# boqian-li/GarmentDreamer

Measured on AMD Instinct MI355X. Metric: SDS iters/sec (rasterize+UNet+bwd), 100k Gaussians ×8 views @512², 1/2/4/8 GPU, higher is better.
Workload: dtype bf16

## Files before the change

garmentdreamer_amd/csrc/nn_conv3x3.hip:

```cpp
#include <hip/hip_runtime.h>
#include <stdlib.h>
#include <stdint.h>
#include <stdio.h>

#include <mutex>
#include <vector>

#include "../../include/gd_nn.h"
#include "nn_device.h"
#include "nn_host.h"

#ifndef GD_CONV_ABLATE
#define GD_CONV_ABLATE 0
#endif

namespace {

using namespace gdnn;

#ifndef GD_PATCH_EPI
#define GD_PATCH_EPI 0
#endif
typedef __attribute__((ext_vector_type(4))) float f32x4;

// ... 15 lines not shown
    constexpr int NA = BM * 8 / THREADS;
    constexpr int NB = BN * 8 / THREADS;
    constexpr int FA = BN / WN / 32;
    constexpr int FB = BM / WM / 32;
    constexpr int kStage = (BM + BN) * BK * 2;
    extern __shared__ __attribute__((aligned(16))) char smem[];
    const int tid = threadIdx.x, lane = tid & 63;
    const int wave = __builtin_amdgcn_readfirstlane(tid >> 6);
    int bid = bid_raw;
    if ((nwg & 7) == 0) bid = (bid & 7) * (nwg >> 3) + (bid >> 3);
    const int tn = bid % tiles_n, tm = bid / tiles_n;
    const int m0 = tm * BM, n0 = tn * BN;
    const int HW = g.Hg * g.Wg;
    const int64_t M = (int64_t)Nimg * HW;
    const int H = g.Hin, W = g.Win;

    const uint32_t row_bytes = (uint32_t)Cin * 2u;
    const uint32_t back = (uint32_t)g.back * row_bytes;
    const __amdgpu_buffer_rsrc_t rs_in = buffer_rsrc((const char*)in - back, (uint32_t)Nimg * (uint32_t)(H * W) * row_bytes + back);
    const __amdgpu_buffer_rsrc_t rs_w = buffer_rsrc(wt, (uint32_t)Cout * (uint32_t)g.wtaps * row_bytes);

    uint32_t a_off[NA];
    int a_y[NA], a_x[NA];
    uint32_t b_off[NB];
#pragma unroll
    for (int i = 0; i < NA; i++) {
        const int q = tid + THREADS * i;
        const int line = q >> 4, c = (q & 15) ^ (line & 15);
        const int r = 2 * line + (c >> 3);
        const int64_t m = (int64_t)m0 + r;
        if (m < M) {
            const int nimg = (int)(m / HW);
            const int rem = (int)(m - (int64_t)nimg * HW);
            const int ga = rem / g.Wg;
            a_y[i] = ga * g.sy;
            a_x[i] = (rem - ga * g.Wg) * g.sx;
            a_off[i] = (uint32_t)((nimg * H + a_y[i]) * W + a_x[i]) * row_bytes + (uint32_t)(c & 7) * 16u;
        } else {
            a_y[i] = -100000; a_x[i] = 0; a_off[i] = kOOB;
        }
    }
#pragma unroll
    for (int i = 0; i < NB; i++) {
        const int q = tid + THREADS * i;
        const int line = q >> 4, c = (q & 15) ^ (line & 15);
        const int r = 2 * line + (c >> 3);
        const int co = n0 + r;
        b_off[i] = co < Cout ? (uint32_t)co * (uint32_t)g.wtaps * row_bytes + (uint32_t)(c & 7) * 16u : kOOB;
    }
    const int kc = Cin / BK;
    const int step0 = partial ? split_idx * steps_per_split : 0;
    const int step1 = partial ? min(g.ntaps * kc, step0 + steps_per_split) : g.ntaps * kc;
    const int nsteps = step1 - step0;
    const int tap0 = step0 / kc;

    int ld_tap = tap0, ld_c = step0 - tap0 * kc;
    uint32_t a_voff[NA];
    auto set_tap = [&](int tap) {
        const int dy = (int)((g.ty4 >> (4 * tap)) & 15u) - 8, dx = (int)((g.tx4 >> (4 * tap)) & 15u) - 8;
#pragma unroll
        for (int i = 0; i < NA; i++) {
            const int yy = a_y[i] + dy, xx = a_x[i] + dx;
            const bool ok = (unsigned)yy < (unsigned)H && (unsigned)xx < (unsigned)W;
            a_voff[i] = ok ? a_off[i] : kOOB;
        }
    };
    set_tap(tap0);
    auto issue = [&](int buf) {
        char* sA = smem + buf * kStage;
        char* sB = sA + BM * BK * 2;
        const int dy = (int)((g.ty4 >> (4 * ld_tap)) & 15u) - 8, dx = (int)((g.tx4 >> (4 * ld_tap)) & 15u) - 8;
        const uint32_t soff_a = (uint32_t)(dy * W + dx + g.back) * row_bytes + (uint32_t)ld_c * (BK * 2);
        const uint32_t soff_b = (uint32_t)((g.w4 >> (4 * ld_tap)) & 15u) * row_bytes + (uint32_t)ld_c * (BK * 2);
#if GD_CONV_ABLATE != 1 && GD_CONV_ABLATE != 2 && GD_CONV_ABLATE < 6
#pragma unroll
        for (int i = 0; i < NA; i++) bload_lds16(rs_in, a_voff[i], soff_a, sA + (wave * 64 + THREADS * i) * 16);
#endif
#if GD_CONV_ABLATE != 2 && GD_CONV_ABLATE < 6
#pragma unroll
        for (int i = 0; i < NB; i++) bload_lds16(rs_w, b_off[i], soff_b, sB + (wave * 64 + THREADS * i) * 16);
#endif
        if (++ld_c == kc) {
            ld_c = 0;
            if (++ld_tap < g.ntaps) set_tap(ld_tap);
        }
    };

    f32x16 acc[FA][FB];
#pragma unroll
    for (int a = 0; a < FA; a++)
#pragma unroll
        for (int b = 0; b < FB; b++)
#pragma unroll
            for (int k = 0; k < 16; k++) acc[a][b][k] = 0.f;

    const int wc = wave % WN, wp = wave / WN;
    const int frow = lane & 31, fk = lane >> 5;
    uint32_t w_rd[FA], p_rd[FB];
#pragma unroll
    for (int a = 0; a < FA; a++) w_rd[a] = (uint32_t)(BM * BK * 2 + swz(wc * (BN / WN) + a * 32 + frow, fk));
#pragma unroll
    for (int b = 0; b < FB; b++) p_rd[b] = (uint32_t)swz(wp * (BM / WM) + b * 32 + frow, fk);

#if GD_CONV_ABLATE == 4 || GD_CONV_ABLATE >= 6
    bf16x8_t wf0[FA], pf0[FB];
#pragma unroll
    for (int a = 0; a < FA; a++) wf0[a] = *(const bf16x8_t*)(smem + w_rd[a]);
#pragma unroll
    for (int b = 0; b < FB; b++) pf0[b] = *(const bf16x8_t*)(smem + p_rd[b]);
#endif
    issue(0);
#if GD_CONV_ABLATE == 8
    for (int s = 0; s < (nsteps > 1 ? 1 : nsteps); s++) {
#else
    for (int s = 0; s < nsteps; s++) {
#endif
        const int buf = s & 1;
        asm volatile("s_waitcnt vmcnt(0)" ::: "memory");
#if GD_CONV_ABLATE != 5 && GD_CONV_ABLATE != 6
        __syncthreads();
#endif
        if (s + 1 < nsteps) issue(buf ^ 1);
        const char* st = smem + buf * kStage;
#pragma unroll
        for (int kk = 0; kk < 4; kk++) {
            bf16x8_t wf[FA], pf[FB];
#if GD_CONV_ABLATE == 4 || GD_CONV_ABLATE >= 6
            if (s > 0) {
#pragma unroll
                for (int a = 0; a < FA; a++)
#pragma unroll
                    for (int b = 0; b < FB; b++)
                        acc[a][b] = __builtin_amdgcn_mfma_f32_32x32x16_bf16(wf0[a], pf0[b], acc[a][b], 0, 0, 0);
                continue;
            }
#endif
#pragma unroll
            for (int a = 0; a < FA; a++) wf[a] = *(const bf16x8_t*)(st + (w_rd[a] ^ (uint32_t)(kk << 5)));
#pragma unroll
            for (int b = 0; b < FB; b++) pf[b] = *(const bf16x8_t*)(st + (p_rd[b] ^ (uint32_t)(kk << 5)));
#pragma unroll
            for (int a = 0; a < FA; a++)
#pragma unroll
                for (int b = 0; b < FB; b++)
#if GD_CONV_ABLATE == 3
                    if (a == 0 && b == 0) acc[a][b] = __builtin_amdgcn_mfma_f32_32x32x16_bf16(wf[a], pf[b], acc[a][b], 0, 0, 0);
                    else { acc[a][b][0] += __builtin_bit_cast(float, (int)wf[a][0] ^ (int)pf[b][1]); }
#else
                    acc[a][b] = __builtin_amdgcn_mfma_f32_32x32x16_bf16(wf[a], pf[b], acc[a][b], 0, 0, 0);
#endif
        }
    }

#pragma unroll
    for (int b = 0; b < FB; b++) {
        const int64_t m = (int64_t)m0 + wp * (BM / WM) + b * 32 + (lane & 31);
        if (m >= M) continue;
        const int nimg = (int)(m / HW);
        const int rem = (int)(m - (int64_t)nimg * HW);
        const int ga = rem / g.Wg, gb = rem - ga * g.Wg;
        const size_t opix = ((size_t)nimg * g.Hout + (size_t)(ga * g.osy + g.ooy)) * g.Wout + (size_t)(gb * g.osx + g.oox);
        const uint16_t* bias_n = bias ? bias + (size_t)nimg * bias_img_stride : nullptr;
#pragma unroll
        for (int a = 0; a < FA; a++) {
#pragma unroll
            for (int q = 0; q < 4; q++) {
                const int co = n0 + wc * (BN / WN) + a * 32 + 8 * q + 4 * fk;
                if (co >= Cout) continue;
                float v[4];
#pragma unroll
                for (int e = 0; e < 4; e++) v[e] = acc[a][b][4 * q + e];
                if (partial) {
                    *(float4*)(partial + (((size_t)split_idx * nwg + bid) * (BN * BM / 4) +
                                          (((wave * FB + b) * FA + a) * 4 + q) * 64 + lane) * 4) = make_float4(v[0], v[1], v[2], v[3]);
                    continue;
                }
                if (bias_n) {
                    const uint2 bb = *(const uint2*)(bias_n + co);
                    v[0] += bf2f((uint16_t)(bb.x & 0xffff)); v[1] += bf2f((uint16_t)(bb.x >> 16));
                    v[2] += bf2f((uint16_t)(bb.y & 0xffff)); v[3] += bf2f((uint16_t)(bb.y >> 16));
                }
                if (residual) {
                    const uint2 rr = *(const uint2*)(residual + opix * Cout + co);
                    v[0] += bf2f((uint16_t)(rr.x & 0xffff)); v[1] += bf2f((uint16_t)(rr.x >> 16));
                    v[2] += bf2f((uint16_t)(rr.y & 0xffff)); v[3] += bf2f((uint16_t)(rr.y >> 16));
                }
                uint2 o;
                o.x = pack_bf16(v[0], v[1]);
                o.y = pack_bf16(v[2], v[3]);
                *(uint2*)(out + opix * Cout + co) = o;
            }
        }
    }
}

template <int BN, int BM, int WN, int WM>
__global__ __launch_bounds__(64 * WN * WM) void conv3x3_nhwc_bf16_kernel(
    const uint16_t* __restrict__ in, const uint16_t* __restrict__ wt, const uint16_t* __restrict__ bias,
    int bias_img_stride, const uint16_t* __restrict__ residual, uint16_t* __restrict__ out, int Nimg, const ConvGeom g,
    int Cin, int Cout, int tiles_n, int nwg, float* __restrict__ partial, int steps_per_split)
{
    conv3x3_nhwc_bf16_body<BN, BM, WN, WM>(in, wt, bias, bias_img_stride, residual, out, Nimg, g, Cin, Cout, tiles_n, nwg,
                                           partial, steps_per_split, (int)blockIdx.x, (int)blockIdx.y);
}

struct ConvGeomSet {
    ConvGeom g[4];
    const uint16_t* wt[4];
    int nwg[4];
    int n;
};

template <int BN, int BM, int WN, int WM>
__global__ __launch_bounds__(64 * WN * WM) void conv3x3_nhwc_bf16_multi_kernel(
    const uint16_t* __restrict__ in, const uint16_t* __restrict__ bias, int bias_img_stride,
    const uint16_t* __restrict__ residual, uint16_t* __restrict__ out, int Nimg, const ConvGeomSet gs, int Cin, int Cout,
    int tiles_n)
{
    const int cls = (int)blockIdx.z;
    const int nwg = gs.nwg[cls];
    if ((int)blockIdx.x >= nwg) return;
    conv3x3_nhwc_bf16_body<BN, BM, WN, WM>(in, gs.wt[cls], bias, bias_img_stride, residual, out, Nimg, gs.g[cls], Cin, Cout,
                                           tiles_n, nwg, nullptr, 0, (int)blockIdx.x, 0);
}

constexpr int kPatch = 18, kPatchPix = kPatch * kPatch;

__device__ __forceinline__ float silu_fast(float z) { return z * __builtin_amdgcn_rcpf(1.0f + __expf(-z)); }

__device__ __forceinline__ float row16_sum(float v)
{
    v += __builtin_bit_cast(float, __builtin_amdgcn_update_dpp(0, __builtin_bit_cast(int, v), 0xB1, 0xf, 0xf, false));
    v += __builtin_bit_cast(float, __builtin_amdgcn_update_dpp(0, __builtin_bit_cast(int, v), 0x4E, 0xf, 0xf, false));
    v += __builtin_bit_cast(float, __builtin_amdgcn_update_dpp(0, __builtin_bit_cast(int, v), 0x141, 0xf, 0xf, false));
    v += __builtin_bit_cast(float, __builtin_amdgcn_update_dpp(0, __builtin_bit_cast(int, v), 0x140, 0xf, 0xf, false));
    return v;
}

__device__ __forceinline__ void stat_accumulate(float2& st, uint2 o)
{
    const float r0 = __uint_as_float(o.x << 16), r1 = __uint_as_float(o.x & 0xffff0000u);
    const float r2 = __uint_as_float(o.y << 16), r3 = __uint_as_float(o.y & 0xffff0000u);
    st.x += (r0 + r1) + (r2 + r3);
    st.y += fmaf(r0, r0, fmaf(r1, r1, fmaf(r2, r2, r3 * r3)));
}

__device__ __forceinline__ void patch_col(int fn, int& rr, int& fx)
{
    if (fn < 4) { rr = 0; fx = fn; }
    else if (fn < 12) { rr = 1; fx = fn - 4; }
    else if (fn < 16) { rr = 0; fx = fn - 8; }
    else if (fn < 20) { rr = 1; fx = fn - 8; }
    else if (fn < 28) { rr = 0; fx = fn - 12; }
    else { rr = 1; fx = fn - 16; }
}

constexpr int kTrRow = 80;
constexpr int kTrWave = 64 * kTrRow;

constexpr int kResRound = 64 * 64;

__device__ __forceinline__ void res_tile_lane(int lane, uint32_t pix_bytes, uint32_t img_row_bytes, uint32_t (&off)[2])
{
    const uint32_t chunk = (uint32_t)((lane & 3) ^ ((lane >> 4) & 3));
#pragma unroll
    for (int h = 0; h < 2; h++) {
        int rr, fx;
        patch_col(16 * h + (lane >> 2), rr, fx);
        off[h] = (uint32_t)rr * img_row_bytes + (uint32_t)fx * pix_bytes + chunk * 16u;
    }
}

__device__ __forceinline__ void res_tile_issue(__amdgpu_buffer_rsrc_t rs, const uint32_t (&off)[2], uint32_t base,
                                               uint32_t two_rows, char* slot)
{
#pragma unroll
    for (int i = 0; i < 4; i++) bload_lds16(rs, off[i & 1], base + (uint32_t)(i >> 1) * two_rows, slot + i * 1024);
}

typedef __attribute__((ext_vector_type(2))) uint32_t res_u32x2;
typedef __attribute__((ext_vector_type(4))) uint32_t res_u32x4;

__device__ __forceinline__ void res_tile_read(uint32_t slot_off, int lane, res_u32x2 (&r)[2][4])
{
    const int fn = lane & 31, fk = lane >> 5;
    const uint32_t a0 = slot_off + (uint32_t)(fn * 64 + 8 * fk), key = (uint32_t)((fn >> 2) & 3);
    const uint32_t q0 = a0 + (key << 4), q1 = a0 + ((1u ^ key) << 4), q2 = a0 + ((2u ^ key) << 4), q3 = a0 + ((3u ^ key) << 4);
    asm volatile("ds_read_b64 %0, %8\n\tds_read_b64 %1, %9\n\tds_read_b64 %2, %10\n\tds_read_b64 %3, %11\n\t"
                 "ds_read_b64 %4, %8 offset:2048\n\tds_read_b64 %5, %9 offset:2048\n\t"
                 "ds_read_b64 %6, %10 offset:2048\n\tds_read_b64 %7, %11 offset:2048\n\ts_waitcnt lgkmcnt(0)"
                 : "=&v"(r[0][0]), "=&v"(r[0][1]), "=&v"(r[0][2]), "=&v"(r[0][3]), "=&v"(r[1][0]), "=&v"(r[1][1]),
                   "=&v"(r[1][2]), "=&v"(r[1][3])
                 : "v"(q0), "v"(q1), "v"(q2), "v"(q3)
                 : "memory");
}

struct ResTile {
    uint16_t* out;
    size_t pix0;
    int Cout;
    float* stat_img;
    int stat_rows, stat_row;
    bool stat_ok;
};

struct PatchPix {
    int W;
    __device__ __forceinline__ int operator()(int pr) const
    {
        int rr, fx;
        patch_col(pr & 31, rr, fx);
        return (2 * (pr >> 5) + rr) * W + fx;
    }
};

template <class PixOf, class AfterRead>
__device__ __forceinline__ void res_round(const f32x16& acc0, const f32x16& acc1, const uint2 (&bb)[4], uint32_t slot_off,
                                          uint32_t tr_off, int lane, const ResTile& t, int co0, PixOf pix_of,
                                          AfterRead after_read)
{
    const int fk = lane >> 5, fn = lane & 31;
    res_u32x2 rv[2][4];
    res_tile_read(slot_off, lane, rv);
    after_read();
#pragma unroll
    for (int q = 0; q < 4; q++) {
        const int co = co0 + 8 * q + 4 * fk;
        const float bv[4] = {bf2f((uint16_t)(bb[q].x & 0xffff)), bf2f((uint16_t)(bb[q].x >> 16)),
                             bf2f((uint16_t)(bb[q].y & 0xffff)), bf2f((uint16_t)(bb[q].y >> 16))};
        float2 st = make_float2(0.f, 0.f);
#pragma unroll
        for (int j = 0; j < 2; j++) {
            float v[4];
#pragma unroll
            for (int e = 0; e < 4; e++) v[e] = (j ? acc1 : acc0)[4 * q + e] + bv[e];
            const uint32_t r0 = rv[j][q][0], r1 = rv[j][q][1];
            v[0] += bf2f((uint16_t)(r0 & 0xffff)); v[1] += bf2f((uint16_t)(r0 >> 16));
            v[2] += bf2f((uint16_t)(r1 & 0xffff)); v[3] += bf2f((uint16_t)(r1 >> 16));
            uint2 o;
            o.x = pack_bf16(v[0], v[1]);
            o.y = pack_bf16(v[2], v[3]);
            const res_u32x2 ov = {o.x, o.y};
            asm volatile("ds_write_b64 %0, %1" ::"v"(tr_off + (uint32_t)((j * 32 + fn) * kTrRow + 16 * q + 8 * fk)), "v"(ov)
                         : "memory");
            if (t.stat_img) stat_accumulate(st, o);
        }
        if (t.stat_img) {
            const float sx = row16_sum(st.x), sy = row16_sum(st.y);
            if ((lane & 15) == 0 && t.stat_ok)
                *(float2*)(t.stat_img + ((size_t)(co >> 2) * t.stat_rows + t.stat_row + ((lane >> 4) & 1)) * 2) =
                    make_float2(sx, sy);
        }
    }
    res_u32x4 tv[4];
    asm volatile("ds_read_b128 %0, %4\n\tds_read_b128 %1, %4 offset:1280\n\tds_read_b128 %2, %4 offset:2560\n\t"
                 "ds_read_b128 %3, %4 offset:3840\n\ts_waitcnt lgkmcnt(0)"
                 : "=&v"(tv[0]), "=&v"(tv[1]), "=&v"(tv[2]), "=&v"(tv[3])
                 : "v"(tr_off + (uint32_t)((lane >> 2) * kTrRow + (lane & 3) * 16))
                 : "memory");
    static_assert(16 * kTrRow == 1280, "offsets of the four reads");
#pragma unroll
    for (int i = 0; i < 4; i++) {
        const int pr = (lane >> 2) + 16 * i;
        *(uint4*)(t.out + (t.pix0 + (size_t)pix_of(pr)) * t.Cout + co0 + 8 * (lane & 3)) =
            make_uint4(tv[i][0], tv[i][1], tv[i][2], tv[i][3]);
    }
}

template <int BN, int WN, int FA, int FB>
__device__ __forceinline__ void patch_epilogue(f32x16 (&acc)[FA][FB], char* tr, int nimg, int tyi, int txi, int n0, int wc,
                                               int wp, int lane, int H, int W, int Cout, const uint16_t* __restrict__ bias,
                                               int bias_img_stride, const uint16_t* __restrict__ residual,
                                               uint16_t* __restrict__ out, float* __restrict__ stat_part, int tpi,
                                               int tiles_x)
{
    const int fk = lane >> 5, fn = lane & 31;
    int rr, fx;
    patch_col(fn, rr, fx);
    bool ok[FB];
    size_t opix[FB];
#pragma unroll
    for (int b = 0; b < FB; b++) {
        const int oy = tyi * 16 + 4 * wp + 2 * b + rr, ox = txi * 16 + fx;
        ok[b] = oy < H && ox < W;
        opix[b] = ((size_t)nimg * H + oy) * W + ox;
    }
    const uint16_t* bias_n = bias ? bias + (size_t)nimg * bias_img_stride : nullptr;
    const int stat_rows = tpi * 8;
    const int stat_row = (tyi * tiles_x + txi) * 8 + wp * 2 + ((lane >> 4) & 1);
    const bool wide = GD_PATCH_EPI != 2 && tr != nullptr && (Cout & 7) == 0;
#pragma unroll
    for (int a = 0; a < FA; a++) {
#pragma unroll
        for (int q = 0; q < 4; q++) {
            const int co = n0 + wc * (BN / WN) + a * 32 + 8 * q + 4 * fk;
            const bool cok = co < Cout;
            float bv[4] = {0.f, 0.f, 0.f, 0.f};
            if (bias_n && cok) {
                const uint2 bb = *(const uint2*)(bias_n + co);
                bv[0] = bf2f((uint16_t)(bb.x & 0xffff)); bv[1] = bf2f((uint16_t)(bb.x >> 16));
                bv[2] = bf2f((uint16_t)(bb.y & 0xffff)); bv[3] = bf2f((uint16_t)(bb.y >> 16));
            }
            float2 st = make_float2(0.f, 0.f);
#pragma unroll
            for (int b = 0; b < FB; b++) {
                if (!ok[b] || !cok) continue;
                float v[4];
#pragma unroll
                for (int e = 0; e < 4; e++) v[e] = acc[a][b][4 * q + e] + bv[e];
                if (residual) {
                    const uint2 rv = *(const uint2*)(residual + opix[b] * Cout + co);
                    v[0] += bf2f((uint16_t)(rv.x & 0xffff)); v[1] += bf2f((uint16_t)(rv.x >> 16));
                    v[2] += bf2f((uint16_t)(rv.y & 0xffff)); v[3] += bf2f((uint16_t)(rv.y >> 16));
                }
                uint2 o;
                o.x = pack_bf16(v[0], v[1]);
                o.y = pack_bf16(v[2], v[3]);
                if (wide) *(uint2*)(tr + (b * 32 + fn) * kTrRow + 16 * q + 8 * fk) = o;
                else if (GD_PATCH_EPI != 1 || H < 0) *(uint2*)(out + opix[b] * Cout + co) = o;
                if (stat_part) stat_accumulate(st, o);
            }
            if (stat_part) {
                const float sx = row16_sum(st.x), sy = row16_sum(st.y);
                if ((lane & 15) == 0 && cok)
                    *(float2*)(stat_part + (((size_t)nimg * (Cout >> 2) + (co >> 2)) * stat_rows + stat_row) * 2) =
                        make_float2(sx, sy);
            }
        }
        if (wide) {
            __builtin_amdgcn_wave_barrier();
#pragma unroll
            for (int i = 0; i < FB * 2; i++) {
                const int pr = (lane >> 2) + 16 * i, ch = lane & 3;
                int rr2, fx2;
                patch_col(pr & 31, rr2, fx2);
                const int oy = tyi * 16 + 4 * wp + 2 * (pr >> 5) + rr2, ox = txi * 16 + fx2;
                const int co8 = n0 + wc * (BN / WN) + a * 32 + 8 * ch;
                if (oy < H && ox < W && co8 < Cout) {
                    const uint4 v = *(const uint4*)(tr + pr * kTrRow + ch * 16);
                    if (GD_PATCH_EPI != 1 || H < 0) *(uint4*)(out + (((size_t)nimg * H + oy) * W + ox) * Cout + co8) = v;
                }
            }
            __builtin_amdgcn_wave_barrier();
        }
    }
}

template <int BN, int WN, int WM, bool GN, bool RES>
__global__ __launch_bounds__(64 * WN * WM) void conv3x3_gn_patch_kernel(
    const uint16_t* __restrict__ in, const uint16_t* __restrict__ wt, const uint16_t* __restrict__ bias,
    int bias_img_stride, const uint16_t* __restrict__ residual, uint16_t* __restrict__ out, int Nimg, int H, int W,
    int Cin, int Cout, const float* __restrict__ mean_rstd, const uint16_t* __restrict__ gamma,
    const uint16_t* __restrict__ beta, int G, int apply_silu, int tiles_n, int tiles_x, int tiles_y, int nwg,
    float* __restrict__ stat_part)
{
    constexpr int BM = 256;
    constexpr int THREADS = 64 * WN * WM;
    constexpr int NB = BN * 8 / THREADS;
    constexpr int NA = (kPatchPix * 8 + THREADS - 1) / THREADS;
    constexpr int FA = BN / WN / 32, FB = BM / WM / 32;
    static_assert(FB == 2 && THREADS % 8 == 0, "wave pixel block = 4 patch rows x 16");
    constexpr int kAStage = (kPatchPix + 4) * BK * 2;
    constexpr int kBStage = BN * BK * 2;
    extern __shared__ __attribute__((aligned(16))) char smem[];
    char* sA = smem;
    char* sB = smem + 2 * kAStage;

    const int tid = threadIdx.x, lane = tid & 63;
    const int wave = __builtin_amdgcn_readfirstlane(tid >> 6);
    int bid = blockIdx.x;
    if ((nwg & 7) == 0) bid = (bid & 7) * (nwg >> 3) + (bid >> 3);
    const int tn = bid % tiles_n, tm = bid / tiles_n;
    const int tpi = tiles_x * tiles_y;
    const int nimg = tm / tpi, trem = tm - nimg * tpi;
    const int tyi = trem / tiles_x, txi = trem - tyi * tiles_x;
    const int y0 = tyi * 16 - 1, x0 = txi * 16 - 1;
    const int n0 = tn * BN;

    const uint32_t row_bytes = (uint32_t)Cin * 2u;
    const __amdgpu_buffer_rsrc_t rs_in = buffer_rsrc(in, (uint32_t)Nimg * (uint32_t)(H * W) * row_bytes);
    const __amdgpu_buffer_rsrc_t rs_w = buffer_rsrc(wt, (uint32_t)Cout * 9u * row_bytes);

    const int a_chunk = tid & 7;
    uint32_t a_goff[NA];
    uint32_t a_lds[NA];
    uint32_t a_keep = 0;
    uint32_t a_slot = 0;
#pragma unroll
    for (int i = 0; i < NA; i++) {
        const int pix = (tid + THREADS * i) >> 3;
        const int py = pix / kPatch, px = pix - py * kPatch;
        const int gy = y0 + py, gx = x0 + px;
        const bool slot = pix < kPatchPix;
        const bool inimg = slot && (unsigned)gy < (unsigned)H && (unsigned)gx < (unsigned)W;
        const int oct = GN ? a_chunk : (a_chunk ^ ((pix >> 1) & 7));
        a_goff[i] = inimg ? (uint32_t)((nimg * H + gy) * W + gx) * row_bytes + (uint32_t)oct * 16u : kOOB;
        a_lds[i] = (uint32_t)pix * 128u + (uint32_t)((a_chunk ^ ((pix >> 1) & 7)) << 4);
        if (inimg) a_keep |= 1u << i;
        if (slot) a_slot |= 1u << i;
    }
    uint4 a_reg[NA];
    auto loadA = [&](int c) {
#pragma unroll
        for (int i = 0; i < NA; i++) {
            auto v = __builtin_amdgcn_raw_buffer_load_b128(rs_in, (int)a_goff[i], (int)(c * (BK * 2)), 0);
            a_reg[i] = __builtin_bit_cast(uint4, v);
        }
    };
    const uint32_t tab_off = (uint32_t)(uintptr_t)(smem + 2 * kAStage + 2 * kBStage);
    auto storeA = [&](int buf, int c) {
        const uint32_t dst_off = (uint32_t)(uintptr_t)(sA + buf * kAStage);
        float sc[8], sh[8];
        if (mean_rstd) gn_table_read(tab_off, c * (BK / 8) + a_chunk, sc, sh);
#pragma unroll
        for (int i = 0; i < NA; i++) {
            if (!((a_slot >> i) & 1u)) continue;
            uint4 v = a_reg[i];
            if (mean_rstd) {
                uint32_t w4[4] = {v.x, v.y, v.z, v.w};
                const bool keep = (a_keep >> i) & 1u;
#pragma unroll
                for (int k = 0; k < 4; k++) {
                    float lo = __uint_as_float(w4[k] << 16), hi = __uint_as_float(w4[k] & 0xffff0000u);
                    lo = lo * sc[2 * k] + sh[2 * k];
                    hi = hi * sc[2 * k + 1] + sh[2 * k + 1];
                    if (apply_silu) { lo = silu_fast(lo); hi = silu_fast(hi); }
                    w4[k] = keep ? pack_bf16(lo, hi) : 0u;
                }
                v = make_uint4(w4[0], w4[1], w4[2], w4[3]);
            }
            typedef __attribute__((ext_vector_type(4))) uint32_t vec4;
            const vec4 vv = {v.x, v.y, v.z, v.w};
            asm volatile("ds_write_b128 %0, %1" ::"v"(dst_off + a_lds[i]), "v"(vv) : "memory");
        }
    };

    uint32_t b_off[NB];
#pragma unroll
    for (int i = 0; i < NB; i++) {
        const int q = tid + THREADS * i;
        const int line = q >> 4, cc = (q & 15) ^ (line & 15);
        const int r = 2 * line + (cc >> 3);
        const int co = n0 + r;
        b_off[i] = co < Cout ? (uint32_t)co * 9u * row_bytes + (uint32_t)(cc & 7) * 16u : kOOB;
    }
    auto issueB = [&](int buf, int tap, int c) {
        char* dst = sB + buf * kBStage;
        const uint32_t soff = (uint32_t)tap * row_bytes + (uint32_t)c * (BK * 2);
#pragma unroll
        for (int i = 0; i < NB; i++) bload_lds16(rs_w, b_off[i], soff, dst + (wave * 64 + THREADS * i) * 16);
    };

    f32x16 acc[FA][FB];
#pragma unroll
    for (int a = 0; a < FA; a++)
#pragma unroll
        for (int b = 0; b < FB; b++)
#pragma unroll
            for (int k = 0; k < 16; k++) acc[a][b][k] = 0.f;

    const int wc = wave % WN, wp = wave / WN;
    const int fk = lane >> 5, fn = lane & 31;
    int rr, fx;
    if (fn < 4) { rr = 0; fx = fn; }
    else if (fn < 12) { rr = 1; fx = fn - 4; }
    else if (fn < 16) { rr = 0; fx = fn - 8; }
    else if (fn < 20) { rr = 1; fx = fn - 8; }
    else if (fn < 28) { rr = 0; fx = fn - 12; }
    else { rr = 1; fx = fn - 16; }
    uint32_t w_rd[FA];
    int p_base[FB];
#pragma unroll
    for (int a = 0; a < FA; a++) w_rd[a] = (uint32_t)swz(wc * (BN / WN) + a * 32 + fn, fk);
#pragma unroll
    for (int b = 0; b < FB; b++) p_base[b] = (4 * wp + 2 * b + rr) * kPatch + fx;

    const int kc = Cin / BK;
    const int nsteps = 9 * kc;
    auto issueA = [&](int buf, int c) {
        char* dst = sA + buf * kAStage;
#pragma unroll
        for (int i = 0; i < NA; i++) {
            if (i == NA - 1 && wave * 64 + THREADS * i >= kPatchPix * 8) continue;
            bload_lds16(rs_in, a_goff[i], (uint32_t)c * (BK * 2), dst + (wave * 64 + THREADS * i) * 16);
        }
    };
    static_assert(FA == 2 || FA == 4, "rounds of the residual tile");
    const bool dma = RES && residual != nullptr && (Cout & 7) == 0 && tyi * 16 + 16 <= H && txi * 16 + 16 <= W && n0 + BN <= Cout &&
                     (uint64_t)Nimg * (uint64_t)(H * W) * (uint64_t)Cout * 2u < (1ull << 32);
    const uint32_t res_pix = (uint32_t)Cout * 2u, res_row = (uint32_t)W * res_pix;
    const __amdgpu_buffer_rsrc_t rs_res = buffer_rsrc(residual, (uint32_t)Nimg * (uint32_t)(H * W) * res_pix);
    auto res_slot = [&](int r) -> char* {
        if (r == 0 || r == 3) return sA + (kc & 1) * kAStage + wave * kResRound;
        return sB + (r - 1) * (8 * kResRound) + wave * kResRound;
    };
    auto issueR = [&](int r) {
        uint32_t off[2];
        res_tile_lane(lane, res_pix, res_row, off);
        const uint32_t base = (uint32_t)((nimg * H + tyi * 16 + 4 * wp) * W + txi * 16) * res_pix +
                              (uint32_t)(n0 + wc * (BN / WN) + r * 32) * 2u;
        res_tile_issue(rs_res, off, base, 2u * res_row, res_slot(r));
    };

    if (GN) {
        if (mean_rstd) gn_table_fill(tab_off, tid, THREADS, Cin, G, nimg, mean_rstd, gamma, beta);
        loadA(0);
        issueB(0, 0, 0);
        if (mean_rstd) gn_table_sync();
        storeA(0, 0);
    } else {
        issueA(0, 0);
        issueB(0, 0, 0);
    }
    int s = 0;
    for (int c = 0; c < kc; c++) {
        const char* pa = sA + (c & 1) * kAStage;
        for (int tap = 0; tap < 9; tap++, s++) {
            const int bufB = s & 1;
            if (GN) asm volatile("s_waitcnt vmcnt(0) lgkmcnt(0)" ::: "memory");
            else asm volatile("s_waitcnt vmcnt(0)" ::: "memory");
            __syncthreads();
            if (s + 1 < nsteps) issueB(bufB ^ 1, tap == 8 ? 0 : tap + 1, tap == 8 ? c + 1 : c);
            if (c + 1 < kc) {
                if (GN) {
                    if (tap == 0) loadA(c + 1);
                    else if (tap == 1) storeA((c + 1) & 1, c + 1);
                } else if (tap == 0) {
                    issueA((c + 1) & 1, c + 1);
                }
            } else if (tap == 0 && dma) {
                issueR(0);
            }
            const char* pb = sB + bufB * kBStage;
            const int tapoff = (tap / 3) * kPatch + (tap % 3);
            uint32_t p_rd[FB], p_sw[FB];
#pragma unroll
            for (int b = 0; b < FB; b++) {
                const int p = p_base[b] + tapoff;
                p_rd[b] = (uint32_t)p * 128u;
                p_sw[b] = (uint32_t)((p >> 1) & 7);
            }
#pragma unroll
            for (int kk = 0; kk < 4; kk++) {
                bf16x8_t wf[FA], pf[FB];
#pragma unroll
                for (int a = 0; a < FA; a++) wf[a] = *(const bf16x8_t*)(pb + (w_rd[a] ^ (uint32_t)(kk << 5)));
#pragma unroll
                for (int b = 0; b < FB; b++)
                    pf[b] = *(const bf16x8_t*)(pa + p_rd[b] + ((((uint32_t)(2 * kk + fk)) ^ p_sw[b]) << 4));
#pragma unroll
                for (int a = 0; a < FA; a++)
#pragma unroll
                    for (int b = 0; b < FB; b++)
                        acc[a][b] = __builtin_amdgcn_mfma_f32_32x32x16_bf16(wf[a], pf[b], acc[a][b], 0, 0, 0);
            }
        }
    }

    if (GD_PATCH_EPI != 2) __syncthreads();
    if (GD_PATCH_EPI == 0 && dma) {
        const uint32_t tr_off = (uint32_t)(uintptr_t)(sA + ((kc - 1) & 1) * kAStage + wave * kTrWave);
        const uint16_t* bias_d = bias ? bias + (size_t)nimg * bias_img_stride : nullptr;
        uint2 bb[FA][4];
#pragma unroll
        for (int a = 0; a < FA; a++)
#pragma unroll
            for (int q = 0; q < 4; q++)
                bb[a][q] = bias_d ? *(const uint2*)(bias_d + n0 + wc * (BN / WN) + a * 32 + 8 * q + 4 * fk) : make_uint2(0u, 0u);
        asm volatile("" ::: "memory");
        issueR(1);
        if (FA == 4) issueR(2);
        ResTile t;
        t.out = out; t.Cout = Cout;
        t.pix0 = ((size_t)nimg * H + (tyi * 16 + 4 * wp)) * W + txi * 16;
        t.stat_rows = tpi * 8;
        t.stat_img = stat_part ? stat_part + (size_t)nimg * (Cout >> 2) * t.stat_rows * 2 : nullptr;
        t.stat_row = (tyi * tiles_x + txi) * 8 + wp * 2;
        t.stat_ok = true;
#pragma unroll
        for (int r = 0; r < FA; r++) {
            if (r == FA - 3) asm volatile("s_waitcnt vmcnt(8)" ::: "memory");
            else if (r == FA - 2 && r > 0) asm volatile("s_waitcnt vmcnt(4)" ::: "memory");
            else if (r == FA - 1) asm volatile("s_waitcnt vmcnt(0)" ::: "memory");
            res_round(acc[r][0], acc[r][1], bb[r], (uint32_t)(uintptr_t)res_slot(r), tr_off, lane, t,
                      n0 + wc * (BN / WN) + r * 32, PatchPix{W}, [&] { if (FA == 4 && r == 0) issueR(3); });
        }
        return;
    }
    patch_epilogue<BN, WN, FA, FB>(acc, sA + ((kc - 1) & 1) * kAStage + wave * kTrWave, nimg, tyi, txi, n0, wc, wp, lane, H, W,
                                   Cout, bias, bias_img_stride, residual, out, stat_part, tpi, tiles_x);
}

template <int BN, int WN, int WM, bool GN>
__global__ __launch_bounds__(64 * WN * WM) void conv3x3_patch_stream_kernel(
    const uint16_t* __restrict__ in, const uint16_t* __restrict__ wt, const uint16_t* __restrict__ bias,
    int bias_img_stride, const uint16_t* __restrict__ residual, uint16_t* __restrict__ out, int Nimg, int H, int W,
    int Cin, int Cout, const float* __restrict__ mean_rstd, const uint16_t* __restrict__ gamma,
    const uint16_t* __restrict__ beta, int G, int apply_silu, int tiles_n, int tiles_x, int tiles_y, int nwg,
    float* __restrict__ stat_part)
{
    constexpr int BM = 256;
    constexpr int THREADS = 64 * WN * WM;
    constexpr int NB = BN * 8 / THREADS;
    constexpr int NA = (kPatchPix * 8 + THREADS - 1) / THREADS;
    constexpr int FA = BN / WN / 32, FB = BM / WM / 32;
    static_assert(FB == 2 && THREADS % 8 == 0, "wave pixel block = 4 patch rows x 16");
    constexpr int kAStage = (kPatchPix + 4) * BK * 2;
    constexpr int kBStage = BN * BK * 2;
    extern __shared__ __attribute__((aligned(16))) char smem[];
    char* sA = smem;
    char* sB = smem + 2 * kAStage;

    const int tid = threadIdx.x, lane = tid & 63;
    const int wave = __builtin_amdgcn_readfirstlane(tid >> 6);
    const int tpi = tiles_x * tiles_y;
    const bool remap = (nwg & 7) == 0 && (GN || (gridDim.x & 7) == 0);
    struct Tile { int nimg, tyi, txi, n0; };
    auto decode = [&](int vb) {
        int bid = vb;
        if (remap) bid = (vb & 7) * (nwg >> 3) + (vb >> 3);
        const int tn = bid % tiles_n, tm = bid / tiles_n;
        Tile t;
        t.nimg = tm / tpi;
        const int trem = tm - t.nimg * tpi;
        t.tyi = trem / tiles_x;
        t.txi = trem - t.tyi * tiles_x;
        t.n0 = tn * BN;
        return t;
    };

    const uint32_t row_bytes = (uint32_t)Cin * 2u;
    const __amdgpu_buffer_rsrc_t rs_in = buffer_rsrc(in, (uint32_t)Nimg * (uint32_t)(H * W) * row_bytes);
    const __amdgpu_buffer_rsrc_t rs_w = buffer_rsrc(wt, (uint32_t)Cout * 9u * row_bytes);

    const int a_chunk = tid & 7;
    uint32_t a_goff[NA];
    uint32_t a_lds[NA];
    uint32_t a_keep = 0;
    uint32_t a_slot = 0;
#pragma unroll
    for (int i = 0; i < NA; i++) {
        const int pix = (tid + THREADS * i) >> 3;
        a_lds[i] = (uint32_t)pix * 128u + (uint32_t)((a_chunk ^ ((pix >> 1) & 7)) << 4);
        if (pix < kPatchPix) a_slot |= 1u << i;
    }
    auto setupA = [&](const Tile& t) {
        const int y0 = t.tyi * 16 - 1, x0 = t.txi * 16 - 1;
        a_keep = 0;
#pragma unroll
        for (int i = 0; i < NA; i++) {
            const int pix = (tid + THREADS * i) >> 3;
            const int py = pix / kPatch, px = pix - py * kPatch;
            const int gy = y0 + py, gx = x0 + px;
            const bool inimg = pix < kPatchPix && (unsigned)gy < (unsigned)H && (unsigned)gx < (unsigned)W;
            const int oct = GN ? a_chunk : (a_chunk ^ ((pix >> 1) & 7));
            a_goff[i] = inimg ? (uint32_t)((t.nimg * H + gy) * W + gx) * row_bytes + (uint32_t)oct * 16u : kOOB;
            if (inimg) a_keep |= 1u << i;
        }
    };
    uint4 a_reg[NA];
    auto loadA = [&](int c) {
#pragma unroll
        for (int i = 0; i < NA; i++) {
            auto v = __builtin_amdgcn_raw_buffer_load_b128(rs_in, (int)a_goff[i], (int)(c * (BK * 2)), 0);
            a_reg[i] = __builtin_bit_cast(uint4, v);
        }
    };
    const uint32_t tab_off = (uint32_t)(uintptr_t)(smem + 2 * kAStage + 2 * kBStage);
    auto storeA = [&](int buf, int c) {
        const uint32_t dst_off = (uint32_t)(uintptr_t)(sA + buf * kAStage);
        float sc[8], sh[8];
        if (mean_rstd) gn_table_read(tab_off, c * (BK / 8) + a_chunk, sc, sh);
#pragma unroll
        for (int i = 0; i < NA; i++) {
            if (!((a_slot >> i) & 1u)) continue;
            uint4 v = a_reg[i];
            if (mean_rstd) {
                uint32_t w4[4] = {v.x, v.y, v.z, v.w};
                const bool keep = (a_keep >> i) & 1u;
#pragma unroll
                for (int k = 0; k < 4; k++) {
                    float lo = __uint_as_float(w4[k] << 16), hi = __uint_as_float(w4[k] & 0xffff0000u);
                    lo = lo * sc[2 * k] + sh[2 * k];
                    hi = hi * sc[2 * k + 1] + sh[2 * k + 1];
                    if (apply_silu) { lo = silu_fast(lo); hi = silu_fast(hi); }
                    w4[k] = keep ? pack_bf16(lo, hi) : 0u;
                }
                v = make_uint4(w4[0], w4[1], w4[2], w4[3]);
            }
            typedef __attribute__((ext_vector_type(4))) uint32_t vec4;
            const vec4 vv = {v.x, v.y, v.z, v.w};
            asm volatile("ds_write_b128 %0, %1" ::"v"(dst_off + a_lds[i]), "v"(vv) : "memory");
        }
    };

    uint32_t b_off[NB];
    auto setupB = [&](const Tile& t) {
#pragma unroll
        for (int i = 0; i < NB; i++) {
            const int q = tid + THREADS * i;
            const int line = q >> 4, cc = (q & 15) ^ (line & 15);
            const int r = 2 * line + (cc >> 3);
            const int co = t.n0 + r;
            b_off[i] = co < Cout ? (uint32_t)co * 9u * row_bytes + (uint32_t)(cc & 7) * 16u : kOOB;
        }
    };
    auto issueB = [&](int buf, int tap, int c) {
        char* dst = sB + buf * kBStage;
        const uint32_t soff = (uint32_t)tap * row_bytes + (uint32_t)c * (BK * 2);
#pragma unroll
        for (int i = 0; i < NB; i++) bload_lds16(rs_w, b_off[i], soff, dst + (wave * 64 + THREADS * i) * 16);
    };

    f32x16 acc[FA][FB];

    const int wc = wave % WN, wp = wave / WN;
    const int fk = lane >> 5, fn = lane & 31;
    int rr, fx;
    if (fn < 4) { rr = 0; fx = fn; }
    else if (fn < 12) { rr = 1; fx = fn - 4; }
    else if (fn < 16) { rr = 0; fx = fn - 8; }
    else if (fn < 20) { rr = 1; fx = fn - 8; }
    else if (fn < 28) { rr = 0; fx = fn - 12; }
    else { rr = 1; fx = fn - 16; }
    uint32_t w_rd[FA];
    int p_base[FB];
#pragma unroll
    for (int a = 0; a < FA; a++) w_rd[a] = (uint32_t)swz(wc * (BN / WN) + a * 32 + fn, fk);
#pragma unroll
    for (int b = 0; b < FB; b++) p_base[b] = (4 * wp + 2 * b + rr) * kPatch + fx;

    const int kc = Cin / BK;
    auto issueA = [&](int buf, int c) {
        char* dst = sA + buf * kAStage;
#pragma unroll
        for (int i = 0; i < NA; i++) {
            if (i == NA - 1 && wave * 64 + THREADS * i >= kPatchPix * 8) continue;
            bload_lds16(rs_in, a_goff[i], (uint32_t)c * (BK * 2), dst + (wave * 64 + THREADS * i) * 16);
        }
    };
    int vb = blockIdx.x;
    Tile cur = decode(vb);
    setupB(cur);
    setupA(cur);
#pragma unroll
    for (int a = 0; a < FA; a++)
#pragma unroll
        for (int b = 0; b < FB; b++)
#pragma unroll
            for (int k = 0; k < 16; k++) acc[a][b][k] = 0.f;
    if (GN) {
        if (mean_rstd) gn_table_fill(tab_off, tid, THREADS, Cin, G, cur.nimg, mean_rstd, gamma, beta);
        loadA(0);
        issueB(0, 0, 0);
        if (mean_rstd) gn_table_sync();
        storeA(0, 0);
    } else {
        issueA(0, 0);
        issueB(0, 0, 0);
    }
    int s = 0;
    int ga = 0;
    for (;;) {
        const int vnext = vb + (int)gridDim.x;
        const bool has_next = !GN && vnext < nwg;
        const Tile nxt = decode(has_next ? vnext : vb);
        for (int c = 0; c < kc; c++, ga++) {
            const char* pa = sA + (ga & 1) * kAStage;
            const bool last_chunk = c + 1 == kc;
            if (last_chunk && has_next) setupA(nxt);
            for (int tap = 0; tap < 9; tap++, s++) {
                const int bufB = s & 1;
                if (GN) asm volatile("s_waitcnt vmcnt(0) lgkmcnt(0)" ::: "memory");
                else asm volatile("s_waitcnt vmcnt(0)" ::: "memory");
                __syncthreads();
                if (!(last_chunk && tap == 8)) {
                    issueB(bufB ^ 1, tap == 8 ? 0 : tap + 1, tap == 8 ? c + 1 : c);
                } else if (has_next) {
                    setupB(nxt);
                    issueB(bufB ^ 1, 0, 0);
                }
                if (!last_chunk || has_next) {
                    const int nc = last_chunk ? 0 : c + 1;
                    const int st = (ga + 1) & 1;
                    if (GN) {
                        if (tap == 0) loadA(nc);
                        else if (tap == 1) storeA(st, nc);
                    } else if (tap == 0) {
                        issueA(st, nc);
                    }
                }
                const char* pb = sB + bufB * kBStage;
                const int tapoff = (tap / 3) * kPatch + (tap % 3);
                uint32_t p_rd[FB], p_sw[FB];
#pragma unroll
                for (int b = 0; b < FB; b++) {
                    const int p = p_base[b] + tapoff;
                    p_rd[b] = (uint32_t)p * 128u;
                    p_sw[b] = (uint32_t)((p >> 1) & 7);
                }
#pragma unroll
                for (int kk = 0; kk < 4; kk++) {
                    bf16x8_t wf[FA], pf[FB];
#pragma unroll
                    for (int a = 0; a < FA; a++) wf[a] = *(const bf16x8_t*)(pb + (w_rd[a] ^ (uint32_t)(kk << 5)));
#pragma unroll
                    for (int b = 0; b < FB; b++)
                        pf[b] = *(const bf16x8_t*)(pa + p_rd[b] + ((((uint32_t)(2 * kk + fk)) ^ p_sw[b]) << 4));
#pragma unroll
                    for (int a = 0; a < FA; a++)
#pragma unroll
                        for (int b = 0; b < FB; b++)
                            acc[a][b] = __builtin_amdgcn_mfma_f32_32x32x16_bf16(wf[a], pf[b], acc[a][b], 0, 0, 0);
                }
            }
        }

        if (GD_PATCH_EPI != 2) __syncthreads();
        patch_epilogue<BN, WN, FA, FB>(acc, sA + ((ga - 1) & 1) * kAStage + wave * kTrWave, cur.nimg, cur.tyi, cur.txi, cur.n0,
                                       wc, wp, lane, H, W, Cout, bias, bias_img_stride, residual, out, stat_part, tpi,
                                       tiles_x);
        if (!has_next) break;
        cur = nxt;
        vb = vnext;
#pragma unroll
        for (int a = 0; a < FA; a++)
#pragma unroll
            for (int b = 0; b < FB; b++)
#pragma unroll
                for (int k = 0; k < 16; k++) acc[a][b][k] = 0.f;
    }
}

#include "nn_conv_wino.h"
#include "nn_conv_wide.h"
#include "nn_conv_first_dgrad.h"
#ifdef GD_NN_EXPERIMENTAL_STREAM
#include "nn_conv_stream.h"
#endif
#ifdef GD_NN_EXPERIMENTAL_REGW
#include "nn_conv_regw.h"
#endif

template <int BM_T>
__global__ __launch_bounds__(256) void conv_splitk_reduce_kernel(const float* __restrict__ partial, int S, int nwg,
                                                                 int tiles_n, int64_t M, int Cout, int HWg, int Wg, int Hout,
                                                                 int Wout, int osy, int osx, int ooy, int oox,
                                                                 const uint16_t* __restrict__ bias, int bias_img_stride,
                                                                 const uint16_t* __restrict__ residual,
                                                                 uint16_t* __restrict__ out)
{
    constexpr int kQuads = 128 * BM_T / 4, kBlocks = kQuads / 256;
    const int tile = blockIdx.x / kBlocks;
    const int r = ((blockIdx.x % kBlocks) << 8) | threadIdx.x;
    const int lane = r & 63, q = (r >> 6) & 3, a = (r >> 8) & 1, b = (r >> 9) & 1, wave = r >> 10;
    const int tn = tile % tiles_n, tm = tile / tiles_n;
    const int64_t m = (int64_t)tm * BM_T + (wave >> 1) * 64 + b * 32 + (lane & 31);
    const int co = tn * 128 + (wave & 1) * 64 + a * 32 + 8 * q + 4 * (lane >> 5);
    if (m >= M || co >= Cout) return;
    float4 v = make_float4(0.f, 0.f, 0.f, 0.f);
    const float4* p = (const float4*)partial + (size_t)tile * kQuads + r;
    for (int sidx = 0; sidx < S; sidx++) {
        const float4 t = p[(size_t)sidx * nwg * kQuads];
        v.x += t.x; v.y += t.y; v.z += t.z; v.w += t.w;
    }
    const size_t nimg = (size_t)(m / HWg);
    const int rem = (int)(m - (int64_t)nimg * HWg);
    const int ga = rem / Wg, gb = rem - ga * Wg;
    const size_t o = ((nimg * Hout + (size_t)(ga * osy + ooy)) * Wout + (size_t)(gb * osx + oox)) * Cout + co;
    if (bias) {
        const uint2 bb = *(const uint2*)(bias + nimg * (size_t)bias_img_stride + co);
        v.x += bf2f((uint16_t)(bb.x & 0xffff)); v.y += bf2f((uint16_t)(bb.x >> 16));
        v.z += bf2f((uint16_t)(bb.y & 0xffff)); v.w += bf2f((uint16_t)(bb.y >> 16));
    }
    if (residual) {
        const uint2 rr = *(const uint2*)(residual + o);
        v.x += bf2f((uint16_t)(rr.x & 0xffff)); v.y += bf2f((uint16_t)(rr.x >> 16));
        v.z += bf2f((uint16_t)(rr.y & 0xffff)); v.w += bf2f((uint16_t)(rr.y >> 16));
    }
    uint2 ov;
    ov.x = pack_bf16(v.x, v.y);
    ov.y = pack_bf16(v.z, v.w);
    *(uint2*)(out + o) = ov;
}

template <int CIN>
__global__ __launch_bounds__(256) void conv3x3_first_kernel(const uint16_t* __restrict__ in,
                                                            const uint16_t* __restrict__ wt,
                                                            const uint16_t* __restrict__ bias,
                                                            uint16_t* __restrict__ out, int Nimg, int H, int W, int Cout)
{
    constexpr int PX = 4;
    extern __shared__ __attribute__((aligned(16))) float s_w[];
    const int K = 9 * CIN;
    for (int i = threadIdx.x; i < K * Cout; i += 256) {
        const int k = i / Cout, co = i - k * Cout;
        s_w[i] = bf2f(wt[(size_t)co * K + k]);
    }
    __syncthreads();
    const int octs = Cout >> 3;
    const int oct = threadIdx.x % octs, grp = threadIdx.x / octs;
    const int gpb = 256 / octs;
    const int gx = (W + PX - 1) / PX;
    const int64_t total = (int64_t)Nimg * H * gx;
    if (grp >= gpb) return;
    for (int64_t g = (int64_t)blockIdx.x * gpb + grp; g < total; g += (int64_t)gridDim.x * gpb) {
    const int n = (int)((uint32_t)g / (uint32_t)(H * gx));
    const int rem = (int)((uint32_t)g - (uint32_t)n * (uint32_t)(H * gx));
    const int y = rem / gx, x0 = (rem - y * gx) * PX;

    float acc[PX][8];
    {
        const uint4 bq = bias ? *(const uint4*)(bias + oct * 8) : make_uint4(0, 0, 0, 0);
        const uint32_t bw[4] = {bq.x, bq.y, bq.z, bq.w};
#pragma unroll
        for (int p = 0; p < PX; p++)
#pragma unroll
            for (int k = 0; k < 8; k++) acc[p][k] = bf2f((uint16_t)(bw[k >> 1] >> ((k & 1) * 16)));
    }
#pragma unroll 1
    for (int r = 0; r < 3; r++) {
        const int yy = y + r - 1;
        if ((unsigned)yy >= (unsigned)H) continue;
        const uint16_t* row = in + ((size_t)n * H + yy) * W * CIN;
        float win[PX + 2][CIN];
#pragma unroll
        for (int c = 0; c < PX + 2; c++) {
            const int xx = x0 + c - 1;
            const bool ok = (unsigned)xx < (unsigned)W;
#pragma unroll
            for (int ci = 0; ci < CIN; ci++) win[c][ci] = ok ? bf2f(row[(size_t)(ok ? xx : 0) * CIN + ci]) : 0.f;
        }
        const float* wr = s_w + (size_t)r * 3 * CIN * Cout + oct * 8;
#pragma unroll
        for (int kx = 0; kx < 3; kx++)
#pragma unroll
            for (int ci = 0; ci < CIN; ci++) {
                const float4 w0 = *(const float4*)(wr + (kx * CIN + ci) * Cout);
                const float4 w1 = *(const float4*)(wr + (kx * CIN + ci) * Cout + 4);
                const float wv[8] = {w0.x, w0.y, w0.z, w0.w, w1.x, w1.y, w1.z, w1.w};
#pragma unroll
                for (int p = 0; p < PX; p++) {
                    const float xv = win[p + kx][ci];
#pragma unroll
                    for (int k = 0; k < 8; k++) acc[p][k] += xv * wv[k];
                }
            }
    }
#pragma unroll
    for (int p = 0; p < PX; p++) {
        if (x0 + p >= W) break;
        uint4 o;
        o.x = pack_bf16(acc[p][0], acc[p][1]); o.y = pack_bf16(acc[p][2], acc[p][3]);
        o.z = pack_bf16(acc[p][4], acc[p][5]); o.w = pack_bf16(acc[p][6], acc[p][7]);
        *(uint4*)(out + (((size_t)n * H + y) * W + x0 + p) * Cout + oct * 8) = o;
    }
    }
}

template <int CIN>
__global__ __launch_bounds__(256) void conv3x3_first_mfma_kernel(const uint16_t* __restrict__ in,
                                                                 const uint16_t* __restrict__ wt,
                                                                 const uint16_t* __restrict__ bias,
                                                                 uint16_t* __restrict__ out, int Nimg, int H, int W,
                                                                 float* __restrict__ stat_part)
{
    constexpr int K = 9 * CIN, KS = (K + 16) / 16, FA = 4, Cout = 128;
    const int lane = threadIdx.x & 63, fn = lane & 31, fk = lane >> 5;
    const int wave_g = blockIdx.x * 4 + (threadIdx.x >> 6), nwaves = gridDim.x * 4;
    const int segs_x = (W + 31) >> 5;
    const int64_t segs = (int64_t)H * segs_x;

    int tap[KS][8];
    bf16x8_t wa[FA][KS];
#pragma unroll
    for (int s = 0; s < KS; s++) {
#pragma unroll
        for (int j = 0; j < 8; j++) {
            const int k = 16 * s + 8 * fk + j;
            const int ky = k / (3 * CIN), kx = (k / CIN) % 3, ci = k % CIN;
            const int need = k == K ? 32 : k > K ? 16 : ((ky == 0 ? 1 : 0) | (ky == 2 ? 2 : 0) | (kx == 0 ? 4 : 0) | (kx == 2 ? 8 : 0));
            const int off = k >= K ? 0 : ((ky - 1) * W + (kx - 1)) * CIN + ci;
            tap[s][j] = off * 64 + need;
        }
#pragma unroll
        for (int a = 0; a < FA; a++) {
            short w8[8];
#pragma unroll
            for (int j = 0; j < 8; j++) {
                const int k = 16 * s + 8 * fk + j;
                w8[j] = k < K ? (short)wt[(size_t)(32 * a + fn) * K + k] : (k == K && bias) ? (short)bias[32 * a + fn] : (short)0;
            }
            wa[a][s] = bf16x8_t{w8[0], w8[1], w8[2], w8[3], w8[4], w8[5], w8[6], w8[7]};
        }
    }

    int64_t t = wave_g;
    for (int n = 0; n < Nimg; n++) {
        float2 st[FA][4];
#pragma unroll
        for (int a = 0; a < FA; a++)
#pragma unroll
            for (int q = 0; q < 4; q++) st[a][q] = make_float2(0.f, 0.f);
        for (; t < (int64_t)(n + 1) * segs; t += nwaves) {
            const int seg = (int)(t - (int64_t)n * segs);
            const int y = seg / segs_x, x = (seg - y * segs_x) * 32 + fn;
            const bool pix_ok = x < W;
            const int have = pix_ok ? ((y > 0 ? 1 : 0) | (y < H - 1 ? 2 : 0) | (x > 0 ? 4 : 0) | (x < W - 1 ? 8 : 0)) : 0;
            const uint16_t* base = in + (((size_t)n * H + y) * W + (pix_ok ? x : 0)) * CIN;
            f32x16 acc[FA];
#pragma unroll
            for (int a = 0; a < FA; a++)
#pragma unroll
                for (int r = 0; r < 16; r++) acc[a][r] = 0.f;
#pragma unroll
            for (int s = 0; s < KS; s++) {
                short p8[8];
#pragma unroll
                for (int j = 0; j < 8; j++) {
                    const int need = tap[s][j] & 63;
                    const bool ok = pix_ok && (need & ~have) == 0;
                    p8[j] = need == 32 ? (short)0x3F80 : ok ? (short)base[tap[s][j] >> 6] : (short)0;
                }
                const bf16x8_t pb = bf16x8_t{p8[0], p8[1], p8[2], p8[3], p8[4], p8[5], p8[6], p8[7]};
#pragma unroll
                for (int a = 0; a < FA; a++) acc[a] = __builtin_amdgcn_mfma_f32_32x32x16_bf16(wa[a][s], pb, acc[a], 0, 0, 0);
            }
            uint16_t* orow = out + (((size_t)n * H + y) * W + x) * Cout + 8 * fk;
#pragma unroll
            for (int a = 0; a < FA; a++) {
#pragma unroll
                for (int q = 0; q < 4; q += 2) {
                    uint2 o0, o1;
                    o0.x = pack_bf16(acc[a][4 * q], acc[a][4 * q + 1]);
                    o0.y = pack_bf16(acc[a][4 * q + 2], acc[a][4 * q + 3]);
                    o1.x = pack_bf16(acc[a][4 * q + 4], acc[a][4 * q + 5]);
                    o1.y = pack_bf16(acc[a][4 * q + 6], acc[a][4 * q + 7]);
                    if (stat_part && pix_ok) {
                        stat_accumulate(st[a][q], o0);
                        stat_accumulate(st[a][q + 1], o1);
                    }
                    const auto sx = __builtin_amdgcn_permlane32_swap(o0.x, o1.x, false, false);
                    const auto sy = __builtin_amdgcn_permlane32_swap(o0.y, o1.y, false, false);
                    if (pix_ok) *(uint4*)(orow + 32 * a + 8 * q) = make_uint4(sx[0], sy[0], sx[1], sy[1]);
                }
            }
        }
        if (stat_part) {
            const int rows = nwaves * 2, row = wave_g * 2 + ((lane >> 4) & 1);
#pragma unroll
            for (int a = 0; a < FA; a++) {
#pragma unroll
                for (int q = 0; q < 4; q++) {
                    const float sx = row16_sum(st[a][q].x), sy = row16_sum(st[a][q].y);
                    const int quad = 8 * a + 2 * q + fk;
                    if ((lane & 15) == 0)
                        *(float2*)(stat_part + (((size_t)n * (Cout >> 2) + quad) * rows + row) * 2) = make_float2(sx, sy);
                }
            }
        }
    }
}

__global__ void conv3x3_flip_weights_kernel(const uint16_t* __restrict__ w, uint16_t* __restrict__ wf, int Cout,
                                            int Cin)
{
    const size_t total = (size_t)Cout * 9 * Cin;
    for (size_t i = (size_t)blockIdx.x * blockDim.x + threadIdx.x; i < total; i += (size_t)gridDim.x * blockDim.x) {
        const int co = (int)(i % Cout);
        const int tap = (int)((i / Cout) % 9);
        const int ci = (int)(i / ((size_t)Cout * 9));
        wf[i] = w[((size_t)co * 9 + (8 - tap)) * Cin + ci];
    }
}

int g_route_scale = 1;
int g_force_split = -1;
int g_force_variant = -1;

struct ConvEnv {
    int split_px = 0;
    int multi_class = 1;
    int patch_persistent = 1;
    int first_grid = 2048;
};
const ConvEnv& conv_env()
{
    static const ConvEnv env = [] {
        ConvEnv v;
        if (const char* e = getenv("GD_NN_SPLIT_PX")) v.split_px = atoi(e);
        if (const char* e = getenv("GD_NN_CONV_MULTI")) v.multi_class = atoi(e);
        if (const char* e = getenv("GD_NN_PATCH_PERSISTENT")) v.patch_persistent = atoi(e) != 0;
        if (const char* e = getenv("GD_NN_FIRST_GRID")) v.first_grid = atoi(e) > 0 ? atoi(e) : v.first_grid;
        return v;
    }();
    return env;
}

int num_cus(int dev)
{
    static const int cus = [dev] {
        int c = 0;
        return hipDeviceGetAttribute(&c, hipDeviceAttributeMultiprocessorCount, dev) == hipSuccess && c > 0 ? c : 256;
    }();
    return cus;
}

struct ConvProf {
    std::mutex mu;
    bool on = false;
    struct Rec { hipEvent_t a, b; };
    std::vector<Rec> pending;
    std::vector<hipEvent_t> pool;
    double total_ms = 0, total_flops = 0, total_bytes = 0;
    int64_t launches = 0;
    hipEvent_t get()
    {
        if (!pool.empty()) { hipEvent_t e = pool.back(); pool.pop_back(); return e; }
        hipEvent_t e;
        return hipEventCreate(&e) == hipSuccess ? e : nullptr;
    }
} g_cprof;

struct ProfScope {
    hipStream_t s;
    hipEvent_t a = nullptr, b = nullptr;
    ProfScope(const ProfScope&) = delete;
    ProfScope& operator=(const ProfScope&) = delete;
    explicit ProfScope(hipStream_t stream) : s(stream)
    {
        if (!g_cprof.on) return;
        std::lock_guard<std::mutex> lk(g_cprof.mu);
        a = g_cprof.get(); b = g_cprof.get();
        if (a && b) (void)hipEventRecord(a, s);
    }
    void close(double flops, double bytes)
    {
        if (!a || !b) return;
        (void)hipEventRecord(b, s);
        std::lock_guard<std::mutex> lk(g_cprof.mu);
        g_cprof.pending.push_back({a, b});
        g_cprof.total_flops += flops;
        g_cprof.total_bytes += bytes;
        a = b = nullptr;
    }
    ~ProfScope()
    {
        if (!a && !b) return;
        std::lock_guard<std::mutex> lk(g_cprof.mu);
        if (a) g_cprof.pool.push_back(a);
        if (b) g_cprof.pool.push_back(b);
    }
    void close_s1(int64_t M, int Cin, int Cout, bool residual)
    {
        close(2.0 * (double)M * Cout * 9.0 * Cin,
              2.0 * ((double)M * Cin + 9.0 * Cin * Cout + (double)M * Cout + (residual ? (double)M * Cout : 0.0)));
    }
};

struct TiledArgs {
    void* stream;
    const void* x;
    const float* mean_rstd;
    const void *gamma, *beta;
    int groups, silu;
    const void *w, *bias;
    int bias_img_stride;
    const void* residual;
    void* y;
    int N, H, W, Cin, Cout;
    float* stat_part;
};
constexpr int kCuLds = 160 * 1024;
static bool gn_table_fits(int lds, int Cin) { return lds + gn_table_bytes(Cin) <= kCuLds; }
template <auto Kern>
int launch_tiled(const TiledArgs& a, int lds, int tile_w, int bn, bool persistent)
{
    const int dev = current_device();
    if (dev < 0) return dev;
    if (a.mean_rstd) {
        if (!gn_table_fits(lds, a.Cin)) return fail(GD_NN_ERR_INVALID_ARG, "GroupNorm scale / shift table of Cin channels does not fit the LDS");
        lds += gn_table_bytes(a.Cin);
    }
    if (const int r = reserve_lds<Kern>(dev, a.mean_rstd ? kCuLds : lds)) return r;
    hipStream_t s = (hipStream_t)a.stream;
    const int tiles_x = (a.W + tile_w - 1) / tile_w, tiles_y = (a.H + 15) / 16, tiles_n = (a.Cout + bn - 1) / bn;
    const int nwg = a.N * tiles_x * tiles_y * tiles_n;
    int grid = nwg;
    if (persistent && nwg > num_cus(dev)) grid = (nwg & 7) == 0 ? (num_cus(dev) & ~7) : num_cus(dev);
    ProfScope prof(s);
    hipLaunchKernelGGL(Kern, dim3(grid), dim3(512), lds, s, (const uint16_t*)a.x, (const uint16_t*)a.w,
                       (const uint16_t*)a.bias, a.bias_img_stride, (const uint16_t*)a.residual, (uint16_t*)a.y, a.N, a.H,
                       a.W, a.Cin, a.Cout, a.mean_rstd, (const uint16_t*)a.gamma, (const uint16_t*)a.beta, a.groups, a.silu,
                       tiles_n, tiles_x, tiles_y, nwg, a.stat_part);
    prof.close_s1((int64_t)a.N * a.H * a.W, a.Cin, a.Cout, a.residual != nullptr);
    return launch_status();
}

}

extern "C" {

const char* gd_nn_conv_last_error(void) { return g_err; }

static int pick_split(int64_t tiles, int steps, int target = 420)
{
    int s = (int)((target + tiles / 2) / tiles);
    const int cap = steps * 2 / 15 < 24 ? steps * 2 / 15 : 24;
    if (s > cap) s = cap;
    return s < 2 ? 1 : s;
}

static size_t split_ws_bytes(int split, int64_t M, int Cout)
{
    return (size_t)split * (size_t)((M + 255) / 256 * 2) * (size_t)((Cout + 127) / 128) * 16384u * sizeof(float);
}

static int split_tile_px(int64_t M, int Cout)
{
    const int forced = conv_env().split_px;
    if (forced == 128 || forced == 256) return forced;
    M *= g_route_scale;
    return (M >= 1024 && Cout >= 1024) || M >= 2048 ? 256 : 128;
}

static bool small_tile_nosplit(int64_t M, int Cout, int ntaps, int Cin)
{
    if (g_force_split >= 0 || g_force_variant >= 0) return false;
    M *= g_route_scale;
    const int64_t t128 = ((M + 127) / 128) * ((Cout + 127) / 128), t64 = ((M + 63) / 64) * ((Cout + 63) / 64);
    return ntaps == 9 && Cin <= 320 && Cout <= 320 && Cout % 8 == 0 && t128 < 256 && t64 >= 256;
}

static int choose_split(int64_t M, int Cout, int ntaps, int Cin)
{
    const int steps = ntaps * (Cin / BK);
    if (g_force_split >= 0) return g_force_split > 1 && g_force_split <= steps ? g_force_split : 1;
    if (small_tile_nosplit(M, Cout, ntaps, Cin)) return 1;
    const int px = split_tile_px(M, Cout);
    M *= g_route_scale;
    if (((M + 127) / 128) * ((Cout + 127) / 128) >= 256) return 1;
    const int64_t tiles = ((M + px - 1) / px) * ((Cout + 127) / 128);
    if (tiles >= 256 || Cout % 8 || steps < 8) return 1;
    return pick_split(tiles, steps, px == 256 ? 256 : 420);
}

static void add_tap(ConvGeom& g, int dy, int dx, int widx)
{
    g.ty4 |= (uint64_t)(dy + 8) << (4 * g.ntaps);
    g.tx4 |= (uint64_t)(dx + 8) << (4 * g.ntaps);
    g.w4 |= (uint64_t)widx << (4 * g.ntaps);
    g.ntaps++;
}

static int finalize_geom(ConvGeom& g, int N, int Cin, int Cout)
{
    int minlin = 0;
    for (int t = 0; t < g.ntaps; t++) {
        const int dy = (int)((g.ty4 >> (4 * t)) & 15u) - 8, dx = (int)((g.tx4 >> (4 * t)) & 15u) - 8;
        minlin = dy * g.Win + dx < minlin ? dy * g.Win + dx : minlin;
    }
    g.back = -minlin;
    if (g.wtaps == 0) g.wtaps = 9;
    if (((double)N * g.Hin * g.Win + g.back) * Cin * 2.0 >= 2147483648.0 || (double)Cout * 9.0 * Cin * 2.0 >= 2147483648.0)
        return fail(GD_NN_ERR_INVALID_ARG, "conv3x3: activation / weight tensor must be < 2 GiB (32-bit buffer offsets)");
    return GD_NN_OK;
}

static int tile_variant(int64_t M, int Cin, int Cout)
{
    const int64_t Ms = M * g_route_scale;
    const int64_t t256 = ((Ms + 255) / 256) * ((Cout + 255) / 256);
    const int64_t t128x256 = ((Ms + 255) / 256) * ((Cout + 127) / 128);
    if (Cout % 256 == 0 && t256 >= 192) return 2;
    return t128x256 >= 512 && (Cin >= 512 || Ms >= (1 << 20)) ? 1 : 0;
}

static int s1_geom(ConvGeom& g, const void* x, const void* weight, const void* y, int N, int H, int W, int Cin, int Cout)
{
    if (!x || !weight || !y) return fail(GD_NN_ERR_INVALID_ARG, "null pointer");
    if (N <= 0 || H <= 0 || W <= 0 || Cin % BK || Cout % 4 || Cin <= 0 || Cout <= 0)
        return fail(GD_NN_ERR_INVALID_ARG, "conv3x3: need Cin % 64 == 0 and Cout % 4 == 0");
    g = ConvGeom{};
    g.Hin = g.Hg = g.Hout = H;
    g.Win = g.Wg = g.Wout = W;
    g.sy = g.sx = g.osy = g.osx = 1;
    for (int ky = 0; ky < 3; ky++)
        for (int kx = 0; kx < 3; kx++) add_tap(g, ky - 1, kx - 1, ky * 3 + kx);
    return GD_NN_OK;
}

static int launch_conv(hipStream_t s, const void* x, const void* weight, const void* bias, int bias_img_stride,
                       const void* residual, void* y, int N, ConvGeom g, int Cin, int Cout, void* ws = nullptr,
                       size_t ws_bytes = 0)
{
    const int dev = current_device();
    if (dev < 0) return dev;
    if (const int r = finalize_geom(g, N, Cin, Cout)) return r;
    const int64_t M = (int64_t)N * g.Hg * g.Wg;
    if (M <= 0) return GD_NN_OK;
    int split = ws ? choose_split(M, Cout, g.ntaps, Cin) : 1;
    if (split > 1 && ws_bytes < split_ws_bytes(split, M, Cout)) split = 1;
    float* partial = split > 1 ? (float*)ws : nullptr;
    const int total_steps = g.ntaps * (Cin / BK);
    const int tps = split > 1 ? (total_steps + split - 1) / split : total_steps;
    if (split > 1) split = (total_steps + tps - 1) / tps;
    const int spx = split > 1 ? split_tile_px(M, Cout) : 128;
    int variant = split > 1 ? (spx == 256 ? 1 : 0) : g_force_variant;
    if (variant < 0 && small_tile_nosplit(M, Cout, g.ntaps, Cin)) variant = 6;
    if (variant < 0)
        variant = Cout <= 32 && M * g_route_scale >= (1 << 18) ? 4 : tile_variant(M, Cin, Cout);
    ProfScope prof(s);
#define GD_LAUNCH(BN_, BM_, WN_, WM_)                                                                              \
    do {                                                                                                           \
        constexpr auto kern = conv3x3_nhwc_bf16_kernel<BN_, BM_, WN_, WM_>;                                        \
        constexpr int lds = 2 * (BN_ + BM_) * BK * 2;                                                              \
        if (const int r = reserve_lds<kern>(dev, lds)) return r;                                                   \
        const int tiles_m = (int)((M + BM_ - 1) / BM_), tiles_n = (Cout + BN_ - 1) / BN_;                          \
        const int nwg = tiles_m * tiles_n;                                                                         \
        hipLaunchKernelGGL(kern, dim3(nwg, split), dim3(64 * WN_ * WM_), lds, s, (const uint16_t*)x,               \
                           (const uint16_t*)weight, (const uint16_t*)bias, bias_img_stride,                        \
                           (const uint16_t*)residual, (uint16_t*)y, N, g, Cin, Cout, tiles_n, nwg, partial, tps);  \
    } while (0)
    if (variant == 2) GD_LAUNCH(256, 256, 2, 4);
    else if (variant == 4) GD_LAUNCH(32, 256, 1, 4);
    else if (variant == 1) GD_LAUNCH(128, 256, 2, 4);
    else if (variant == 5) GD_LAUNCH(64, 128, 2, 2);
    else if (variant == 6) GD_LAUNCH(64, 64, 2, 2);
    else if (variant == 7) GD_LAUNCH(128, 64, 2, 2);
    else GD_LAUNCH(128, 128, 2, 2);
#undef GD_LAUNCH
    if (split > 1) {
        const int tiles_n = (Cout + 127) / 128, nwg = (int)((M + spx - 1) / spx) * tiles_n;
        if (spx == 256)
            hipLaunchKernelGGL(conv_splitk_reduce_kernel<256>, dim3((unsigned)nwg * 32u), dim3(256), 0, s, partial, split, nwg,
                               tiles_n, M, Cout, g.Hg * g.Wg, g.Wg, g.Hout, g.Wout, g.osy, g.osx, g.ooy, g.oox,
                               (const uint16_t*)bias, bias_img_stride, (const uint16_t*)residual, (uint16_t*)y);
        else
            hipLaunchKernelGGL(conv_splitk_reduce_kernel<128>, dim3((unsigned)nwg * 16u), dim3(256), 0, s, partial, split, nwg,
                               tiles_n, M, Cout, g.Hg * g.Wg, g.Wg, g.Hout, g.Wout, g.osy, g.osx, g.ooy, g.oox,
                               (const uint16_t*)bias, bias_img_stride, (const uint16_t*)residual, (uint16_t*)y);
    }
    prof.close(2.0 * (double)M * Cout * (double)g.ntaps * Cin,
               2.0 * ((double)N * g.Hin * g.Win * Cin + (double)g.ntaps * Cin * Cout + (double)M * Cout +
                      (residual ? (double)M * Cout : 0.0)));
    return launch_status();
}

static int launch_conv_multi(hipStream_t s, const void* x, const void* const* weights, const void* bias, int bias_img_stride,
                             const void* residual, void* y, int N, ConvGeom* geoms, int ncls, int Cin, int Cout, bool may_split)
{
    if (!conv_env().multi_class || ncls < 2 || ncls > 4 || g_force_variant >= 0 || g_force_split >= 0) return 0;
    const int dev = current_device();
    if (dev < 0) return dev;
    int64_t Msum = 0;
    double flops = 0, bytes = 0;
    for (int c = 0; c < ncls; c++) {
        ConvGeom& g = geoms[c];
        if (const int r = finalize_geom(g, N, Cin, Cout)) return r;
        const int64_t M = (int64_t)N * g.Hg * g.Wg;
        if (M <= 0) return 0;
        if (may_split && choose_split(M, Cout, g.ntaps, Cin) > 1) return 0;
        Msum += M;
        flops += 2.0 * (double)M * Cout * (double)g.ntaps * Cin;
        bytes += 2.0 * ((double)g.ntaps * Cin * Cout + (double)M * Cout + (residual ? (double)M * Cout : 0.0));
    }
    bytes += 2.0 * (double)N * geoms[0].Hin * geoms[0].Win * Cin;
    const int variant = tile_variant(Msum, Cin, Cout);
    ProfScope prof(s);
#define GD_LAUNCH_M(BN_, BM_, WN_, WM_)                                                                            \
    do {                                                                                                           \
        constexpr auto kern = conv3x3_nhwc_bf16_multi_kernel<BN_, BM_, WN_, WM_>;                                  \
        constexpr int lds = 2 * (BN_ + BM_) * BK * 2;                                                              \
        if (const int r = reserve_lds<kern>(dev, lds)) return r;                                                   \
        ConvGeomSet gs = {};                                                                                       \
        gs.n = ncls;                                                                                               \
        const int tiles_n = (Cout + BN_ - 1) / BN_;                                                                \
        int nmax = 0;                                                                                              \
        for (int c = 0; c < ncls; c++) {                                                                           \
            gs.g[c] = geoms[c];                                                                                    \
            gs.wt[c] = (const uint16_t*)weights[c];                                                                \
            const int64_t M = (int64_t)N * geoms[c].Hg * geoms[c].Wg;                                              \
            gs.nwg[c] = (int)((M + BM_ - 1) / BM_) * tiles_n;                                                      \
            nmax = gs.nwg[c] > nmax ? gs.nwg[c] : nmax;                                                            \
        }                                                                                                          \
        hipLaunchKernelGGL(kern, dim3(nmax, 1, ncls), dim3(64 * WN_ * WM_), lds, s, (const uint16_t*)x,            \
                           (const uint16_t*)bias, bias_img_stride, (const uint16_t*)residual, (uint16_t*)y, N, gs, \
                           Cin, Cout, tiles_n);                                                                    \
    } while (0)
    if (variant == 2) GD_LAUNCH_M(256, 256, 2, 4);
    else if (variant == 1) GD_LAUNCH_M(128, 256, 2, 4);
    else GD_LAUNCH_M(128, 128, 2, 2);
#undef GD_LAUNCH_M
    prof.close(flops, bytes);
    const int r = launch_status();
    return r < 0 ? r : 1;
}

static int launch_patch(void* stream, const void* x, const float* mean_rstd, const void* gamma, const void* beta,
                        int groups, int apply_silu, const void* weight, const void* bias, int bias_img_stride,
                        const void* residual, void* y, int N, int H, int W, int Cin, int Cout,
                        float* stat_part = nullptr)
{
    if (!x || !weight || !y) return fail(GD_NN_ERR_INVALID_ARG, "null pointer");
    if (N <= 0 || H <= 0 || W <= 0 || Cin % BK || Cout % 4 || Cin <= 0 || Cout <= 0)
        return fail(GD_NN_ERR_INVALID_ARG, "conv3x3_gn: need Cin % 64 == 0 and Cout % 4 == 0");
    if (mean_rstd && (!gamma || !beta || groups <= 0 || Cin % groups))
        return fail(GD_NN_ERR_INVALID_ARG, "conv3x3_gn: GroupNorm needs gamma, beta and Cin % groups == 0");
    if ((double)N * H * W * Cin * 2.0 >= 2147483648.0 || (double)Cout * 9.0 * Cin * 2.0 >= 2147483648.0)
        return fail(GD_NN_ERR_INVALID_ARG, "conv3x3_gn: activation / weight tensor must be < 2 GiB (32-bit buffer offsets)");
    const TiledArgs a = {stream, x, mean_rstd, gamma, beta, groups, apply_silu, weight, bias, bias_img_stride, residual, y,
                         N, H, W, Cin, Cout, stat_part};
    int bn = (Cout % 256 == 0) ? 256 : 128;
    if (g_force_variant == 1 || g_force_variant == 0) bn = 128;
    if (g_force_variant == 2) bn = 256;
    const bool persistent = conv_env().patch_persistent != 0;
    constexpr auto lds = [](int slab) { return 2 * (kPatchPix + 4) * BK * 2 + 2 * slab * BK * 2; };
    if (mean_rstd && bn == 256 && !gn_table_fits(lds(256), Cin)) bn = 128;
    if (bn == 256) {
        if (!mean_rstd) return launch_tiled<conv3x3_patch_stream_kernel<256, 2, 4, false>>(a, lds(256), 16, 256, persistent);
        return residual ? launch_tiled<conv3x3_gn_patch_kernel<256, 2, 4, true, true>>(a, lds(256), 16, 256, false)
                        : launch_tiled<conv3x3_gn_patch_kernel<256, 2, 4, true, false>>(a, lds(256), 16, 256, false);
    }
    if (!mean_rstd) return launch_tiled<conv3x3_patch_stream_kernel<128, 2, 4, false>>(a, lds(128), 16, 128, persistent);
    return residual ? launch_tiled<conv3x3_gn_patch_kernel<128, 2, 4, true, true>>(a, lds(128), 16, 128, false)
                    : launch_tiled<conv3x3_gn_patch_kernel<128, 2, 4, true, false>>(a, lds(128), 16, 128, false);
}


static bool prefer_patch(int N, int H, int W, int Cout)
{
    if (g_force_variant >= 0 || g_force_split >= 0) return g_force_variant == 3;
    if (Cout < 64 || H < 16 || W < 16) return false;
    const int bn = Cout % 256 == 0 ? 256 : 128;
    const int64_t wgs = (int64_t)N * g_route_scale * ((H + 15) / 16) * ((W + 15) / 16) * ((Cout + bn - 1) / bn);
    return wgs >= 256;
}

size_t gd_nn_conv3x3_ws_bytes(int N, int H, int W, int Cin, int Cout)
{
    if (N <= 0 || H <= 0 || W <= 0 || Cout <= 0) return 0;
    if (prefer_patch(N, H, W, Cout)) return 0;
    const int64_t M = (int64_t)N * H * W;
    const int split = choose_split(M, Cout, 9, Cin);
    return split > 1 ? split_ws_bytes(split, M, Cout) : 0;
}

int gd_nn_conv_force_split(int s)
{
    g_force_split = s;
    return GD_NN_OK;
}

int gd_nn_conv_set_route_scale(int k)
{
    if (k < 1) return fail(GD_NN_ERR_INVALID_ARG, "conv route scale must be >= 1");
    g_route_scale = k;
    return GD_NN_OK;
}

int gd_nn_conv3x3_forward_ws(void* stream, const void* x, const void* weight, const void* bias, int bias_img_stride,
                             const void* residual, void* y, int N, int H, int W, int Cin, int Cout, void* ws,
                             size_t ws_bytes)
{
    ConvGeom g;
    if (const int r = s1_geom(g, x, weight, y, N, H, W, Cin, Cout)) return r;
    if (prefer_patch(N, H, W, Cout))
        return launch_patch(stream, x, nullptr, nullptr, nullptr, 0, 0, weight, bias, bias_img_stride, residual, y, N, H, W,
                            Cin, Cout);
    return launch_conv((hipStream_t)stream, x, weight, bias, bias_img_stride, residual, y, N, g, Cin, Cout, ws, ws_bytes);
}

int gd_nn_conv3x3_forward(void* stream, const void* x, const void* weight, const void* bias, int bias_img_stride,
                          const void* residual, void* y, int N, int H, int W, int Cin, int Cout)
{
    ConvGeom g;
    if (const int r = s1_geom(g, x, weight, y, N, H, W, Cin, Cout)) return r;
    return launch_conv((hipStream_t)stream, x, weight, bias, bias_img_stride, residual, y, N, g, Cin, Cout);
}

int gd_nn_conv3x3_gn_forward(void* stream, const void* x, const float* mean_rstd, const void* gamma, const void* beta,
                             int groups, int apply_silu, const void* weight, const void* bias, int bias_img_stride,
                             const void* residual, void* y, int N, int H, int W, int Cin, int Cout)
{
    return launch_patch(stream, x, mean_rstd, gamma, beta, groups, apply_silu, weight, bias, bias_img_stride, residual, y,
                        N, H, W, Cin, Cout);
}

size_t gd_nn_conv3x3_stat_rows(int N, int H, int W, int Cout, int gn_entry)
{
    if (N <= 0 || H <= 0 || W <= 0 || Cout <= 0 || Cout % 4) return 0;
    if (!gn_entry && !prefer_patch(N, H, W, Cout)) return 0;
    return (size_t)((H + 15) / 16) * ((W + 15) / 16) * 8;
}

int gd_nn_conv3x3_gn_forward_stats(void* stream, const void* x, const float* mean_rstd, const void* gamma,
                                   const void* beta, int groups, int apply_silu, const void* weight, const void* bias,
                                   int bias_img_stride, const void* residual, void* y, int N, int H, int W, int Cin,
                                   int Cout, float* stat_part)
{
    return launch_patch(stream, x, mean_rstd, gamma, beta, groups, apply_silu, weight, bias, bias_img_stride, residual, y,
                        N, H, W, Cin, Cout, stat_part);
}

int gd_nn_conv3x3_forward_stats(void* stream, const void* x, const void* weight, const void* bias, int bias_img_stride,
                                const void* residual, void* y, int N, int H, int W, int Cin, int Cout, float* stat_part)
{
    if (!stat_part) return fail(GD_NN_ERR_INVALID_ARG, "conv3x3_forward_stats: stat_part is NULL");
    if (!prefer_patch(N, H, W, Cout))
        return fail(GD_NN_ERR_INVALID_ARG, "conv3x3_forward_stats: this shape does not run on the patch-staged kernel "
                                           "(gd_nn_conv3x3_stat_rows() == 0)");
    return launch_patch(stream, x, nullptr, nullptr, nullptr, 0, 0, weight, bias, bias_img_stride, residual, y, N, H, W,
                        Cin, Cout, stat_part);
}


size_t gd_nn_conv3x3_wino_weights_bytes(int Cout, int Cin)
{
    if (Cout <= 0 || Cin <= 0 || Cin % kWinoCK) return 0;
    return (size_t)((Cout + 127) / 128) * 3 * (size_t)(Cin / kWinoCK) * (size_t)kWinoWStage;
}

int gd_nn_conv3x3_wino_weights(void* stream, const void* weight, void* u, int Cout, int Cin)
{
    if (!weight || !u || Cout <= 0 || Cin <= 0) return fail(GD_NN_ERR_INVALID_ARG, "wino_weights: bad argument");
    if (Cin % kWinoCK) return fail(GD_NN_ERR_INVALID_ARG, "wino_weights: Cin % 32 != 0");
    const size_t total = gd_nn_conv3x3_wino_weights_bytes(Cout, Cin) / 16;
    const int grid = (int)((total + 255) / 256 < 4096 ? (total + 255) / 256 : 4096);
    hipLaunchKernelGGL(conv3x3_wino_weights_kernel, dim3(grid), dim3(256), 0, (hipStream_t)stream, (const uint16_t*)weight,
                       (uint16_t*)u, Cout, Cin);
    return launch_status();
}

int gd_nn_conv3x3_wino_supported(int N, int H, int W, int Cin, int Cout)
{
    if (N <= 0 || H < 16 || W < 16 || Cin <= 0 || Cout < 64) return 0;
    if (Cin % kWinoCK || Cout % 8) return 0;
    if ((double)N * H * W * Cin * 2.0 >= 2147483648.0 || (double)gd_nn_conv3x3_wino_weights_bytes(Cout, Cin) >= 2147483648.0) return 0;
    return 1;
}

static int launch_wino(void* stream, const void* x, const float* mean_rstd, const void* gamma, const void* beta, int groups,
                       int apply_silu, const void* u, const void* bias, int bias_img_stride, const void* residual, void* y,
                       int N, int H, int W, int Cin, int Cout, float* stat_part)
{
    if (!x || !u || !y) return fail(GD_NN_ERR_INVALID_ARG, "null pointer");
    if (!gd_nn_conv3x3_wino_supported(N, H, W, Cin, Cout))
        return fail(GD_NN_ERR_INVALID_ARG, "conv3x3_wino: need Cin % 32 == 0, Cout % 8 == 0, Cout >= 64, H, W >= 16, tensors < 2 GiB");
    if (mean_rstd && (!gamma || !beta || groups <= 0 || Cin % groups))
        return fail(GD_NN_ERR_INVALID_ARG, "conv3x3_wino: GroupNorm needs gamma, beta and Cin % groups == 0");
    const TiledArgs a = {stream, x, mean_rstd, gamma, beta, groups, apply_silu, u, bias, bias_img_stride, residual, y,
                         N, H, W, Cin, Cout, stat_part};
    if (residual)
        return mean_rstd ? launch_tiled<conv3x3_wino_kernel<true, true>>(a, kWinoLds, 16, 128, false)
                         : launch_tiled<conv3x3_wino_kernel<false, true>>(a, kWinoLds, 16, 128, false);
    return mean_rstd ? launch_tiled<conv3x3_wino_kernel<true, false>>(a, kWinoLds, 16, 128, false)
                     : launch_tiled<conv3x3_wino_kernel<false, false>>(a, kWinoLds, 16, 128, false);
}

int gd_nn_conv3x3_wino_forward(void* stream, const void* x, const void* u, const void* bias, int bias_img_stride,
                               const void* residual, void* y, int N, int H, int W, int Cin, int Cout, float* stat_part)
{
    return launch_wino(stream, x, nullptr, nullptr, nullptr, 0, 0, u, bias, bias_img_stride, residual, y, N, H, W, Cin,
                       Cout, stat_part);
}

int gd_nn_conv3x3_wino_gn_forward(void* stream, const void* x, const float* mean_rstd, const void* gamma, const void* beta,
                                  int groups, int apply_silu, const void* u, const void* bias, int bias_img_stride,
                                  const void* residual, void* y, int N, int H, int W, int Cin, int Cout, float* stat_part)
{
    if (!mean_rstd) return fail(GD_NN_ERR_INVALID_ARG, "conv3x3_wino_gn: mean_rstd is NULL");
    return launch_wino(stream, x, mean_rstd, gamma, beta, groups, apply_silu, u, bias, bias_img_stride, residual, y, N, H, W,
                       Cin, Cout, stat_part);
}

size_t gd_nn_conv3x3_wide_weights_bytes(int Cout, int Cin)
{
    if (Cout <= 0 || Cin <= 0 || Cin % kWideCK) return 0;
    return (size_t)((Cout + 127) / 128) * 3 * (size_t)(Cin / kWideCK) * (size_t)kWideWStage;
}

int gd_nn_conv3x3_wide_weights(void* stream, const void* weight, void* u, int Cout, int Cin)
{
    if (!weight || !u || Cout <= 0 || Cin <= 0 || Cin % kWideCK) return fail(GD_NN_ERR_INVALID_ARG, "wide_weights: bad argument");
    const size_t total = gd_nn_conv3x3_wide_weights_bytes(Cout, Cin) / 16;
    const int grid = (int)((total + 255) / 256 < 4096 ? (total + 255) / 256 : 4096);
    hipLaunchKernelGGL(conv3x3_wide_weights_kernel, dim3(grid), dim3(256), 0, (hipStream_t)stream, (const uint16_t*)weight,
                       (uint16_t*)u, Cout, Cin);
    return launch_status();
}

#ifdef GD_NN_EXPERIMENTAL_STREAM
#include "nn_conv_stream_api.h"
#endif

int gd_nn_conv3x3_wide_supported(int N, int H, int W, int Cin, int Cout)
{
    if (N <= 0 || H < 16 || W < 16 || Cin <= 0 || Cout < 64) return 0;
    if (Cin % kWideCK || Cout % 8) return 0;
    if ((double)N * H * W * Cin * 2.0 >= 2147483648.0 || (double)gd_nn_conv3x3_wide_weights_bytes(Cout, Cin) >= 2147483648.0) return 0;
    return 1;
}

static int launch_wide(void* stream, const void* x, const float* mean_rstd, const void* gamma, const void* beta, int groups,
                       int apply_silu, const void* u, const void* bias, int bias_img_stride, const void* residual, void* y,
                       int N, int H, int W, int Cin, int Cout, float* stat_part)
{
    if (!x || !u || !y) return fail(GD_NN_ERR_INVALID_ARG, "null pointer");
    if (!gd_nn_conv3x3_wide_supported(N, H, W, Cin, Cout))
        return fail(GD_NN_ERR_INVALID_ARG, "conv3x3_wide: need Cin % 32 == 0, Cout % 8 == 0, Cout >= 64, H, W >= 16, tensors < 2 GiB");
    if (mean_rstd && (!gamma || !beta || groups <= 0 || Cin % groups))
        return fail(GD_NN_ERR_INVALID_ARG, "conv3x3_wide: GroupNorm needs gamma, beta and Cin % groups == 0");
    const TiledArgs a = {stream, x, mean_rstd, gamma, beta, groups, apply_silu, u, bias, bias_img_stride, residual, y,
                         N, H, W, Cin, Cout, stat_part};
    if (residual)
        return mean_rstd ? launch_tiled<conv3x3_wide_kernel<true, true>>(a, kWideLds, 32, 128, false)
                         : launch_tiled<conv3x3_wide_kernel<false, true>>(a, kWideLds, 32, 128, false);
    return mean_rstd ? launch_tiled<conv3x3_wide_kernel<true, false>>(a, kWideStages, 32, 128, false)
                     : launch_tiled<conv3x3_wide_kernel<false, false>>(a, kWideStages, 32, 128, false);
}

int gd_nn_conv3x3_wide_forward(void* stream, const void* x, const void* u, const void* bias, int bias_img_stride,
                               const void* residual, void* y, int N, int H, int W, int Cin, int Cout, float* stat_part)
{
    return launch_wide(stream, x, nullptr, nullptr, nullptr, 0, 0, u, bias, bias_img_stride, residual, y, N, H, W, Cin,
                       Cout, stat_part);
}

int gd_nn_conv3x3_wide_gn_forward(void* stream, const void* x, const float* mean_rstd, const void* gamma, const void* beta,
                                  int groups, int apply_silu, const void* u, const void* bias, int bias_img_stride,
                                  const void* residual, void* y, int N, int H, int W, int Cin, int Cout, float* stat_part)
{
    if (!mean_rstd) return fail(GD_NN_ERR_INVALID_ARG, "conv3x3_wide_gn: mean_rstd is NULL");
    return launch_wide(stream, x, mean_rstd, gamma, beta, groups, apply_silu, u, bias, bias_img_stride, residual, y, N, H, W,
                       Cin, Cout, stat_part);
}

#ifdef GD_NN_EXPERIMENTAL_REGW
#include "nn_conv_regw_api.h"
#endif

static int first_mfma_grid(int N, int H, int W)
{
    const int64_t tiles = (int64_t)N * H * ((W + 31) / 32);
    int64_t grid = (tiles + 3) / 4;
    const int64_t cap = 512;
    if (grid > cap) grid = cap;
    return (int)(grid < 1 ? 1 : grid);
}

size_t gd_nn_conv3x3_first_stat_rows(int N, int H, int W, int Cin, int Cout)
{
    if (N <= 0 || H <= 0 || W <= 0 || Cin < 1 || Cin > 4 || Cout != 128 || g_force_variant >= 0) return 0;
    return (size_t)first_mfma_grid(N, H, W) * 8;
}

static int first_forward(void* stream, const void* x, const void* weight, const void* bias, void* y, int N, int H, int W,
                         int Cin, int Cout, float* stat_part)
{
    if (!x || !weight || !y) return fail(GD_NN_ERR_INVALID_ARG, "null pointer");
    if (N <= 0 || H <= 0 || W <= 0 || Cin < 1 || Cin > 4 || Cout % 8 || Cout <= 0 || (size_t)9 * Cin * Cout * 4 > 65536)
        return fail(GD_NN_ERR_INVALID_ARG, "conv3x3_first: need 1 <= Cin <= 4, Cout % 8 == 0 and 36*Cin*Cout <= 64 KiB of LDS");
    if (stat_part && Cout != 128) return fail(GD_NN_ERR_INVALID_ARG, "conv3x3_first: statistics need Cout == 128");
    if (Cout == 128 && g_force_variant < 0) {
        if ((double)N * H * W * Cin >= 2147483648.0) return fail(GD_NN_ERR_INVALID_ARG, "conv3x3_first: tensor too large");
        const int grid = first_mfma_grid(N, H, W);
#define GD_FIRST_M(C_)                                                                                             \
    hipLaunchKernelGGL(conv3x3_first_mfma_kernel<C_>, dim3(grid), dim3(256), 0, (hipStream_t)stream,                \
                       (const uint16_t*)x, (const uint16_t*)weight, (const uint16_t*)bias, (uint16_t*)y, N, H, W, stat_part)
        if (Cin == 1) GD_FIRST_M(1);
        else if (Cin == 2) GD_FIRST_M(2);
        else if (Cin == 3) GD_FIRST_M(3);
        else GD_FIRST_M(4);
#undef GD_FIRST_M
        return launch_status();
    }
    const int octs = Cout / 8, gpb = 256 / octs;
    const int64_t groups = (int64_t)N * H * ((W + 3) / 4);
    const int64_t blocks = (groups + gpb - 1) / gpb;
    if (blocks > 2147483647LL) return fail(GD_NN_ERR_INVALID_ARG, "conv3x3_first: tensor too large");
    const size_t lds = (size_t)9 * Cin * Cout * sizeof(float);
    hipStream_t s = (hipStream_t)stream;
    const int first_grid = conv_env().first_grid;
    if (groups > 2147483647LL) return fail(GD_NN_ERR_INVALID_ARG, "conv3x3_first: tensor too large");
#define GD_FIRST(C_)                                                                                               \
    hipLaunchKernelGGL(conv3x3_first_kernel<C_>, dim3((unsigned)(blocks < first_grid ? blocks : first_grid)), dim3(256), lds, s, (const uint16_t*)x,    \
                       (const uint16_t*)weight, (const uint16_t*)bias, (uint16_t*)y, N, H, W, Cout)
    if (Cin == 1) GD_FIRST(1);
    else if (Cin == 2) GD_FIRST(2);
    else if (Cin == 3) GD_FIRST(3);
    else GD_FIRST(4);
#undef GD_FIRST
    return launch_status();
}

int gd_nn_conv3x3_first_forward(void* stream, const void* x, const void* weight, const void* bias, void* y, int N, int H,
                                int W, int Cin, int Cout)
{
    return first_forward(stream, x, weight, bias, y, N, H, W, Cin, Cout, nullptr);
}

int gd_nn_conv3x3_first_forward_stats(void* stream, const void* x, const void* weight, const void* bias, void* y, int N,
                                      int H, int W, int Cin, int Cout, float* stat_part)
{
    if (!stat_part) return fail(GD_NN_ERR_INVALID_ARG, "conv3x3_first_forward_stats: stat_part is NULL");
    return first_forward(stream, x, weight, bias, y, N, H, W, Cin, Cout, stat_part);
}

static ConvGeom s2_forward_geom(int Hin, int Win, int pad_lo)
{
    ConvGeom g = {};
    g.Hin = Hin; g.Win = Win;
    g.Hg = g.Hout = (Hin + pad_lo - 2) / 2 + 1;
    g.Wg = g.Wout = (Win + pad_lo - 2) / 2 + 1;
    g.sy = g.sx = 2;
    g.osy = g.osx = 1;
    for (int ky = 0; ky < 3; ky++)
        for (int kx = 0; kx < 3; kx++) add_tap(g, ky - pad_lo, kx - pad_lo, ky * 3 + kx);
    return g;
}

static bool s2_dgrad_geom(ConvGeom& g, int Hin, int Win, int pad_lo, int py, int px)
{
    const int Ho = (Hin + pad_lo - 2) / 2 + 1, Wo = (Win + pad_lo - 2) / 2 + 1;
    g = ConvGeom{};
    g.Hin = Ho; g.Win = Wo;
    g.Hg = (Hin - py + 1) / 2; g.Wg = (Win - px + 1) / 2;
    g.sy = g.sx = 1;
    g.Hout = Hin; g.Wout = Win;
    g.osy = g.osx = 2; g.ooy = py; g.oox = px;
    for (int ky = 0; ky < 3; ky++) {
        if ((py + pad_lo - ky) & 1) continue;
        for (int kx = 0; kx < 3; kx++) {
            if ((px + pad_lo - kx) & 1) continue;
            add_tap(g, (py + pad_lo - ky) / 2, (px + pad_lo - kx) / 2, 8 - (ky * 3 + kx));
        }
    }
    return g.Hg > 0 && g.Wg > 0;
}

static size_t geom_ws_bytes(int N, const ConvGeom& g, int Cin, int Cout)
{
    const int64_t M = (int64_t)N * g.Hg * g.Wg;
    const int split = choose_split(M, Cout, g.ntaps, Cin);
    return split > 1 ? split_ws_bytes(split, M, Cout) : 0;
}

size_t gd_nn_conv3x3_s2_ws_bytes(int N, int Hin, int Win, int Cin, int Cout, int pad_lo, int dgrad)
{
    if (N <= 0 || Hin < 2 || Win < 2 || Cin <= 0 || Cout <= 0 || Cin % 4 || Cout % 4) return 0;
    if (!dgrad) return Cin % BK ? 0 : geom_ws_bytes(N, s2_forward_geom(Hin, Win, pad_lo), Cin, Cout);
    if (Cout % BK) return 0;
    size_t need = 0;
    for (int py = 0; py < 2; py++)
        for (int px = 0; px < 2; px++) {
            ConvGeom g;
            if (!s2_dgrad_geom(g, Hin, Win, pad_lo, py, px)) continue;
            const size_t b = geom_ws_bytes(N, g, Cout, Cin);
            need = b > need ? b : need;
        }
    return need;
}

int gd_nn_conv3x3_s2_forward_ws(void* stream, const void* x, const void* weight, const void* bias, void* y, int N,
                                int Hin, int Win, int Cin, int Cout, int pad_lo, void* ws, size_t ws_bytes)
{
    if (!x || !weight || !y) return fail(GD_NN_ERR_INVALID_ARG, "null pointer");
// ... 176 lines not shown
```

garmentdreamer_amd/csrc/nn_conv_wide.h:

```cpp
#pragma once
#include "nn_device.h"

constexpr int kWideCK = 32;
constexpr int kWidePW = 34, kWidePix = 18 * kWidePW;
constexpr int kWidePStage = 2560 * 16;
constexpr int kWideWStage = 3 * 128 * kWideCK * 2;
constexpr int kWideStages = 2 * kWidePStage + 2 * kWideWStage;
constexpr int kWideRes = 16384;
constexpr int kWideLds = kWideStages + kWideRes;

__global__ __launch_bounds__(256) void conv3x3_wide_weights_kernel(const uint16_t* __restrict__ w, uint16_t* __restrict__ u,
                                                                   int Cout, int Cin)
{
    const int kc = Cin / kWideCK;
    const int tiles_n = (Cout + 127) / 128;
    const size_t total = (size_t)tiles_n * 3 * kc * 1536;
    for (size_t i = (size_t)blockIdx.x * blockDim.x + threadIdx.x; i < total; i += (size_t)gridDim.x * blockDim.x) {
        const int q = (int)(i % 1536);
        const size_t sl = i / 1536;
        const int c = (int)(sl % kc);
        const int ky = (int)((sl / kc) % 3);
        const int tn = (int)(sl / kc / 3);
        const int pc = q & 3, row = (q >> 2) & 127, kx = q >> 9;
        const int co = tn * 128 + row;
        const int ci0 = c * kWideCK + ((pc ^ ((row >> 2) & 3)) << 3);
        uint4 v = make_uint4(0u, 0u, 0u, 0u);
        if (co < Cout) v = *(const uint4*)(w + (((size_t)co * 3 + ky) * 3 + kx) * Cin + ci0);
        *(uint4*)(u + i * 8) = v;
    }
}

template <bool GN, bool RES>
__global__ __launch_bounds__(512) void conv3x3_wide_kernel(
    const uint16_t* __restrict__ in, const uint16_t* __restrict__ uw, const uint16_t* __restrict__ bias,
    int bias_img_stride, const uint16_t* __restrict__ residual, uint16_t* __restrict__ out, int Nimg, int H, int W,
    int Cin, int Cout, const float* __restrict__ mean_rstd, const uint16_t* __restrict__ gamma,
    const uint16_t* __restrict__ beta, int G, int apply_silu, int tiles_n, int tiles_x, int tiles_y, int nwg,
    float* __restrict__ stat_part)
{
    constexpr int THREADS = 512;
    typedef __attribute__((ext_vector_type(4))) uint32_t u32x4;
    extern __shared__ __attribute__((aligned(16))) char smem[];
    char* sP = smem;
    char* sW = smem + 2 * kWidePStage;

    const int tid = threadIdx.x, lane = tid & 63;
    const int wave = __builtin_amdgcn_readfirstlane(tid >> 6);
    int bid = blockIdx.x;
    if ((nwg & 7) == 0) bid = (bid & 7) * (nwg >> 3) + (bid >> 3);
    const int tn = bid % tiles_n, tm = bid / tiles_n;
    const int tpi = tiles_x * tiles_y;
    const int nimg = tm / tpi, trem = tm - nimg * tpi;
    const int tyi = trem / tiles_x, txi = trem - tyi * tiles_x;
    const int y0 = tyi * 16 - 1, x0 = txi * 32 - 1;
    const int n0 = tn * 128;

    const uint32_t row_bytes = (uint32_t)Cin * 2u;
    const __amdgpu_buffer_rsrc_t rs_in = buffer_rsrc(in, (uint32_t)Nimg * (uint32_t)(H * W) * row_bytes);
    const int kc = Cin / kWideCK;
    const __amdgpu_buffer_rsrc_t rs_w = buffer_rsrc(uw, (uint32_t)tiles_n * 3u * (uint32_t)kc * (uint32_t)kWideWStage);

    uint32_t p_goff[5];
    uint32_t p_keep = 0;
#pragma unroll
    for (int i = 0; i < 5; i++) {
        const int q = tid + THREADS * i;
        const int pix = q >> 2;
        const int py = (pix * 1928) >> 16, px = pix - py * kWidePW;
        const int gy = y0 + py, gx = x0 + px;
        const bool inimg = (pix < kWidePix) & ((unsigned)gy < (unsigned)H) & ((unsigned)gx < (unsigned)W);
        const int oct = GN ? (q & 3) : (q & 3) ^ ((pix >> 2) & 3);
        p_goff[i] = inimg ? (uint32_t)((nimg * H + gy) * W + gx) * row_bytes + (uint32_t)oct * 16u : kOOB;
        if (inimg) p_keep |= 1u << i;
    }
    auto issueP = [&](int buf, int c) {
        char* dst = sP + buf * kWidePStage;
#pragma unroll
        for (int i = 0; i < 5; i++) {
            if (i == 4 && wave == 7) continue;
            bload_lds16(rs_in, p_goff[i], (uint32_t)c * (kWideCK * 2), dst + (wave * 64 + THREADS * i) * 16);
        }
    };
    u32x4 p_reg[3];
    auto loadP = [&](int c, int i0, int i1) {
#pragma unroll
        for (int i = i0; i < i1; i++) {
            if (i == 4 && wave == 7) continue;
            p_reg[i - i0] = __builtin_bit_cast(u32x4, __builtin_amdgcn_raw_buffer_load_b128(rs_in, (int)p_goff[i],
                                                                                         (int)(c * (kWideCK * 2)), 0));
        }
    };
    const uint32_t sP_off = (uint32_t)(uintptr_t)sP;
    const uint32_t tab_off = (uint32_t)(uintptr_t)(smem + (RES ? kWideLds : kWideStages));
    auto storeP = [&](int buf, int c, int i0, int i1) {
        float sc[8], sh[8];
        gn_table_read(tab_off, c * (kWideCK / 8) + (tid & 3), sc, sh);
#pragma unroll
        for (int i = i0; i < i1; i++) {
            if (i == 4 && wave == 7) continue;
            const int q = tid + THREADS * i, pix = q >> 2;
            const bool keep = (p_keep >> i) & 1u;
            u32x4 v;
#pragma unroll
            for (int k = 0; k < 4; k++) {
                float lo = __uint_as_float(p_reg[i - i0][k] << 16), hi = __uint_as_float(p_reg[i - i0][k] & 0xffff0000u);
                lo = lo * sc[2 * k] + sh[2 * k];
                hi = hi * sc[2 * k + 1] + sh[2 * k + 1];
                if (apply_silu) { lo = silu_fast(lo); hi = silu_fast(hi); }
                v[k] = keep ? pack_bf16(lo, hi) : 0u;
            }
            asm volatile("ds_write_b128 %0, %1" ::"v"(sP_off + (uint32_t)(buf * kWidePStage) + (uint32_t)pix * 64u +
                                                       (uint32_t)(((q & 3) ^ ((pix >> 2) & 3)) << 4)), "v"(v) : "memory");
        }
    };
    const uint32_t w_voff = (uint32_t)tid * 16u;
    auto issueW = [&](int buf, int ky, int c) {
        char* dst = sW + buf * kWideWStage;
        const uint32_t soff = (uint32_t)((tn * 3 + ky) * kc + c) * (uint32_t)kWideWStage;
#pragma unroll
        for (int i = 0; i < 3; i++)
            bload_lds16(rs_w, w_voff + (uint32_t)(THREADS * 16 * i), soff, dst + (wave * 64 + THREADS * i) * 16);
    };

    const int wc = wave & 1, wr = wave >> 1;
    const int fk = lane >> 5, fn = lane & 31;
    int rr, fx;
    patch_col(fn, rr, fx);
    f32x16 acc[2][4];
#pragma unroll
    for (int a = 0; a < 2; a++)
#pragma unroll
        for (int b = 0; b < 4; b++)
#pragma unroll
            for (int k = 0; k < 16; k++) acc[a][b][k] = 0.f;
    int p_base[4];
#pragma unroll
    for (int b = 0; b < 4; b++) p_base[b] = (4 * wr + 2 * (b & 1) + rr) * kWidePW + 16 * (b >> 1) + fx;
    uint32_t a_rd[2];
#pragma unroll
    for (int a = 0; a < 2; a++) a_rd[a] = (uint32_t)((wc * 64 + a * 32 + fn) * 64);
    const uint32_t a_key = (uint32_t)((fn >> 2) & 3);

    const bool dma = RES && residual != nullptr && tyi * 16 + 16 <= H && txi * 32 + 32 <= W && n0 + 128 <= Cout &&
                     (uint64_t)Nimg * (uint64_t)(H * W) * (uint64_t)Cout * 2u < (1ull << 32);
    const uint32_t res_pix = (uint32_t)Cout * 2u, res_row = (uint32_t)W * res_pix;
    const __amdgpu_buffer_rsrc_t rs_res = buffer_rsrc(residual, (uint32_t)Nimg * (uint32_t)(H * W) * res_pix);
    auto res_slot = [&](int r) -> char* {
        if (r == 0 || r == 3) return sP + (kc & 1) * kWidePStage + wave * kResRound;
        return smem + 2 * kWidePStage + (r - 1) * (8 * kResRound) + wave * kResRound;
    };
    auto issueR = [&](int r) {
        uint32_t off[2];
        res_tile_lane(lane, res_pix, res_row, off);
        const uint32_t base = (uint32_t)((nimg * H + tyi * 16 + 4 * wr) * W + txi * 32 + 16 * (r >> 1)) * res_pix +
                              (uint32_t)(n0 + wc * 64 + (r & 1) * 32) * 2u;
        res_tile_issue(rs_res, off, base, 2u * res_row, res_slot(r));
    };

    const int nsteps = 3 * kc;
    if (GN) {
        gn_table_fill(tab_off, tid, THREADS, Cin, G, nimg, mean_rstd, gamma, beta);
        loadP(0, 0, 3);
        gn_table_sync();
        storeP(0, 0, 0, 3); loadP(0, 3, 5); storeP(0, 0, 3, 5);
    } else {
        issueP(0, 0);
    }
    issueW(0, 0, 0);
    int s = 0;
    for (int c = 0; c < kc; c++) {
        const char* pa = sP + (c & 1) * kWidePStage;
        for (int ky = 0; ky < 3; ky++, s++) {
            const int bufW = s & 1;
            asm volatile("s_waitcnt vmcnt(0) lgkmcnt(0)" ::: "memory");
            __syncthreads();
            if (s + 1 < nsteps) issueW(bufW ^ 1, ky == 2 ? 0 : ky + 1, ky == 2 ? c + 1 : c);
            if (c + 1 < kc) {
                if (GN) {
                    if (ky == 0) loadP(c + 1, 0, 3);
                    else if (ky == 1) { storeP((c + 1) & 1, c + 1, 0, 3); loadP(c + 1, 3, 5); }
                    else storeP((c + 1) & 1, c + 1, 3, 5);
                } else if (ky == 0) {
                    issueP((c + 1) & 1, c + 1);
                }
            } else if (ky == 0 && dma) {
                issueR(0);
            }
            const char* pw = sW + bufW * kWideWStage;
#pragma unroll 1
            for (int kx = 0; kx < 3; kx++) {
                uint32_t p_rd[4], p_sw[4];
#pragma unroll
                for (int b = 0; b < 4; b++) {
                    const int p = p_base[b] + ky * kWidePW + kx;
                    p_rd[b] = (uint32_t)p * 64u;
                    p_sw[b] = (uint32_t)((p >> 2) & 3);
                }
#pragma unroll
                for (int kk = 0; kk < 2; kk++) {
                    const uint32_t ch = (uint32_t)(kk * 2 + fk);
                    bf16x8_t wf[2], pf[4];
#pragma unroll
                    for (int a = 0; a < 2; a++)
                        wf[a] = *(const bf16x8_t*)(pw + kx * (128 * 64) + a_rd[a] + ((ch ^ a_key) << 4));
#pragma unroll
                    for (int b = 0; b < 4; b++) pf[b] = *(const bf16x8_t*)(pa + p_rd[b] + ((ch ^ p_sw[b]) << 4));
#pragma unroll
                    for (int a = 0; a < 2; a++)
#pragma unroll
                        for (int b = 0; b < 4; b++)
                            acc[a][b] = __builtin_amdgcn_mfma_f32_32x32x16_bf16(wf[a], pf[b], acc[a][b], 0, 0, 0);
                }
            }
        }
    }

    __syncthreads();
    if (dma) {
        const uint32_t tr_off = (uint32_t)(uintptr_t)(sP + ((kc - 1) & 1) * kWidePStage + wave * kTrWave);
        const uint16_t* bias_d = bias ? bias + (size_t)nimg * bias_img_stride : nullptr;
        uint2 bb[2][4];
#pragma unroll
        for (int a = 0; a < 2; a++)
#pragma unroll
            for (int q = 0; q < 4; q++)
                bb[a][q] = bias_d ? *(const uint2*)(bias_d + n0 + wc * 64 + a * 32 + 8 * q + 4 * fk) : make_uint2(0u, 0u);
        asm volatile("" ::: "memory");
        issueR(1);
        issueR(2);
        ResTile t;
        t.out = out; t.Cout = Cout;
        t.stat_rows = ((H + 15) / 16) * ((W + 15) / 16) * 8;
        t.stat_img = stat_part ? stat_part + (size_t)nimg * (Cout >> 2) * t.stat_rows * 2 : nullptr;
        const int t16x = (W + 15) / 16;
#pragma unroll
        for (int r = 0; r < 4; r++) {
            const int bh = r >> 1, a = r & 1;
            if (r == 1) asm volatile("s_waitcnt vmcnt(8)" ::: "memory");
            else if (r == 2) asm volatile("s_waitcnt vmcnt(4)" ::: "memory");
            else if (r == 3) asm volatile("s_waitcnt vmcnt(0)" ::: "memory");
            const int cx = 2 * txi + bh;
            t.pix0 = ((size_t)nimg * H + (tyi * 16 + 4 * wr)) * W + (txi * 32 + 16 * bh);
            t.stat_row = (tyi * t16x + cx) * 8 + wr * 2;
            t.stat_ok = cx < t16x;
            res_round(acc[a][2 * bh], acc[a][2 * bh + 1], bb[a], (uint32_t)(uintptr_t)res_slot(r), tr_off, lane, t,
                      n0 + wc * 64 + a * 32, PatchPix{W}, [&] { if (r == 0) issueR(3); });
        }
        return;
    }
    char* tr = smem + wave * kTrWave;
    const uint16_t* bias_n = bias ? bias + (size_t)nimg * bias_img_stride : nullptr;
    const int stat_rows = ((H + 15) / 16) * ((W + 15) / 16) * 8;
#pragma unroll
    for (int bh = 0; bh < 2; bh++) {
        bool ok[2];
        size_t opix[2];
#pragma unroll
        for (int j = 0; j < 2; j++) {
            const int oy = tyi * 16 + 4 * wr + 2 * j + rr, ox = txi * 32 + 16 * bh + fx;
            ok[j] = oy < H && ox < W;
            opix[j] = ((size_t)nimg * H + oy) * W + ox;
        }
        const int t16x = (W + 15) / 16, cx = 2 * txi + bh;
        const int stat_row = (tyi * t16x + cx) * 8 + wr * 2 + ((lane >> 4) & 1);
#pragma unroll
        for (int a = 0; a < 2; a++) {
#pragma unroll
            for (int q = 0; q < 4; q++) {
                const int co = n0 + wc * 64 + a * 32 + 8 * q + 4 * fk;
                const bool cok = co < Cout;
                float bv[4] = {0.f, 0.f, 0.f, 0.f};
                if (bias_n && cok) {
                    const uint2 bb = *(const uint2*)(bias_n + co);
                    bv[0] = bf2f((uint16_t)(bb.x & 0xffff)); bv[1] = bf2f((uint16_t)(bb.x >> 16));
                    bv[2] = bf2f((uint16_t)(bb.y & 0xffff)); bv[3] = bf2f((uint16_t)(bb.y >> 16));
                }
                float2 st = make_float2(0.f, 0.f);
#pragma unroll
                for (int j = 0; j < 2; j++) {
                    if (!ok[j] || !cok) continue;
                    const int b = 2 * bh + j;
                    float v[4];
#pragma unroll
                    for (int e = 0; e < 4; e++) v[e] = acc[a][b][4 * q + e] + bv[e];
                    if (residual) {
                        const uint2 rv = *(const uint2*)(residual + opix[j] * Cout + co);
                        v[0] += bf2f((uint16_t)(rv.x & 0xffff)); v[1] += bf2f((uint16_t)(rv.x >> 16));
                        v[2] += bf2f((uint16_t)(rv.y & 0xffff)); v[3] += bf2f((uint16_t)(rv.y >> 16));
                    }
                    uint2 o;
                    o.x = pack_bf16(v[0], v[1]);
                    o.y = pack_bf16(v[2], v[3]);
                    *(uint2*)(tr + (j * 32 + fn) * kTrRow + 16 * q + 8 * fk) = o;
                    if (stat_part) stat_accumulate(st, o);
                }
                if (stat_part) {
                    const float sx = row16_sum(st.x), sy = row16_sum(st.y);
                    if ((lane & 15) == 0 && cok && cx < t16x)
                        *(float2*)(stat_part + (((size_t)nimg * (Cout >> 2) + (co >> 2)) * stat_rows + stat_row) * 2) =
                            make_float2(sx, sy);
                }
            }
            __builtin_amdgcn_wave_barrier();
#pragma unroll
            for (int i = 0; i < 4; i++) {
                const int pr = (lane >> 2) + 16 * i, ch = lane & 3;
                int rr2, fx2;
                patch_col(pr & 31, rr2, fx2);
                const int oy = tyi * 16 + 4 * wr + 2 * (pr >> 5) + rr2, ox = txi * 32 + 16 * bh + fx2;
                const int co8 = n0 + wc * 64 + a * 32 + 8 * ch;
                if (oy < H && ox < W && co8 < Cout) {
                    const uint4 v = *(const uint4*)(tr + pr * kTrRow + ch * 16);
                    *(uint4*)(out + (((size_t)nimg * H + oy) * W + ox) * Cout + co8) = v;
                }
            }
            __builtin_amdgcn_wave_barrier();
        }
    }
}
```

garmentdreamer_amd/csrc/nn_conv_wino.h:

```cpp
#pragma once
#include "nn_device.h"

#ifndef GD_WINO_ABLATE
#define GD_WINO_ABLATE 0
#endif

constexpr int kWinoCK = 32;
constexpr int kWinoVStage = 4 * 18 * 8 * kWinoCK * 2;
constexpr int kWinoWStage = 4 * 128 * kWinoCK * 2;
constexpr int kWinoPBytes = 21 * 1024;
constexpr int kWinoLds = 2 * kWinoVStage + 2 * kWinoWStage + kWinoPBytes;

__device__ __forceinline__ uint16_t f2bf_finite(float f)
{
    uint32_t u = __float_as_uint(f);
    u += 0x7fffu + ((u >> 16) & 1u);
    return (uint16_t)(u >> 16);
}

__global__ __launch_bounds__(256) void conv3x3_wino_weights_kernel(const uint16_t* __restrict__ w,
                                                                   uint16_t* __restrict__ u, int Cout, int Cin)
{
    const int kc = Cin / kWinoCK;
    const int tiles_n = (Cout + 127) / 128;
// ... 111 lines not shown
        const uint32_t soff = (uint32_t)((tn * 3 + ky) * kc + c) * (uint32_t)kWinoWStage;
#pragma unroll
        for (int i = 0; i < 4; i++)
            bload_lds16(rs_w, w_voff + (uint32_t)(THREADS * 16 * i), soff, dst + (wave * 64 + THREADS * i) * 16);
    };
    auto transform_item = [&](char* dstV, int item) {
        const int c = item & 3, t = (item >> 2) & 7, r = item >> 5;
        const char* src = sP + (r * kPatch + 2 * t) * 64 + c * 16;
        u32x4 d[4];
#pragma unroll
        for (int j = 0; j < 4; j++) d[j] = *(const u32x4*)(src + j * 64);
        uint32_t v[4][4];
#pragma unroll
        for (int k = 0; k < 4; k++) {
            const uint32_t w0 = d[0][k], w1 = d[1][k], w2 = d[2][k], w3 = d[3][k];
            const float a0 = __uint_as_float(w0 << 16), b0 = __uint_as_float(w0 & 0xffff0000u);
            const float a1 = __uint_as_float(w1 << 16), b1 = __uint_as_float(w1 & 0xffff0000u);
            const float a2 = __uint_as_float(w2 << 16), b2 = __uint_as_float(w2 & 0xffff0000u);
            const float a3 = __uint_as_float(w3 << 16), b3 = __uint_as_float(w3 & 0xffff0000u);
            v[0][k] = pack_bf16(a0 - a2, b0 - b2);
            v[1][k] = pack_bf16(a1 + a2, b1 + b2);
            v[2][k] = pack_bf16(a2 - a1, b2 - b1);
            v[3][k] = pack_bf16(a1 - a3, b1 - b3);
        }
        const int key = ((r & 1) << 1) | (t >> 2);
        const uint32_t o = (uint32_t)(uintptr_t)(dstV + r * 512 + t * 64 + ((c ^ key) << 4));
#pragma unroll
        for (int p = 0; p < 4; p++) {
            const u32x4 pv = {v[p][0], v[p][1], v[p][2], v[p][3]};
            asm volatile("ds_write_b128 %0, %1 offset:%2" ::"v"(o), "v"(pv), "n"(p * 9216) : "memory");
        }
    };

    const int pp = wave & 1, wc = (wave >> 1) & 1, wq = wave >> 2;
    const int fk = lane >> 5, fn = lane & 31;
    f32x16 acc[2][2][2];
#pragma unroll
    for (int p = 0; p < 2; p++)
#pragma unroll
        for (int a = 0; a < 2; a++)
#pragma unroll
            for (int b = 0; b < 2; b++)
#pragma unroll
                for (int k = 0; k < 16; k++) acc[p][a][b][k] = 0.f;
    uint32_t a_rd[2], b_rd[2];
#pragma unroll
    for (int a = 0; a < 2; a++) a_rd[a] = (uint32_t)((wc * 64 + a * 32 + fn) * 64);
#pragma unroll
    for (int b = 0; b < 2; b++) b_rd[b] = (uint32_t)((wq * 8 + b * 4 + (fn >> 3)) * 512 + (fn & 7) * 64);
    const uint32_t a_key = (uint32_t)((fn >> 2) & 3);
    const uint32_t b_keylo = (uint32_t)((fn & 7) >> 2);

    const int nsteps = 3 * kc;
    if (GN) {
        gn_table_fill(tab_off, tid, THREADS, Cin, G, nimg, mean_rstd, gamma, beta);
        loadP(0);
        gn_table_sync();
        storeP(0);
    } else {
        issueP(0);
    }
    issueW(0, 0, 0);
    asm volatile("s_waitcnt vmcnt(0)" ::: "memory");
    __syncthreads();
    transform_item(sV, tid);
    if (wave == 0) transform_item(sV, 512 + lane);
    __syncthreads();
    if (kc > 1) { if (GN) { loadP(1); storeP(1); } else issueP(1); }
    int s = 0;
    for (int c = 0; c < kc; c++) {
        const char* pv = sV + (c & 1) * kWinoVStage;
        char* nv = sV + ((c + 1) & 1) * kWinoVStage;
        for (int ky = 0; ky < 3; ky++, s++) {
            const int bufW = s & 1;
            asm volatile("s_waitcnt vmcnt(0)" ::: "memory");
            __syncthreads();
            if (s + 1 < nsteps && GD_WINO_ABLATE != 2) issueW(bufW ^ 1, ky == 2 ? 0 : ky + 1, ky == 2 ? c + 1 : c);
            if (c + 1 < kc) {
                if (ky == 0) {
                    if (GD_WINO_ABLATE != 1) transform_item(nv, tid);
                    if (GN && c + 2 < kc) loadP(c + 2);
                } else if (ky == 1) {
                    if (wave == (c & 7) && GD_WINO_ABLATE != 1) transform_item(nv, 512 + lane);
                } else if (c + 2 < kc) {
                    if (GN) storeP(c + 2); else issueP(c + 2);
                }
            }
            const char* pw = sW + bufW * kWinoWStage;
            const uint32_t b_key = ((((uint32_t)(fn >> 3) + (uint32_t)ky) & 1u) << 1) | b_keylo;
#pragma unroll
            for (int kk = 0; kk < 2; kk++) {
                const uint32_t ch = (uint32_t)(kk * 2 + fk);
#pragma unroll
                for (int p = 0; p < 2; p++) {
                    const int pos = 2 * pp + p;
                    bf16x8_t wf[2], vf[2];
#pragma unroll
                    for (int a = 0; a < 2; a++)
                        wf[a] = *(const bf16x8_t*)(pw + pos * (128 * 64) + a_rd[a] + ((ch ^ a_key) << 4));
#pragma unroll
                    for (int b = 0; b < 2; b++)
                        vf[b] = *(const bf16x8_t*)(pv + pos * 9216 + b_rd[b] + ky * 512 + ((ch ^ b_key) << 4));
                    if (GD_WINO_ABLATE == 4) {
#pragma unroll
                        for (int a = 0; a < 2; a++)
#pragma unroll
                            for (int b = 0; b < 2; b++) acc[p][a][b][0] += (float)wf[a][0] * (float)vf[b][1];
                    } else {
#pragma unroll
                        for (int a = 0; a < 2; a++)
#pragma unroll
                            for (int b = 0; b < 2; b++)
                                acc[p][a][b] = __builtin_amdgcn_mfma_f32_32x32x16_bf16(wf[a], vf[b], acc[p][a][b], 0, 0, 0);
                    }
                }
            }
        }
    }

    __syncthreads();
    if (GD_WINO_ABLATE != 5) {
        char* mine = smem + wave * 16384;
#pragma unroll
        for (int a = 0; a < 2; a++)
#pragma unroll
            for (int b = 0; b < 2; b++) {
#pragma unroll
                for (int q = 0; q < 4; q++) {
                    f32x4 sd;
#pragma unroll
                    for (int e = 0; e < 4; e++) sd[e] = pp ? acc[0][a][b][4 * q + e] : acc[1][a][b][4 * q + e];
                    *(f32x4*)(mine + ((a * 2 + b) * 4 + q) * 1024 + lane * 16) = sd;
                }
            }
    }
    __syncthreads();
    {
        const char* theirs = smem + (wave ^ 1) * 16384;
#pragma unroll
        for (int a = 0; a < 2; a++)
#pragma unroll
            for (int b = 0; b < 2; b++)
#pragma unroll
                for (int q = 0; q < 4; q++) {
                    const f32x4 rv = GD_WINO_ABLATE == 5 ? f32x4{0.f, 1.f, 2.f, 3.f}
                                                         : *(const f32x4*)(theirs + ((a * 2 + b) * 4 + q) * 1024 + lane * 16);
#pragma unroll
                    for (int e = 0; e < 4; e++) {
                        const float sm = acc[0][a][b][4 * q + e] + acc[1][a][b][4 * q + e];
                        acc[0][a][b][4 * q + e] = pp ? rv[e] - sm : sm + rv[e];
                    }
                }
    }
    __syncthreads();

    char* tr = smem + wave * kTrWave;
    if (RES && residual != nullptr && tyi * 16 + 16 <= H && txi * 16 + 16 <= W && n0 + BN <= Cout && (Cout & 7) == 0 &&
        (uint64_t)Nimg * (uint64_t)(H * W) * (uint64_t)Cout * 2u < (1ull << 32)) {
        const uint32_t res_pix = (uint32_t)Cout * 2u, res_row = (uint32_t)W * res_pix;
        const __amdgpu_buffer_rsrc_t rs_res = buffer_rsrc(residual, (uint32_t)Nimg * (uint32_t)(H * W) * res_pix);
        const uint16_t* bias_d = bias ? bias + (size_t)nimg * bias_img_stride : nullptr;
        uint2 bb[2][4];
#pragma unroll
        for (int a = 0; a < 2; a++)
#pragma unroll
            for (int q = 0; q < 4; q++)
                bb[a][q] = bias_d ? *(const uint2*)(bias_d + n0 + wc * 64 + a * 32 + 8 * q + 4 * fk) : make_uint2(0u, 0u);
        asm volatile("" ::: "memory");
        const uint32_t lane_off = (uint32_t)(lane >> 5) * res_row + (uint32_t)(2 * ((lane >> 2) & 7)) * res_pix +
                                  (uint32_t)(((lane & 3) ^ ((lane >> 4) & 3)) * 16);
        const uint32_t base = (uint32_t)((nimg * H + tyi * 16 + wq * 8) * W + txi * 16 + pp) * res_pix + (uint32_t)(n0 + wc * 64) * 2u;
        char* slot = smem + 8 * kTrWave + wave * (2 * kResRound);
#pragma unroll
        for (int a = 0; a < 2; a++)
#pragma unroll
            for (int i = 0; i < 4; i++)
                bload_lds16(rs_res, lane_off, base + (uint32_t)(2 * i) * res_row + (uint32_t)(a * 64), slot + a * kResRound + i * 1024);
        ResTile t;
        t.out = out; t.Cout = Cout;
        t.pix0 = ((size_t)nimg * H + (tyi * 16 + wq * 8)) * W + txi * 16 + pp;
        t.stat_rows = tpi * 8;
        t.stat_img = stat_part ? stat_part + (size_t)nimg * (Cout >> 2) * t.stat_rows * 2 : nullptr;
        t.stat_row = (tyi * tiles_x + txi) * 8 + (pp * 2 + wq) * 2;
        t.stat_ok = true;
        const auto pix_of = [W](int pr) { return ((pr >> 5) * 4 + ((pr & 31) >> 3)) * W + 2 * (pr & 7); };
        asm volatile("s_waitcnt vmcnt(4)" ::: "memory");
        res_round(acc[0][0][0], acc[0][0][1], bb[0], (uint32_t)(uintptr_t)slot, (uint32_t)(uintptr_t)tr, lane, t, n0 + wc * 64,
                  pix_of, [] {});
        asm volatile("s_waitcnt vmcnt(0)" ::: "memory");
        res_round(acc[0][1][0], acc[0][1][1], bb[1], (uint32_t)(uintptr_t)(slot + kResRound), (uint32_t)(uintptr_t)tr, lane, t,
                  n0 + wc * 64 + 32, pix_of, [] {});
        return;
    }
    bool ok[2];
    size_t opix[2];
#pragma unroll
    for (int b = 0; b < 2; b++) {
        const int oy = tyi * 16 + wq * 8 + b * 4 + (fn >> 3), ox = txi * 16 + 2 * (fn & 7) + pp;
        ok[b] = oy < H && ox < W;
        opix[b] = ((size_t)nimg * H + oy) * W + ox;
    }
    const uint16_t* bias_n = bias ? bias + (size_t)nimg * bias_img_stride : nullptr;
    const int stat_rows = tpi * 8;
    const int stat_row = (tyi * tiles_x + txi) * 8 + (pp * 2 + wq) * 2 + ((lane >> 4) & 1);
    const bool wide = (Cout & 7) == 0;
#pragma unroll
    for (int a = 0; a < 2; a++) {
#pragma unroll
        for (int q = 0; q < 4; q++) {
            const int co = n0 + wc * 64 + a * 32 + 8 * q + 4 * fk;
            const bool cok = co < Cout;
            float bv[4] = {0.f, 0.f, 0.f, 0.f};
            if (bias_n && cok) {
                const uint2 bb = *(const uint2*)(bias_n + co);
                bv[0] = bf2f((uint16_t)(bb.x & 0xffff)); bv[1] = bf2f((uint16_t)(bb.x >> 16));
                bv[2] = bf2f((uint16_t)(bb.y & 0xffff)); bv[3] = bf2f((uint16_t)(bb.y >> 16));
            }
            float2 st = make_float2(0.f, 0.f);
#pragma unroll
            for (int b = 0; b < 2; b++) {
                if (!ok[b] || !cok) continue;
                float v[4];
#pragma unroll
                for (int e = 0; e < 4; e++) v[e] = acc[0][a][b][4 * q + e] + bv[e];
                if (residual) {
                    const uint2 rv = *(const uint2*)(residual + opix[b] * Cout + co);
                    v[0] += bf2f((uint16_t)(rv.x & 0xffff)); v[1] += bf2f((uint16_t)(rv.x >> 16));
                    v[2] += bf2f((uint16_t)(rv.y & 0xffff)); v[3] += bf2f((uint16_t)(rv.y >> 16));
                }
                uint2 o;
                o.x = pack_bf16(v[0], v[1]);
                o.y = pack_bf16(v[2], v[3]);
                if (wide) *(uint2*)(tr + (b * 32 + fn) * kTrRow + 16 * q + 8 * fk) = o;
                else *(uint2*)(out + opix[b] * Cout + co) = o;
                if (stat_part) stat_accumulate(st, o);
            }
            if (stat_part) {
                const float sx = row16_sum(st.x), sy = row16_sum(st.y);
                if ((lane & 15) == 0 && cok)
                    *(float2*)(stat_part + (((size_t)nimg * (Cout >> 2) + (co >> 2)) * stat_rows + stat_row) * 2) =
                        make_float2(sx, sy);
            }
        }
        if (wide) {
            __builtin_amdgcn_wave_barrier();
#pragma unroll
            for (int i = 0; i < 4; i++) {
                const int pr = (lane >> 2) + 16 * i, ch = lane & 3;
                const int oy = tyi * 16 + wq * 8 + (pr >> 5) * 4 + ((pr & 31) >> 3), ox = txi * 16 + 2 * (pr & 7) + pp;
                const int co8 = n0 + wc * 64 + a * 32 + 8 * ch;
                if (oy < H && ox < W && co8 < Cout) {
                    const uint4 v = *(const uint4*)(tr + pr * kTrRow + ch * 16);
                    if (GD_WINO_ABLATE != 6 || H < 0) *(uint4*)(out + (((size_t)nimg * H + oy) * W + ox) * Cout + co8) = v;
                }
            }
            __builtin_amdgcn_wave_barrier();
        }
    }
}
```

garmentdreamer_amd/nn_ops.py:

```python
from __future__ import annotations

import ctypes as C
import os
import weakref

import torch
import torch.nn.functional as F

_HERE = os.path.dirname(os.path.abspath(__file__))
_LIB_PATH = os.path.join(_HERE, "libgd_nn.so")
_LIB_OVERRIDDEN = False
_lib = None


def use_library(path: str) -> None:
    global _LIB_PATH, _LIB_OVERRIDDEN
    if _lib is not None:
        raise RuntimeError("libgd_nn.so is already loaded")
    _LIB_PATH, _LIB_OVERRIDDEN = os.path.abspath(path), True


_vp, _i, _f = C.c_void_p, C.c_int, C.c_float
SIGNATURES = {
    "gd_nn_groupnorm_silu_forward": (_i, [_vp, _vp, _vp, _vp, _vp, _i, _i, _i, _i, _f, _i, _vp, _vp]),
    "gd_nn_groupnorm_silu_fused_supported": (_i, [_i, _i, _i, _i]),
    "gd_nn_groupnorm_silu_fused_forward": (_i, [_vp, _vp, _vp, _vp, _vp, _i, _i, _i, _i, _f, _i]),
    "gd_nn_groupnorm_silu_fused_forward_stats": (_i, [_vp, _vp, _vp, _vp, _vp, _i, _i, _i, _i, _f, _i, _vp]),
    "gd_nn_groupnorm_silu_fused_backward": (_i, [_vp, _vp, _vp, _vp, _vp, _vp, _vp, _i, _i, _i, _i, _i]),
    "gd_nn_groupnorm_silu_fused_backward_supported": (_i, [_i, _i, _i, _i]),
    "gd_nn_groupnorm_silu_backward": (_i, [_vp, _vp, _vp, _vp, _vp, _vp, _vp, _i, _i, _i, _i, _i, _vp, _vp, _vp]),
    "gd_nn_groupnorm_ws_bytes": (C.c_size_t, [_i, _i]),
    "gd_nn_conv3x3_forward": (_i, [_vp, _vp, _vp, _vp, _i, _vp, _vp, _i, _i, _i, _i, _i]),
    "gd_nn_conv3x3_ws_bytes": (C.c_size_t, [_i, _i, _i, _i, _i]),
    "gd_nn_conv3x3_forward_ws": (_i, [_vp, _vp, _vp, _vp, _i, _vp, _vp, _i, _i, _i, _i, _i, _vp, C.c_size_t]),
    "gd_nn_conv_force_split": (_i, [_i]),
    "gd_nn_conv_set_route_scale": (_i, [_i]),
    "gd_nn_conv3x3_flip_weights": (_i, [_vp, _vp, _vp, _i, _i]),
    "gd_nn_conv3x3_first_dgrad_supported": (_i, [_i, _i, _i, _i, _i]),
    "gd_nn_conv3x3_first_dgrad_weights": (_i, [_vp, _vp, _vp, _i, _i]),
    "gd_nn_conv3x3_first_dgrad": (_i, [_vp, _vp, _vp, _vp, _i, _i, _i, _i, _i]),
    "gd_nn_groupnorm_stats": (_i, [_vp, _vp, _i, _i, _i, _i, _f, _vp, _vp]),
    "gd_nn_groupnorm_silu_forward_fp8": (_i, [_vp, _vp, _vp, _vp, _vp, _i, _i, _i, _i, _f, _i, _vp, _vp, _f]),
    "gd_nn_conv3x3_gn_forward": (_i, [_vp, _vp, _vp, _vp, _vp, _i, _i, _vp, _vp, _i, _vp, _vp, _i, _i, _i, _i, _i]),
    "gd_nn_linear_320_supported": (_i, [C.c_int64, _i, _i]),
    "gd_nn_linear_320_forward": (_i, [_vp, _vp, _vp, _vp, _vp, C.c_int64]),
    "gd_nn_linear_k320_forward": (_i, [_vp, _vp, _vp, _vp, _vp, C.c_int64, _i]),
    "gd_nn_linear_k320_geglu_forward": (_i, [_vp, _vp, _vp, _vp, _vp, C.c_int64, _i]),
    "gd_nn_linear_320_last_error": (C.c_char_p, []),
    "gd_nn_conv3x3_stat_rows": (C.c_size_t, [_i, _i, _i, _i, _i]),
    "gd_nn_conv3x3_first_stat_rows": (C.c_size_t, [_i, _i, _i, _i, _i]),
    "gd_nn_conv3x3_first_forward_stats": (_i, [_vp, _vp, _vp, _vp, _vp, _i, _i, _i, _i, _i, _vp]),
    "gd_nn_conv3x3_gn_forward_stats": (_i, [_vp, _vp, _vp, _vp, _vp, _i, _i, _vp, _vp, _i, _vp, _vp, _i, _i, _i, _i, _i,
                                            _vp]),
    "gd_nn_conv3x3_forward_stats": (_i, [_vp, _vp, _vp, _vp, _i, _vp, _vp, _i, _i, _i, _i, _i, _vp]),
    "gd_nn_conv3x3_wino_supported": (_i, [_i, _i, _i, _i, _i]),
    "gd_nn_conv3x3_wino_weights": (_i, [_vp, _vp, _vp, _i, _i]),
    "gd_nn_conv3x3_wino_weights_bytes": (C.c_size_t, [_i, _i]),
    "gd_nn_conv3x3_wino_forward": (_i, [_vp, _vp, _vp, _vp, _i, _vp, _vp, _i, _i, _i, _i, _i, _vp]),
    "gd_nn_conv3x3_wino_gn_forward": (_i, [_vp, _vp, _vp, _vp, _vp, _i, _i, _vp, _vp, _i, _vp, _vp, _i, _i, _i, _i, _i, _vp]),
    "gd_nn_conv3x3_wide_supported": (_i, [_i, _i, _i, _i, _i]),
    "gd_nn_conv3x3_wide_weights": (_i, [_vp, _vp, _vp, _i, _i]),
    "gd_nn_conv3x3_wide_weights_bytes": (C.c_size_t, [_i, _i]),
    "gd_nn_conv3x3_wide_forward": (_i, [_vp, _vp, _vp, _vp, _i, _vp, _vp, _i, _i, _i, _i, _i, _vp]),
    "gd_nn_conv3x3_wide_gn_forward": (_i, [_vp, _vp, _vp, _vp, _vp, _i, _i, _vp, _vp, _i, _vp, _vp, _i, _i, _i, _i, _i, _vp]),
    "gd_nn_groupnorm_finish_partials": (_i, [_vp, _vp, _i, C.c_size_t, _i, _i, _i, _f, _vp]),
    "gd_nn_conv3x3_first_forward": (_i, [_vp, _vp, _vp, _vp, _vp, _i, _i, _i, _i, _i]),
    "gd_nn_conv3x3_s2_forward": (_i, [_vp, _vp, _vp, _vp, _vp, _i, _i, _i, _i, _i, _i]),
    "gd_nn_conv3x3_s2_dgrad": (_i, [_vp, _vp, _vp, _vp, _i, _i, _i, _i, _i, _i]),
    "gd_nn_conv3x3_s2_ws_bytes": (C.c_size_t, [_i, _i, _i, _i, _i, _i, _i]),
    "gd_nn_conv3x3_s2_forward_ws": (_i, [_vp, _vp, _vp, _vp, _vp, _i, _i, _i, _i, _i, _i, _vp, C.c_size_t]),
    "gd_nn_conv3x3_s2_dgrad_ws": (_i, [_vp, _vp, _vp, _vp, _i, _i, _i, _i, _i, _i, _vp, C.c_size_t]),
    "gd_nn_conv3x3_up2_forward": (_i, [_vp, _vp, _vp, _vp, _vp, _vp, _i, _i, _i, _i, _i]),
    "gd_nn_conv_force_variant": (_i, [_i]),
    "gd_nn_linear_forward": (_i, [_vp, _vp, _vp, _vp, _vp, _vp, C.c_int64, _i, _i]),
    "gd_nn_gemm_supported": (_i, [C.c_int64, _i, _i, _i]),
    "gd_nn_gemm_forward": (_i, [_vp, _vp, _vp, _vp, _vp, _vp, C.c_int64, _i, _i]),
    "gd_nn_gemm_geglu_forward": (_i, [_vp, _vp, _vp, _vp, _vp, C.c_int64, _i, _i]),
    "gd_nn_gemm_last_error": (C.c_char_p, []),
    "gd_nn_conv_profile_enable": (_i, [_i]),
    "gd_nn_conv_profile_reset": (_i, []),
    "gd_nn_conv_profile_read": (_i, [C.POINTER(C.c_double), C.POINTER(C.c_int64), C.POINTER(C.c_double)]),
    "gd_nn_conv_profile_read_bytes": (_i, [C.POINTER(C.c_double)]),
    "gd_nn_geglu_forward": (_i, [_vp, _vp, _vp, C.c_int64, _i]),
    "gd_nn_geglu_backward": (_i, [_vp, _vp, _vp, _vp, C.c_int64, _i]),
    "gd_nn_conv1x1_c8": (_i, [_vp, _vp, _vp, _vp, _vp, C.c_int64, _i]),
    "gd_nn_softmax_rows_forward": (_i, [_vp, _vp, _vp, C.c_int64, _i]),
    "gd_nn_softmax_rows_backward": (_i, [_vp, _vp, _vp, _vp, C.c_int64, _i]),
    "gd_nn_layernorm_backward": (_i, [_vp, _vp, _vp, _vp, _vp, _vp, C.c_int64, _i, C.c_float]),
    "gd_nn_add_layernorm_forward": (_i, [_vp, _vp, _vp, _vp, _vp, _f, _vp, _vp, C.c_int64, _i]),
    "gd_nn_add_layernorm_forward_bcast": (_i, [_vp, _vp, _vp, _vp, _vp, _f, _vp, _vp, C.c_int64, _i, C.c_int64]),
    "gd_nn_join_stat_rows": (C.c_size_t, [_i, _i, _i]),
    "gd_nn_add_gn_partials": (_i, [_vp, _vp, _vp, _vp, _vp, _i, _i, _i, _i]),
    "gd_nn_concat_gn_partials": (_i, [_vp, _vp, _vp, _vp, _vp, _i, _i, _i, _i, _i]),
    "gd_nn_attention_ws_bytes": (C.c_size_t, [_i, _i, _i]),
    "gd_nn_attention_d64_forward": (_i, [_vp, _vp, _vp, _vp, _vp, _vp, _i, _i, _i, _i, C.c_int64, _i, C.c_int64, _i,
                                         C.c_int64, _i, C.c_int64, _i, _f, _i]),
    "gd_nn_attention_d64_forward_lse": (_i, [_vp, _vp, _vp, _vp, _vp, _vp, _vp, _i, _i, _i, _i, C.c_int64, _i, C.c_int64, _i,
                                             C.c_int64, _i, C.c_int64, _i, _f, _i]),
    "gd_nn_attention_bwd_ws_bytes": (C.c_size_t, [_i, _i, _i, _i]),
    "gd_nn_attention_d64_backward": (_i, [_vp] * 11 + [_i, _i, _i, _i] + [C.c_int64, _i] * 8 + [_f, _i]),
    "gd_nn_attention_d64_forward_vt": (_i, [_vp, _vp, _vp, _vp, _vp, _i, _i, _i, _i, C.c_int64, _i, C.c_int64, _i, C.c_int64, _i,
                                            _f]),
    "gd_nn_attention_d64_forward_vt_strided": (_i, [_vp, _vp, _vp, _vp, _vp, _i, _i, _i, _i, C.c_int64, _i, C.c_int64, _i, C.c_int64,
                                                    C.c_int64, _i, _f, _i]),
    "gd_nn_attention_last_error": (C.c_char_p, []),
    "gd_nn_vae_prologue_forward": (_i, [_vp, _vp, _vp, _i, _i, _i, _i, _i]),
    "gd_nn_vae_prologue_backward": (_i, [_vp, _vp, _vp, _i, _i, _i, _i, _i, _i]),
    "gd_nn_sparsity_forward": (_i, [_vp, _vp, _vp, C.c_int64, _vp]),
    "gd_nn_sparsity_backward": (_i, [_vp, _vp, _vp, _vp, C.c_int64, _vp]),
    "gd_nn_prologue_last_error": (C.c_char_p, []),
    "gd_nn_fp8_quantize": (_i, [_vp, _vp, _vp, C.c_int64, _f]),
    "gd_nn_fp8_pack_weights": (_i, [_vp, _vp, _vp, C.c_int64, _i, _i, _f]),
    "gd_nn_fp8_linear_forward": (_i, [_vp, _vp, _vp, _vp, _vp, _vp, C.c_int64, _i, _i, _i, _f]),
    "gd_nn_fp8_conv3x3_forward": (_i, [_vp, _vp, _vp, _vp, _i, _vp, _vp, _i, _i, _i, _i, _i, _i, _f]),
    "gd_nn_fp8_last_error": (C.c_char_p, []),
    "gd_nn_conv_last_error": (C.c_char_p, []),
    "gd_nn_elementwise_last_error": (C.c_char_p, []),
    "gd_nn_lora_rowdot": (_i, [_vp, _vp, _vp, _vp, C.c_int64, _i, C.c_float, _i]),
    "gd_nn_lora_rank4_add": (_i, [_vp, _vp, _vp, _vp, _vp, C.c_int64, _i, _i]),
    "gd_nn_lora_row_fused": (_i, [_vp, _vp, _vp, _vp, _vp, _vp, _vp, C.c_int64, _i, _i, C.c_float, _i]),
    "gd_nn_lora_colreduce_scratch_floats": (C.c_size_t, [C.c_int64, _i]),
    "gd_nn_lora_colreduce": (_i, [_vp, _vp, _vp, _vp, _vp, C.c_int64, _i, C.c_float, _i]),
    "gd_nn_lora_colreduce_pair_scratch_floats": (C.c_size_t, [C.c_int64, _i, _i]),
    "gd_nn_lora_colreduce_pair": (_i, [_vp, _vp, _vp, _vp, _vp, _vp, _vp, _vp, C.c_int64, _i, _i]),
    "gd_nn_lora_colreduce_pair_into": (_i, [_vp, _vp, _vp, _vp, _vp, _vp, _vp, _vp, C.c_int64, _i, _i, _i]),
    "gd_nn_lora_colreduce_group_entry_bytes": (C.c_size_t, []),
    "gd_nn_lora_colreduce_group_desc": (_i, [_vp, _vp, _vp, _vp, _vp, _vp, _vp, _vp, C.c_int64, _i, _i, _i, C.POINTER(C.c_int)]),
    "gd_nn_lora_colreduce_group_launch": (_i, [_vp, _vp, _i, _i, _i, _i]),
    "gd_nn_lora_last_error": (C.c_char_p, []),
    "gd_nn_vae_decoder_stem_supported": (_i, [_i, _i, _i, _i]),
    "gd_nn_vae_decoder_stem": (_i, [_vp, _vp, _i, _f, _vp, _vp, _vp, _vp, _vp, _i, _i, _i, _i]),
    "gd_nn_vae_decoder_head_supported": (_i, [_i, _i, _i, _i, _i]),
    "gd_nn_vae_decoder_head": (_i, [_vp, _vp, _vp, _vp, _vp, _i, _vp, _vp, _vp, _i, _i, _i, _i, _i]),
    "gd_nn_vae_decoder_last_error": (C.c_char_p, []),
    "gd_nn_last_error": (C.c_char_p, []),
}


def lib():
    global _lib
    if _lib is None:
        if not os.path.exists(_LIB_PATH):
            raise RuntimeError(f"{_LIB_PATH} not found: build with `python -m garmentdreamer_amd._build`; "
                               "the HIP guidance kernels have no fallback on GPU tensors")
        L = C.CDLL(_LIB_PATH)
        for name, (res, args) in SIGNATURES.items():
            try:
                fn = getattr(L, name)
            except AttributeError:
                if _LIB_OVERRIDDEN:
                    continue
                raise
            fn.restype, fn.argtypes = res, args
        _lib = L
    return _lib


def _check(ret, what, err="gd_nn_last_error"):
    if ret < 0:
        raise RuntimeError(f"{what} failed ({ret}): {getattr(lib(), err)().decode()}")


_gn_ws_cache = {}
_WS_TAG = [None]


class workspace_tag:

    def __init__(self, tag):
        self.tag = tag

    def __enter__(self):
        self.prev, _WS_TAG[0] = _WS_TAG[0], self.tag
        return self

    def __exit__(self, *exc):
        _WS_TAG[0] = self.prev
        return False


def _gn_workspace(x, N, groups):
    stream = torch.cuda.current_stream(x.device)
    key = (x.device.index, stream.cuda_stream, _WS_TAG[0])
    need = lib().gd_nn_groupnorm_ws_bytes(N, groups)
    ws = _gn_ws_cache.get(key)
    if ws is None or ws.numel() < need:
        ws = _gn_ws_cache[key] = torch.zeros(max(need, 1 << 16), dtype=torch.uint8, device=x.device)
    return ws


def reset_workspaces():
    _gn_ws_cache.clear()


_FALLBACKS = {}
_STRICT = False


def set_strict_library(on: bool) -> None:
    global _STRICT
    _STRICT = bool(on)


def library_fallbacks(reset: bool = False) -> dict:
    out = dict(_FALLBACKS)
    if reset:
        _FALLBACKS.clear()
    return out


def _note_fallback(op: str, x, why: str) -> None:
    if not (torch.is_tensor(x) and x.is_cuda and x.dtype == torch.bfloat16):
        return
    key = f"{op}: {why}"
    if _STRICT:
        raise RuntimeError(f"nn_ops strict mode: {key} on a bf16 GPU tensor of shape {tuple(x.shape)} would run on the PyTorch library op")
    _FALLBACKS[key] = _FALLBACKS.get(key, 0) + 1


def _is_nhwc_bf16(x):
    return x.is_cuda and x.dtype == torch.bfloat16 and x.dim() == 4 and x.is_contiguous(memory_format=torch.channels_last)


class _GroupNormSiLU(torch.autograd.Function):
    @staticmethod
    def forward(ctx, x, weight, bias, groups, eps, silu, mean_rstd=None):
# ... 1831 lines not shown
```

include/gd_nn.h:

```cpp
#ifndef GD_NN_H_INCLUDED
#define GD_NN_H_INCLUDED

#include <stddef.h>
#include <stdint.h>

#ifdef __cplusplus
extern "C" {
#endif

#define GD_NN_OK 0
#define GD_NN_ERR_INVALID_ARG (-1)
#define GD_NN_ERR_HIP (-2)

int gd_nn_groupnorm_silu_forward(void* stream, const void* x, void* y, const void* gamma, const void* beta, int N,
                                 int HW, int C, int G, float eps, int apply_silu, double* stats_ws,
                                 float* mean_rstd);

int gd_nn_groupnorm_silu_backward(void* stream, const void* x, const void* dy, const void* gamma,
                                  const void* beta, const float* mean_rstd, void* dx, int N, int HW, int C, int G,
                                  int apply_silu, double* stats_ws, float* group_sums ,
                                  const void* add);

size_t gd_nn_groupnorm_ws_bytes(int N, int G);

int gd_nn_conv3x3_forward(void* stream, const void* x, const void* weight, const void* bias, int bias_img_stride,
                          const void* residual, void* y, int N, int H, int W, int Cin, int Cout);

int gd_nn_conv3x3_flip_weights(void* stream, const void* weight, void* flipped, int Cout, int Cin);

int gd_nn_conv3x3_first_dgrad_supported(int N, int H, int W, int Cin, int Cout);
int gd_nn_conv3x3_first_dgrad_weights(void* stream, const void* weight, void* wpack, int Cout, int Cin);
int gd_nn_conv3x3_first_dgrad(void* stream, const void* dy, const void* wpack, void* dx4, int N, int H, int W, int Cin, int Cout);

int gd_nn_conv_force_variant(int v);

int gd_nn_linear_forward(void* stream, const void* x, const void* weight, const void* bias, const void* residual, void* y,
                         int64_t M, int K, int Nout);
int gd_nn_gemm_supported(int64_t M, int K, int N, int geglu);
int gd_nn_gemm_forward(void* stream, const void* x, const void* weight, const void* bias, const void* residual, void* y,
                       int64_t M, int K, int N);
int gd_nn_gemm_geglu_forward(void* stream, const void* x, const void* weight, const void* bias, void* y, int64_t M, int K,
                             int inner);
const char* gd_nn_gemm_last_error(void);
int gd_nn_conv_profile_enable(int on);
int gd_nn_conv_profile_reset(void);
int gd_nn_conv_profile_read(double* total_ms, int64_t* launches, double* total_flops);
int gd_nn_conv_profile_read_bytes(double* total_bytes);

size_t gd_nn_conv3x3_ws_bytes(int N, int H, int W, int Cin, int Cout);
int gd_nn_conv3x3_forward_ws(void* stream, const void* x, const void* weight, const void* bias, int bias_img_stride,
                             const void* residual, void* y, int N, int H, int W, int Cin, int Cout, void* ws,
                             size_t ws_bytes);
int gd_nn_conv_force_split(int s);
int gd_nn_conv_set_route_scale(int k);

int gd_nn_groupnorm_silu_fused_supported(int N, int HW, int C, int G);
int gd_nn_groupnorm_silu_fused_forward(void* stream, const void* x, void* y, const void* gamma, const void* beta, int N,
                                       int HW, int C, int G, float eps, int apply_silu);
int gd_nn_groupnorm_silu_fused_forward_stats(void* stream, const void* x, void* y, const void* gamma, const void* beta, int N,
                                             int HW, int C, int G, float eps, int apply_silu, float* mean_rstd);
int gd_nn_groupnorm_silu_fused_backward_supported(int N, int HW, int C, int G);
int gd_nn_groupnorm_silu_fused_backward(void* stream, const void* x, const void* dy, const void* gamma, const void* beta,
                                        const float* mean_rstd, void* dx, int N, int HW, int C, int G, int apply_silu);

int gd_nn_groupnorm_stats(void* stream, const void* x, int N, int HW, int C, int G, float eps, double* stats_ws,
                          float* mean_rstd);

int gd_nn_conv3x3_gn_forward(void* stream, const void* x, const float* mean_rstd, const void* gamma, const void* beta,
                             int groups, int apply_silu, const void* weight, const void* bias, int bias_img_stride,
                             const void* residual, void* y, int N, int H, int W, int Cin, int Cout);

size_t gd_nn_conv3x3_stat_rows(int N, int H, int W, int Cout, int gn_entry);
int gd_nn_conv3x3_gn_forward_stats(void* stream, const void* x, const float* mean_rstd, const void* gamma,
                                   const void* beta, int groups, int apply_silu, const void* weight, const void* bias,
                                   int bias_img_stride, const void* residual, void* y, int N, int H, int W, int Cin,
                                   int Cout, float* stat_part);
int gd_nn_conv3x3_forward_stats(void* stream, const void* x, const void* weight, const void* bias, int bias_img_stride,
                                const void* residual, void* y, int N, int H, int W, int Cin, int Cout, float* stat_part);
int gd_nn_conv3x3_wino_supported(int N, int H, int W, int Cin, int Cout);
size_t gd_nn_conv3x3_wino_weights_bytes(int Cout, int Cin);
int gd_nn_conv3x3_wino_weights(void* stream, const void* weight, void* u, int Cout, int Cin);
int gd_nn_conv3x3_wino_forward(void* stream, const void* x, const void* u, const void* bias, int bias_img_stride,
                               const void* residual, void* y, int N, int H, int W, int Cin, int Cout, float* stat_part);
int gd_nn_conv3x3_wino_gn_forward(void* stream, const void* x, const float* mean_rstd, const void* gamma, const void* beta,
                                  int groups, int apply_silu, const void* u, const void* bias, int bias_img_stride,
                                  const void* residual, void* y, int N, int H, int W, int Cin, int Cout, float* stat_part);
int gd_nn_conv3x3_wide_supported(int N, int H, int W, int Cin, int Cout);
size_t gd_nn_conv3x3_wide_weights_bytes(int Cout, int Cin);
int gd_nn_conv3x3_wide_weights(void* stream, const void* weight, void* u, int Cout, int Cin);
int gd_nn_conv3x3_wide_forward(void* stream, const void* x, const void* u, const void* bias, int bias_img_stride,
                               const void* residual, void* y, int N, int H, int W, int Cin, int Cout, float* stat_part);
int gd_nn_conv3x3_wide_gn_forward(void* stream, const void* x, const float* mean_rstd, const void* gamma, const void* beta,
                                  int groups, int apply_silu, const void* u, const void* bias, int bias_img_stride,
                                  const void* residual, void* y, int N, int H, int W, int Cin, int Cout, float* stat_part);
size_t gd_nn_conv3x3_first_stat_rows(int N, int H, int W, int Cin, int Cout);
int gd_nn_conv3x3_first_forward_stats(void* stream, const void* x, const void* weight, const void* bias, void* y, int N,
                                      int H, int W, int Cin, int Cout, float* stat_part);
int gd_nn_groupnorm_finish_partials(void* stream, const float* stat_part, int N, size_t rows, int C, int G, int HW,
                                    float eps, float* mean_rstd);

int gd_nn_linear_320_supported(int64_t M, int K, int N);
int gd_nn_linear_k320_forward(void* stream, const void* x, const void* weight, const void* bias, void* y, int64_t M, int N);
int gd_nn_linear_320_forward(void* stream, const void* x, const void* weight, const void* bias, void* y, int64_t M);
int gd_nn_linear_k320_geglu_forward(void* stream, const void* x, const void* weight, const void* bias, void* y, int64_t M,
                                    int inner);
const char* gd_nn_linear_320_last_error(void);

int gd_nn_conv3x3_first_forward(void* stream, const void* x, const void* weight, const void* bias, void* y, int N, int H,
                                int W, int Cin, int Cout);

int gd_nn_conv3x3_s2_forward(void* stream, const void* x, const void* weight, const void* bias, void* y, int N, int Hin,
                             int Win, int Cin, int Cout, int pad_lo);

int gd_nn_conv3x3_up2_forward(void* stream, const void* x, const void* w_even_rows, const void* w_odd_rows,
                              const void* bias, void* y, int N, int H, int W, int Cin, int Cout);

int gd_nn_conv3x3_s2_dgrad(void* stream, const void* dy, const void* weight_flipped, void* dx, int N, int Hin, int Win,
                           int Cin, int Cout, int pad_lo);

size_t gd_nn_conv3x3_s2_ws_bytes(int N, int Hin, int Win, int Cin, int Cout, int pad_lo, int dgrad);
int gd_nn_conv3x3_s2_forward_ws(void* stream, const void* x, const void* weight, const void* bias, void* y, int N,
                                int Hin, int Win, int Cin, int Cout, int pad_lo, void* ws, size_t ws_bytes);
int gd_nn_conv3x3_s2_dgrad_ws(void* stream, const void* dy, const void* weight_flipped, void* dx, int N, int Hin, int Win,
                              int Cin, int Cout, int pad_lo, void* ws, size_t ws_bytes);

int gd_nn_geglu_forward(void* stream, const void* x, void* y, int64_t rows, int inner);
int gd_nn_geglu_backward(void* stream, const void* x, const void* dy, void* dx, int64_t rows, int inner);
int gd_nn_layernorm_backward(void* stream, const void* s, const void* dy, const void* weight, const void* ds, void* dx,
                             int64_t rows, int C, float eps);

int gd_nn_add_layernorm_forward(void* stream, const void* x, const void* residual, const void* weight, const void* bias,
                                float eps, void* sum_out, void* y, int64_t rows, int C);
int gd_nn_add_layernorm_forward_bcast(void* stream, const void* x, const void* residual, const void* weight,
                                      const void* bias, float eps, void* sum_out, void* y, int64_t rows, int C,
                                      int64_t x_rows);

size_t gd_nn_join_stat_rows(int N, int HW, int C);
int gd_nn_add_gn_partials(void* stream, const void* a, const void* b, void* out, float* stat_part, int N, int Nb, int HW,
                          int C);
int gd_nn_concat_gn_partials(void* stream, const void* a, const void* b, void* out, float* stat_part, int N, int Nb, int HW,
                             int C0, int C1);

size_t gd_nn_attention_ws_bytes(int B, int Skv, int H);
int gd_nn_attention_d64_forward(void* stream, const void* q, const void* k, const void* v, void* o, void* vt_ws, int B, int S,
                                int Skv, int H, int64_t q_bs, int q_rs, int64_t k_bs, int k_rs, int64_t v_bs, int v_rs,
                                int64_t o_bs, int o_rs, float scale, int kv_len);
int gd_nn_attention_d64_forward_lse(void* stream, const void* q, const void* k, const void* v, void* o, float* lse, void* vt_ws,
                                    int B, int S, int Skv, int H, int64_t q_bs, int q_rs, int64_t k_bs, int k_rs, int64_t v_bs,
                                    int v_rs, int64_t o_bs, int o_rs, float scale, int kv_len);
size_t gd_nn_attention_bwd_ws_bytes(int B, int S, int Skv, int H);
int gd_nn_attention_d64_backward(void* stream, const void* q, const void* k, const void* v, const void* o, const void* dout,
                                 const float* lse, void* dq, void* dk, void* dv, void* ws, int B, int S, int Skv, int H,
                                 int64_t q_bs, int q_rs, int64_t k_bs, int k_rs, int64_t v_bs, int v_rs, int64_t o_bs, int o_rs,
                                 int64_t do_bs, int do_rs, int64_t dq_bs, int dq_rs, int64_t dk_bs, int dk_rs, int64_t dv_bs,
                                 int dv_rs, float scale, int kv_len);
int gd_nn_attention_d64_forward_vt(void* stream, const void* q, const void* k, const void* vt, void* o, int B, int S, int Skv,
                                   int H, int64_t q_bs, int q_rs, int64_t k_bs, int k_rs, int64_t o_bs, int o_rs, float scale);
int gd_nn_attention_d64_forward_vt_strided(void* stream, const void* q, const void* k, const void* vt, void* o, int B, int S,
                                           int Skv, int H, int64_t q_bs, int q_rs, int64_t k_bs, int k_rs, int64_t vt_bs,
                                           int64_t o_bs, int o_rs, float scale, int kv_len);
const char* gd_nn_attention_last_error(void);

int gd_nn_vae_prologue_forward(void* stream, const float* x, void* y, int N, int H, int W, int OH, int OW);
int gd_nn_vae_prologue_backward(void* stream, const void* dy, float* dx, int N, int H, int W, int OH, int OW, int CG);

int gd_nn_sparsity_forward(void* stream, const float* depth, const float* dmax, int64_t n, double* sums2);
int gd_nn_sparsity_backward(void* stream, const float* depth, const float* dmax, const float* grad_out, int64_t n,
                            float* d_depth);
const char* gd_nn_prologue_last_error(void);

int gd_nn_fp8_quantize(void* stream, const void* x_bf16, void* y_fp8, int64_t n, float inv_scale);
int gd_nn_groupnorm_silu_forward_fp8(void* stream, const void* x, void* y_fp8, const void* gamma, const void* beta, int N,
                                     int HW, int C, int G, float eps, int apply_silu, double* stats_ws, float* mean_rstd,
                                     float inv_scale);
int gd_nn_fp8_pack_weights(void* stream, const void* w_bf16, void* w_fp8, int64_t rows, int K, int Kp, float inv_scale);
int gd_nn_fp8_linear_forward(void* stream, const void* x_fp8, const void* w_fp8, const void* bias, const void* residual,
                             void* y, int64_t M, int K, int Kp, int Nout, float dq);
int gd_nn_fp8_conv3x3_forward(void* stream, const void* x_fp8, const void* w_fp8, const void* bias, int bias_img_stride,
                              const void* residual, void* y, int N, int H, int W, int Cin, int CinP, int Cout, float dq);
const char* gd_nn_fp8_last_error(void);

const char* gd_nn_conv_last_error(void);
int gd_nn_conv1x1_c8(void* stream, const void* x, const void* weight, const void* bias, void* y, int64_t npix, int transposed);
int gd_nn_softmax_rows_forward(void* stream, const void* x, void* y, int64_t rows, int L);
int gd_nn_softmax_rows_backward(void* stream, const void* p, const void* dp, void* ds, int64_t rows, int L);
const char* gd_nn_elementwise_last_error(void);
int gd_nn_lora_rowdot(void* stream, const void* a, const float* w, float* h, int64_t M, int K, float scale, int w_is_k_by_4);
int gd_nn_lora_rank4_add(void* stream, const float* h, const float* w, const void* base, void* y, int64_t M, int N, int w_is_n_by_4);
int gd_nn_lora_row_fused(void* stream, const void* a, const float* w1, const float* w2, const void* base, float* h, void* y,
                         int64_t M, int K, int N, float scale, int backward);
size_t gd_nn_lora_colreduce_scratch_floats(int64_t M, int J);
int gd_nn_lora_colreduce(void* stream, const void* a, const float* v, float* scratch, float* g, int64_t M, int J, float scale,
                         int g_is_j_by_4);
size_t gd_nn_lora_colreduce_pair_scratch_floats(int64_t M, int N, int K);
int gd_nn_lora_colreduce_pair(void* stream, const void* dy, const float* hs, const void* x, const float* dh, float* scratch,
                              float* d_up, float* d_down, int64_t M, int N, int K);
int gd_nn_lora_colreduce_pair_into(void* stream, const void* dy, const float* hs, const void* x, const float* dh, float* scratch,
                                   float* d_up, float* d_down, int64_t M, int N, int K, int accumulate);
size_t gd_nn_lora_colreduce_group_entry_bytes(void);
int gd_nn_lora_colreduce_group_desc(void* entry, const void* dy, const float* hs, const void* x, const float* dh, float* scratch,
                                    float* d_up, float* d_down, int64_t M, int N, int K, int accumulate, int* grid_xyz);
int gd_nn_lora_colreduce_group_launch(void* stream, const void* table_host, int n_entries, int grid1_x, int grid1_y, int grid2_x);
const char* gd_nn_lora_last_error(void);

int gd_nn_vae_decoder_stem_supported(int N, int h, int w, int Cout);
int gd_nn_vae_decoder_stem(void* stream, const void* latents, int latents_bf16, float inv_scale, const void* pq_weight,
// ... 16 lines not shown
```

Baseline: 23.59.

## Hoist epilogue bias/residual loads and add persistent streaming wide conv kernel

Conv epilogues now issue all bias loads (as bounds-checked buffer loads) and a round of residual loads up front, before the final barrier or store loop, so their latency overlaps instead of being serialized per quad. The LDS transpose store/readback in the patch epilogue is moved to inline asm with batched reads. A new persistent, double-buffered wide conv kernel is added for the no-residual, no-GroupNorm case and is chosen when the tile count divides evenly into the grid with enough tiles per workgroup. It also gets an optional grid-cap override. The hoisted loads raise register pressure, and the new kernel path adds complexity to routing.

```diff
diff --git a/garmentdreamer_amd/csrc/nn_conv3x3.hip b/garmentdreamer_amd/csrc/nn_conv3x3.hip
--- a/garmentdreamer_amd/csrc/nn_conv3x3.hip
+++ b/garmentdreamer_amd/csrc/nn_conv3x3.hip
@@ -191,6 +191,25 @@
         }
     }
 
+    uint2 bq[FB][FA][4];
+    {
+        const uint32_t bias_elems = (uint32_t)(Nimg - 1) * (uint32_t)bias_img_stride + (uint32_t)Cout;
+        const __amdgpu_buffer_rsrc_t rs_bias = buffer_rsrc(bias, bias && !partial ? bias_elems * 2u : 0u);
+#pragma unroll
+        for (int b = 0; b < FB; b++) {
+            const int64_t m = (int64_t)m0 + wp * (BM / WM) + b * 32 + (lane & 31);
+            const uint32_t row = m < M ? (uint32_t)(m / HW) * (uint32_t)bias_img_stride : kOOB;
+#pragma unroll
+            for (int a = 0; a < FA; a++)
+#pragma unroll
+                for (int q = 0; q < 4; q++) {
+                    const int co = n0 + wc * (BN / WN) + a * 32 + 8 * q + 4 * fk;
+                    const uint32_t voff = m < M && co < Cout ? (row + (uint32_t)co) * 2u : kOOB;
+                    bq[b][a][q] = __builtin_bit_cast(uint2, __builtin_amdgcn_raw_buffer_load_b64(rs_bias, (int)voff, 0, 0));
+                }
+        }
+        asm volatile("" ::: "memory");
+    }
 #pragma unroll
     for (int b = 0; b < FB; b++) {
         const int64_t m = (int64_t)m0 + wp * (BM / WM) + b * 32 + (lane & 31);
@@ -199,9 +218,17 @@
         const int rem = (int)(m - (int64_t)nimg * HW);
         const int ga = rem / g.Wg, gb = rem - ga * g.Wg;
         const size_t opix = ((size_t)nimg * g.Hout + (size_t)(ga * g.osy + g.ooy)) * g.Wout + (size_t)(gb * g.osx + g.oox);
-        const uint16_t* bias_n = bias ? bias + (size_t)nimg * bias_img_stride : nullptr;
 #pragma unroll
         for (int a = 0; a < FA; a++) {
+            uint2 rq[4];
+            if (residual && !partial) {
+#pragma unroll
+                for (int q = 0; q < 4; q++) {
+                    const int co = n0 + wc * (BN / WN) + a * 32 + 8 * q + 4 * fk;
+                    rq[q] = *(const uint2*)(residual + (co < Cout ? opix * Cout + co : (size_t)0));
+                }
+                asm volatile("" ::: "memory");
+            }
 #pragma unroll
             for (int q = 0; q < 4; q++) {
                 const int co = n0 + wc * (BN / WN) + a * 32 + 8 * q + 4 * fk;
@@ -214,13 +241,13 @@
                                           (((wave * FB + b) * FA + a) * 4 + q) * 64 + lane) * 4) = make_float4(v[0], v[1], v[2], v[3]);
                     continue;
                 }
-                if (bias_n) {
-                    const uint2 bb = *(const uint2*)(bias_n + co);
+                if (bias) {
+                    const uint2 bb = bq[b][a][q];
                     v[0] += bf2f((uint16_t)(bb.x & 0xffff)); v[1] += bf2f((uint16_t)(bb.x >> 16));
                     v[2] += bf2f((uint16_t)(bb.y & 0xffff)); v[3] += bf2f((uint16_t)(bb.y >> 16));
                 }
                 if (residual) {
-                    const uint2 rr = *(const uint2*)(residual + opix * Cout + co);
+                    const uint2 rr = rq[q];
                     v[0] += bf2f((uint16_t)(rr.x & 0xffff)); v[1] += bf2f((uint16_t)(rr.x >> 16));
                     v[2] += bf2f((uint16_t)(rr.y & 0xffff)); v[3] += bf2f((uint16_t)(rr.y >> 16));
                 }
@@ -282,6 +309,31 @@
     const float r2 = __uint_as_float(o.y << 16), r3 = __uint_as_float(o.y & 0xffff0000u);
     st.x += (r0 + r1) + (r2 + r3);
     st.y += fmaf(r0, r0, fmaf(r1, r1, fmaf(r2, r2, r3 * r3)));
+}
+
+template <int FA>
+__device__ __forceinline__ void epi_bias_quads(uint2 (&bq)[FA][4], const uint16_t* bias_n, int co0, int Cout)
+{
+    const __amdgpu_buffer_rsrc_t rs = buffer_rsrc(bias_n, bias_n ? (uint32_t)Cout * 2u : 0u);
+#pragma unroll
+    for (int a = 0; a < FA; a++)
+#pragma unroll
+        for (int q = 0; q < 4; q++)
+            bq[a][q] = __builtin_bit_cast(uint2, __builtin_amdgcn_raw_buffer_load_b64(rs, (co0 + a * 32 + 8 * q) * 2, 0, 0));
+    asm volatile("" ::: "memory");
+}
+
+__device__ __forceinline__ void epi_residual_round(uint2 (&rq)[2][4], const uint16_t* residual, const size_t (&opix)[2],
+                                                   const bool (&ok)[2], int co0, int Cout)
+{
+#pragma unroll
+    for (int j = 0; j < 2; j++)
+#pragma unroll
+        for (int q = 0; q < 4; q++) {
+            const int co = co0 + 8 * q;
+            rq[j][q] = *(const uint2*)(residual + (ok[j] && co < Cout ? opix[j] * Cout + co : (size_t)0));
+        }
+    asm volatile("" ::: "memory");
 }
 
 __device__ __forceinline__ void patch_col(int fn, int& rr, int& fx)
@@ -406,13 +458,14 @@
     }
 }
 
-template <int BN, int WN, int FA, int FB>
+template <int BN, int WN, int FA, int FB, bool HOIST>
 __device__ __forceinline__ void patch_epilogue(f32x16 (&acc)[FA][FB], char* tr, int nimg, int tyi, int txi, int n0, int wc,
-                                               int wp, int lane, int H, int W, int Cout, const uint16_t* __restrict__ bias,
-                                               int bias_img_stride, const uint16_t* __restrict__ residual,
-                                               uint16_t* __restrict__ out, float* __restrict__ stat_part, int tpi,
-                                               int tiles_x)
-{
+                                               int wp, int lane, int H, int W, int Cout, const uint2 (&bq)[FA][4],
+                                               const uint16_t* __restrict__ bias_n,
+                                               const uint16_t* __restrict__ residual, uint16_t* __restrict__ out,
+                                               float* __restrict__ stat_part, int tpi, int tiles_x)
+{
+    static_assert(FB == 2, "a round = two pixel blocks x four quads, four 16-pixel store instructions");
     const int fk = lane >> 5, fn = lane & 31;
     int rr, fx;
     patch_col(fn, rr, fx);
@@ -424,22 +477,21 @@
         ok[b] = oy < H && ox < W;
         opix[b] = ((size_t)nimg * H + oy) * W + ox;
     }
-    const uint16_t* bias_n = bias ? bias + (size_t)nimg * bias_img_stride : nullptr;
     const int stat_rows = tpi * 8;
     const int stat_row = (tyi * tiles_x + txi) * 8 + wp * 2 + ((lane >> 4) & 1);
     const bool wide = GD_PATCH_EPI != 2 && tr != nullptr && (Cout & 7) == 0;
+    const uint32_t tr_off = (uint32_t)(uintptr_t)tr;
 #pragma unroll
     for (int a = 0; a < FA; a++) {
+        uint2 rq[2][4];
+        if (HOIST && residual) epi_residual_round(rq, residual, opix, ok, n0 + wc * (BN / WN) + a * 32 + 4 * fk, Cout);
 #pragma unroll
         for (int q = 0; q < 4; q++) {
             const int co = n0 + wc * (BN / WN) + a * 32 + 8 * q + 4 * fk;
             const bool cok = co < Cout;
-            float bv[4] = {0.f, 0.f, 0.f, 0.f};
-            if (bias_n && cok) {
-                const uint2 bb = *(const uint2*)(bias_n + co);
-                bv[0] = bf2f((uint16_t)(bb.x & 0xffff)); bv[1] = bf2f((uint16_t)(bb.x >> 16));
-                bv[2] = bf2f((uint16_t)(bb.y & 0xffff)); bv[3] = bf2f((uint16_t)(bb.y >> 16));
-            }
+            const uint2 bb = HOIST ? bq[a][q] : bias_n && cok ? *(const uint2*)(bias_n + co) : make_uint2(0u, 0u);
+            const float bv[4] = {bf2f((uint16_t)(bb.x & 0xffff)), bf2f((uint16_t)(bb.x >> 16)),
+                                 bf2f((uint16_t)(bb.y & 0xffff)), bf2f((uint16_t)(bb.y >> 16))};
             float2 st = make_float2(0.f, 0.f);
 #pragma unroll
             for (int b = 0; b < FB; b++) {
@@ -448,15 +500,22 @@
 #pragma unroll
                 for (int e = 0; e < 4; e++) v[e] = acc[a][b][4 * q + e] + bv[e];
                 if (residual) {
-                    const uint2 rv = *(const uint2*)(residual + opix[b] * Cout + co);
+                    const uint2 rv = HOIST ? rq[b][q] : *(const uint2*)(residual + opix[b] * Cout + co);
                     v[0] += bf2f((uint16_t)(rv.x & 0xffff)); v[1] += bf2f((uint16_t)(rv.x >> 16));
                     v[2] += bf2f((uint16_t)(rv.y & 0xffff)); v[3] += bf2f((uint16_t)(rv.y >> 16));
                 }
                 uint2 o;
                 o.x = pack_bf16(v[0], v[1]);
                 o.y = pack_bf16(v[2], v[3]);
-                if (wide) *(uint2*)(tr + (b * 32 + fn) * kTrRow + 16 * q + 8 * fk) = o;
-                else if (GD_PATCH_EPI != 1 || H < 0) *(uint2*)(out + opix[b] * Cout + co) = o;
+                if (wide && HOIST) {
+                    const res_u32x2 ov = {o.x, o.y};
+                    asm volatile("ds_write_b64 %0, %1" ::"v"(tr_off + (uint32_t)((b * 32 + fn) * kTrRow + 16 * q + 8 * fk)), "v"(ov)
+                                 : "memory");
+                } else if (wide) {
+                    *(uint2*)(tr + (b * 32 + fn) * kTrRow + 16 * q + 8 * fk) = o;
+                } else if (GD_PATCH_EPI != 1 || H < 0) {
+                    *(uint2*)(out + opix[b] * Cout + co) = o;
+                }
                 if (stat_part) stat_accumulate(st, o);
             }
             if (stat_part) {
@@ -467,20 +526,28 @@
             }
         }
         if (wide) {
-            __builtin_amdgcn_wave_barrier();
-#pragma unroll
-            for (int i = 0; i < FB * 2; i++) {
+            res_u32x4 tv[4];
+            if (!HOIST) __builtin_amdgcn_wave_barrier();
+            else
+            asm volatile("ds_read_b128 %0, %4\n\tds_read_b128 %1, %4 offset:1280\n\tds_read_b128 %2, %4 offset:2560\n\t"
+                         "ds_read_b128 %3, %4 offset:3840\n\ts_waitcnt lgkmcnt(0)"
+                         : "=&v"(tv[0]), "=&v"(tv[1]), "=&v"(tv[2]), "=&v"(tv[3])
+                         : "v"(tr_off + (uint32_t)((lane >> 2) * kTrRow + (lane & 3) * 16))
+                         : "memory");
+            static_assert(16 * kTrRow == 1280, "offsets of the four reads");
+#pragma unroll
+            for (int i = 0; i < 4; i++) {
                 const int pr = (lane >> 2) + 16 * i, ch = lane & 3;
                 int rr2, fx2;
                 patch_col(pr & 31, rr2, fx2);
                 const int oy = tyi * 16 + 4 * wp + 2 * (pr >> 5) + rr2, ox = txi * 16 + fx2;
                 const int co8 = n0 + wc * (BN / WN) + a * 32 + 8 * ch;
-                if (oy < H && ox < W && co8 < Cout) {
-                    const uint4 v = *(const uint4*)(tr + pr * kTrRow + ch * 16);
-                    if (GD_PATCH_EPI != 1 || H < 0) *(uint4*)(out + (((size_t)nimg * H + oy) * W + ox) * Cout + co8) = v;
+                if (oy < H && ox < W && co8 < Cout && (GD_PATCH_EPI != 1 || H < 0)) {
+                    if (!HOIST) tv[i] = *(const res_u32x4*)(tr + pr * kTrRow + ch * 16);
+                    *(uint4*)(out + (((size_t)nimg * H + oy) * W + ox) * Cout + co8) = make_uint4(tv[i][0], tv[i][1], tv[i][2], tv[i][3]);
                 }
             }
-            __builtin_amdgcn_wave_barrier();
+            if (!HOIST) __builtin_amdgcn_wave_barrier();
         }
     }
 }
@@ -696,6 +763,9 @@
         }
     }
 
+    const uint16_t* bias_n = bias ? bias + (size_t)nimg * bias_img_stride : nullptr;
+    uint2 bq[FA][4] = {};
+    if (!(GD_PATCH_EPI == 0 && dma)) epi_bias_quads(bq, bias_n, n0 + wc * (BN / WN) + 4 * fk, Cout);
     if (GD_PATCH_EPI != 2) __syncthreads();
     if (GD_PATCH_EPI == 0 && dma) {
         const uint32_t tr_off = (uint32_t)(uintptr_t)(sA + ((kc - 1) & 1) * kAStage + wave * kTrWave);
@@ -726,8 +796,8 @@
         }
         return;
     }
-    patch_epilogue<BN, WN, FA, FB>(acc, sA + ((kc - 1) & 1) * kAStage + wave * kTrWave, nimg, tyi, txi, n0, wc, wp, lane, H, W,
-                                   Cout, bias, bias_img_stride, residual, out, stat_part, tpi, tiles_x);
+    patch_epilogue<BN, WN, FA, FB, true>(acc, sA + ((kc - 1) & 1) * kAStage + wave * kTrWave, nimg, tyi, txi, n0, wc, wp, lane, H, W,
+                                   Cout, bq, bias_n, residual, out, stat_part, tpi, tiles_x);
 }
 
 template <int BN, int WN, int WM, bool GN>
@@ -955,10 +1025,13 @@
             }
         }
 
+        constexpr bool kHoist = BN <= 128;
+        const uint16_t* bias_n = bias ? bias + (size_t)cur.nimg * bias_img_stride : nullptr;
+        uint2 bq[FA][4] = {};
+        if (kHoist) epi_bias_quads(bq, bias_n, cur.n0 + wc * (BN / WN) + 4 * fk, Cout);
         if (GD_PATCH_EPI != 2) __syncthreads();
-        patch_epilogue<BN, WN, FA, FB>(acc, sA + ((ga - 1) & 1) * kAStage + wave * kTrWave, cur.nimg, cur.tyi, cur.txi, cur.n0,
-                                       wc, wp, lane, H, W, Cout, bias, bias_img_stride, residual, out, stat_part, tpi,
-                                       tiles_x);
+        patch_epilogue<BN, WN, FA, FB, kHoist>(acc, sA + ((ga - 1) & 1) * kAStage + wave * kTrWave, cur.nimg, cur.tyi, cur.txi, cur.n0,
+                                       wc, wp, lane, H, W, Cout, bq, bias_n, residual, out, stat_part, tpi, tiles_x);
         if (!has_next) break;
         cur = nxt;
         vb = vnext;
@@ -1216,11 +1289,13 @@
 int g_route_scale = 1;
 int g_force_split = -1;
 int g_force_variant = -1;
+int g_wide_grid_cap = 0;
 
 struct ConvEnv {
     int split_px = 0;
     int multi_class = 1;
     int patch_persistent = 1;
+    int wide_persistent = 1;
     int first_grid = 2048;
 };
 const ConvEnv& conv_env()
@@ -1230,6 +1305,7 @@
         if (const char* e = getenv("GD_NN_SPLIT_PX")) v.split_px = atoi(e);
         if (const char* e = getenv("GD_NN_CONV_MULTI")) v.multi_class = atoi(e);
         if (const char* e = getenv("GD_NN_PATCH_PERSISTENT")) v.patch_persistent = atoi(e) != 0;
+        if (const char* e = getenv("GD_NN_WIDE_PERSISTENT")) v.wide_persistent = atoi(e) != 0;
         if (const char* e = getenv("GD_NN_FIRST_GRID")) v.first_grid = atoi(e) > 0 ? atoi(e) : v.first_grid;
         return v;
     }();
@@ -1312,8 +1388,13 @@
 };
 constexpr int kCuLds = 160 * 1024;
 static bool gn_table_fits(int lds, int Cin) { return lds + gn_table_bytes(Cin) <= kCuLds; }
+static int persistent_grid(int dev, int nwg)
+{
+    if (nwg <= num_cus(dev)) return nwg;
+    return (nwg & 7) == 0 ? (num_cus(dev) & ~7) : num_cus(dev);
+}
 template <auto Kern>
-int launch_tiled(const TiledArgs& a, int lds, int tile_w, int bn, bool persistent)
+int launch_tiled(const TiledArgs& a, int lds, int tile_w, int bn, bool persistent, int grid_cap = 0)
 {
     const int dev = current_device();
     if (dev < 0) return dev;
@@ -1325,8 +1406,8 @@
     hipStream_t s = (hipStream_t)a.stream;
     const int tiles_x = (a.W + tile_w - 1) / tile_w, tiles_y = (a.H + 15) / 16, tiles_n = (a.Cout + bn - 1) / bn;
     const int nwg = a.N * tiles_x * tiles_y * tiles_n;
-    int grid = nwg;
-    if (persistent && nwg > num_cus(dev)) grid = (nwg & 7) == 0 ? (num_cus(dev) & ~7) : num_cus(dev);
+    int grid = persistent ? persistent_grid(dev, nwg) : nwg;
+    if (persistent && grid_cap > 0) grid = nwg < grid_cap ? nwg : grid_cap;
     ProfScope prof(s);
     hipLaunchKernelGGL(Kern, dim3(grid), dim3(512), lds, s, (const uint16_t*)a.x, (const uint16_t*)a.w,
                        (const uint16_t*)a.bias, a.bias_img_stride, (const uint16_t*)a.residual, (uint16_t*)a.y, a.N, a.H,
@@ -1585,6 +1666,12 @@
     return split > 1 ? split_ws_bytes(split, M, Cout) : 0;
 }
 
+int gd_nn_conv_wide_persistent_cap(int cap)
+{
+    g_wide_grid_cap = cap > 0 ? cap : 0;
+    return GD_NN_OK;
+}
+
 int gd_nn_conv_force_split(int s)
 {
     g_force_split = s;
@@ -1752,6 +1839,17 @@
         return fail(GD_NN_ERR_INVALID_ARG, "conv3x3_wide: GroupNorm needs gamma, beta and Cin % groups == 0");
     const TiledArgs a = {stream, x, mean_rstd, gamma, beta, groups, apply_silu, u, bias, bias_img_stride, residual, y,
                          N, H, W, Cin, Cout, stat_part};
+    if (!residual && !mean_rstd) {
+        const int dev = current_device();
+        if (dev < 0) return dev;
+        const int nwg = N * ((W + 31) / 32) * ((H + 15) / 16) * ((Cout + 127) / 128);
+        bool pers = g_wide_grid_cap > 0;
+        if (!pers && conv_env().wide_persistent) {
+            const int grid = persistent_grid(dev, nwg);
+            pers = nwg % grid == 0 && nwg / grid >= 8;
+        }
+        if (pers) return launch_tiled<conv3x3_wide_stream_kernel>(a, kWideStages, 32, 128, true, g_wide_grid_cap);
+    }
     if (residual)
         return mean_rstd ? launch_tiled<conv3x3_wide_kernel<true, true>>(a, kWideLds, 32, 128, false)
                          : launch_tiled<conv3x3_wide_kernel<false, true>>(a, kWideLds, 32, 128, false);
diff --git a/garmentdreamer_amd/csrc/nn_conv_wide.h b/garmentdreamer_amd/csrc/nn_conv_wide.h
--- a/garmentdreamer_amd/csrc/nn_conv_wide.h
+++ b/garmentdreamer_amd/csrc/nn_conv_wide.h
@@ -30,6 +30,128 @@
     }
 }
 
+__device__ __forceinline__ void wide_step(f32x16 (&acc)[2][4], const char* pa, const char* pw, int ky, const int (&p_base)[4],
+                                          const uint32_t (&a_rd)[2], uint32_t a_key, int fk)
+{
+#pragma unroll 1
+    for (int kx = 0; kx < 3; kx++) {
+        uint32_t p_rd[4], p_sw[4];
+#pragma unroll
+        for (int b = 0; b < 4; b++) {
+            const int p = p_base[b] + ky * kWidePW + kx;
+            p_rd[b] = (uint32_t)p * 64u;
+            p_sw[b] = (uint32_t)((p >> 2) & 3);
+        }
+#pragma unroll
+        for (int kk = 0; kk < 2; kk++) {
+            const uint32_t ch = (uint32_t)(kk * 2 + fk);
+            bf16x8_t wf[2], pf[4];
+#pragma unroll
+            for (int a = 0; a < 2; a++)
+                wf[a] = *(const bf16x8_t*)(pw + kx * (128 * 64) + a_rd[a] + ((ch ^ a_key) << 4));
+#pragma unroll
+            for (int b = 0; b < 4; b++) pf[b] = *(const bf16x8_t*)(pa + p_rd[b] + ((ch ^ p_sw[b]) << 4));
+#pragma unroll
+            for (int a = 0; a < 2; a++)
+#pragma unroll
+                for (int b = 0; b < 4; b++)
+                    acc[a][b] = __builtin_amdgcn_mfma_f32_32x32x16_bf16(wf[a], pf[b], acc[a][b], 0, 0, 0);
+        }
+    }
+}
+
+template <bool ASM>
+__device__ __forceinline__ void wide_epilogue_lanes(f32x16 (&acc)[2][4], char* tr, const uint2 (&bq)[2][4],
+                                                    const uint16_t* __restrict__ residual, uint16_t* __restrict__ out,
+                                                    float* __restrict__ stat_part, int nimg, int tyi, int txi, int n0, int wc,
+                                                    int wr, int lane, int H, int W, int Cout)
+{
+    const int fk = lane >> 5, fn = lane & 31;
+    int rr, fx;
+    patch_col(fn, rr, fx);
+    const uint32_t tr_off = (uint32_t)(uintptr_t)tr;
+    (void)tr_off;
+    const int stat_rows = ((H + 15) / 16) * ((W + 15) / 16) * 8;
+#pragma unroll
+    for (int bh = 0; bh < 2; bh++) {
+        bool ok[2];
+        size_t opix[2];
+#pragma unroll
+        for (int j = 0; j < 2; j++) {
+            const int oy = tyi * 16 + 4 * wr + 2 * j + rr, ox = txi * 32 + 16 * bh + fx;
+            ok[j] = oy < H && ox < W;
+            opix[j] = ((size_t)nimg * H + oy) * W + ox;
+        }
+        const int t16x = (W + 15) / 16, cx = 2 * txi + bh;
+        const int stat_row = (tyi * t16x + cx) * 8 + wr * 2 + ((lane >> 4) & 1);
+#pragma unroll
+        for (int a = 0; a < 2; a++) {
+            uint2 rq[2][4];
+            if (residual) epi_residual_round(rq, residual, opix, ok, n0 + wc * 64 + a * 32 + 4 * fk, Cout);
+#pragma unroll
+            for (int q = 0; q < 4; q++) {
+                const int co = n0 + wc * 64 + a * 32 + 8 * q + 4 * fk;
+                const bool cok = co < Cout;
+                const float bv[4] = {bf2f((uint16_t)(bq[a][q].x & 0xffff)), bf2f((uint16_t)(bq[a][q].x >> 16)),
+                                     bf2f((uint16_t)(bq[a][q].y & 0xffff)), bf2f((uint16_t)(bq[a][q].y >> 16))};
+                float2 st = make_float2(0.f, 0.f);
+#pragma unroll
+                for (int j = 0; j < 2; j++) {
+                    if (!ok[j] || !cok) continue;
+                    const int b = 2 * bh + j;
+                    float v[4];
+#pragma unroll
+                    for (int e = 0; e < 4; e++) v[e] = acc[a][b][4 * q + e] + bv[e];
+                    if (residual) {
+                        const uint2 rv = rq[j][q];
+                        v[0] += bf2f((uint16_t)(rv.x & 0xffff)); v[1] += bf2f((uint16_t)(rv.x >> 16));
+                        v[2] += bf2f((uint16_t)(rv.y & 0xffff)); v[3] += bf2f((uint16_t)(rv.y >> 16));
+                    }
+                    uint2 o;
+                    o.x = pack_bf16(v[0], v[1]);
+                    o.y = pack_bf16(v[2], v[3]);
+                    if (ASM) {
+                        const res_u32x2 ov = {o.x, o.y};
+                        asm volatile("ds_write_b64 %0, %1" ::"v"(tr_off + (uint32_t)((j * 32 + fn) * kTrRow + 16 * q + 8 * fk)), "v"(ov)
+                                     : "memory");
+                    } else {
+                        *(uint2*)(tr + (j * 32 + fn) * kTrRow + 16 * q + 8 * fk) = o;
+                    }
+                    if (stat_part) stat_accumulate(st, o);
+                }
+                if (stat_part) {
+                    const float sx = row16_sum(st.x), sy = row16_sum(st.y);
+                    if ((lane & 15) == 0 && cok && cx < t16x)
+                        *(float2*)(stat_part + (((size_t)nimg * (Cout >> 2) + (co >> 2)) * stat_rows + stat_row) * 2) =
+                            make_float2(sx, sy);
+                }
+            }
+            res_u32x4 tv[4];
+            if (ASM)
+                asm volatile("ds_read_b128 %0, %4\n\tds_read_b128 %1, %4 offset:1280\n\tds_read_b128 %2, %4 offset:2560\n\t"
+                             "ds_read_b128 %3, %4 offset:3840\n\ts_waitcnt lgkmcnt(0)"
+                             : "=&v"(tv[0]), "=&v"(tv[1]), "=&v"(tv[2]), "=&v"(tv[3])
+                             : "v"(tr_off + (uint32_t)((lane >> 2) * kTrRow + (lane & 3) * 16))
+                             : "memory");
+            else
+                __builtin_amdgcn_wave_barrier();
+#pragma unroll
+            for (int i = 0; i < 4; i++) {
+                const int pr = (lane >> 2) + 16 * i, ch = lane & 3;
+                int rr2, fx2;
+                patch_col(pr & 31, rr2, fx2);
+                const int oy = tyi * 16 + 4 * wr + 2 * (pr >> 5) + rr2, ox = txi * 32 + 16 * bh + fx2;
+                const int co8 = n0 + wc * 64 + a * 32 + 8 * ch;
+                if (oy < H && ox < W && co8 < Cout) {
+                    if (!ASM) tv[i] = *(const res_u32x4*)(tr + pr * kTrRow + ch * 16);
+                    *(uint4*)(out + (((size_t)nimg * H + oy) * W + ox) * Cout + co8) = make_uint4(tv[i][0], tv[i][1], tv[i][2], tv[i][3]);
+                }
+            }
+            if (!ASM) __builtin_amdgcn_wave_barrier();
+        }
+    }
+}
+
 template <bool GN, bool RES>
 __global__ __launch_bounds__(512) void conv3x3_wide_kernel(
     const uint16_t* __restrict__ in, const uint16_t* __restrict__ uw, const uint16_t* __restrict__ bias,
@@ -187,34 +309,13 @@
                 issueR(0);
             }
             const char* pw = sW + bufW * kWideWStage;
-#pragma unroll 1
-            for (int kx = 0; kx < 3; kx++) {
-                uint32_t p_rd[4], p_sw[4];
-#pragma unroll
-                for (int b = 0; b < 4; b++) {
-                    const int p = p_base[b] + ky * kWidePW + kx;
-                    p_rd[b] = (uint32_t)p * 64u;
-                    p_sw[b] = (uint32_t)((p >> 2) & 3);
-                }
-#pragma unroll
-                for (int kk = 0; kk < 2; kk++) {
-                    const uint32_t ch = (uint32_t)(kk * 2 + fk);
-                    bf16x8_t wf[2], pf[4];
-#pragma unroll
-                    for (int a = 0; a < 2; a++)
-                        wf[a] = *(const bf16x8_t*)(pw + kx * (128 * 64) + a_rd[a] + ((ch ^ a_key) << 4));
-#pragma unroll
-                    for (int b = 0; b < 4; b++) pf[b] = *(const bf16x8_t*)(pa + p_rd[b] + ((ch ^ p_sw[b]) << 4));
-#pragma unroll
-                    for (int a = 0; a < 2; a++)
-#pragma unroll
-                        for (int b = 0; b < 4; b++)
-                            acc[a][b] = __builtin_amdgcn_mfma_f32_32x32x16_bf16(wf[a], pf[b], acc[a][b], 0, 0, 0);
-                }
-            }
-        }
-    }
-
+            wide_step(acc, pa, pw, ky, p_base, a_rd, a_key, fk);
+        }
+    }
+
+    const uint16_t* bias_n = bias ? bias + (size_t)nimg * bias_img_stride : nullptr;
+    uint2 bq[2][4] = {};
+    if (!dma) epi_bias_quads(bq, bias_n, n0 + wc * 64 + 4 * fk, Cout);
     __syncthreads();
     if (dma) {
         const uint32_t tr_off = (uint32_t)(uintptr_t)(sP + ((kc - 1) & 1) * kWidePStage + wave * kTrWave);
@@ -248,73 +349,138 @@
         }
         return;
     }
-    char* tr = smem + wave * kTrWave;
-    const uint16_t* bias_n = bias ? bias + (size_t)nimg * bias_img_stride : nullptr;
-    const int stat_rows = ((H + 15) / 16) * ((W + 15) / 16) * 8;
-#pragma unroll
-    for (int bh = 0; bh < 2; bh++) {
-        bool ok[2];
-        size_t opix[2];
-#pragma unroll
-        for (int j = 0; j < 2; j++) {
-            const int oy = tyi * 16 + 4 * wr + 2 * j + rr, ox = txi * 32 + 16 * bh + fx;
-            ok[j] = oy < H && ox < W;
-            opix[j] = ((size_t)nimg * H + oy) * W + ox;
-        }
-        const int t16x = (W + 15) / 16, cx = 2 * txi + bh;
-        const int stat_row = (tyi * t16x + cx) * 8 + wr * 2 + ((lane >> 4) & 1);
-#pragma unroll
-        for (int a = 0; a < 2; a++) {
-#pragma unroll
-            for (int q = 0; q < 4; q++) {
-                const int co = n0 + wc * 64 + a * 32 + 8 * q + 4 * fk;
-                const bool cok = co < Cout;
-                float bv[4] = {0.f, 0.f, 0.f, 0.f};
-                if (bias_n && cok) {
-                    const uint2 bb = *(const uint2*)(bias_n + co);
-                    bv[0] = bf2f((uint16_t)(bb.x & 0xffff)); bv[1] = bf2f((uint16_t)(bb.x >> 16));
-                    bv[2] = bf2f((uint16_t)(bb.y & 0xffff)); bv[3] = bf2f((uint16_t)(bb.y >> 16));
-                }
-                float2 st = make_float2(0.f, 0.f);
-#pragma unroll
-                for (int j = 0; j < 2; j++) {
-                    if (!ok[j] || !cok) continue;
-                    const int b = 2 * bh + j;
-                    float v[4];
-#pragma unroll
-                    for (int e = 0; e < 4; e++) v[e] = acc[a][b][4 * q + e] + bv[e];
-                    if (residual) {
-                        const uint2 rv = *(const uint2*)(residual + opix[j] * Cout + co);
-                        v[0] += bf2f((uint16_t)(rv.x & 0xffff)); v[1] += bf2f((uint16_t)(rv.x >> 16));
-                        v[2] += bf2f((uint16_t)(rv.y & 0xffff)); v[3] += bf2f((uint16_t)(rv.y >> 16));
+    wide_epilogue_lanes<false>(acc, smem + wave * kTrWave, bq, residual, out, stat_part, nimg, tyi, txi, n0, wc, wr, lane, H, W,
+                               Cout);
+}
+
+__global__ __launch_bounds__(512) void conv3x3_wide_stream_kernel(
+    const uint16_t* __restrict__ in, const uint16_t* __restrict__ uw, const uint16_t* __restrict__ bias,
+    int bias_img_stride, const uint16_t* __restrict__ residual, uint16_t* __restrict__ out, int Nimg, int H, int W,
+    int Cin, int Cout, const float* __restrict__ mean_rstd, const uint16_t* __restrict__ gamma,
+    const uint16_t* __restrict__ beta, int G, int apply_silu, int tiles_n, int tiles_x, int tiles_y, int nwg,
+    float* __restrict__ stat_part)
+{
+    constexpr int THREADS = 512;
+    extern __shared__ __attribute__((aligned(16))) char smem[];
+    char* sP = smem;
+    char* sW = smem + 2 * kWidePStage;
+
+    const int tid = threadIdx.x, lane = tid & 63;
+    const int wave = __builtin_amdgcn_readfirstlane(tid >> 6);
+    const int tpi = tiles_x * tiles_y;
+    const bool remap = (nwg & 7) == 0 && (gridDim.x & 7) == 0;
+    struct Tile { int nimg, tyi, txi, tn; };
+    auto decode = [&](int vb) {
+        int bid = vb;
+        if (remap) bid = (vb & 7) * (nwg >> 3) + (vb >> 3);
+        const int tm = bid / tiles_n;
+        Tile t;
+        t.tn = bid - tm * tiles_n;
+        t.nimg = tm / tpi;
+        const int trem = tm - t.nimg * tpi;
+        t.tyi = trem / tiles_x;
+        t.txi = trem - t.tyi * tiles_x;
+        return t;
+    };
+
+    const uint32_t row_bytes = (uint32_t)Cin * 2u;
+    const __amdgpu_buffer_rsrc_t rs_in = buffer_rsrc(in, (uint32_t)Nimg * (uint32_t)(H * W) * row_bytes);
+    const int kc = Cin / kWideCK;
+    const __amdgpu_buffer_rsrc_t rs_w = buffer_rsrc(uw, (uint32_t)tiles_n * 3u * (uint32_t)kc * (uint32_t)kWideWStage);
+
+    uint32_t p_goff[5];
+    auto setupP = [&](const Tile& t) {
+        const int y0 = t.tyi * 16 - 1, x0 = t.txi * 32 - 1;
+#pragma unroll
+        for (int i = 0; i < 5; i++) {
+            const int q = tid + THREADS * i;
+            const int pix = q >> 2;
+            const int py = (pix * 1928) >> 16, px = pix - py * kWidePW;
+            const int gy = y0 + py, gx = x0 + px;
+            const bool inimg = (pix < kWidePix) & ((unsigned)gy < (unsigned)H) & ((unsigned)gx < (unsigned)W);
+            const int oct = (q & 3) ^ ((pix >> 2) & 3);
+            p_goff[i] = inimg ? (uint32_t)((t.nimg * H + gy) * W + gx) * row_bytes + (uint32_t)oct * 16u : kOOB;
+        }
+    };
+    auto issueP = [&](int buf, int c) {
+        char* dst = sP + buf * kWidePStage;
+#pragma unroll
+        for (int i = 0; i < 5; i++) {
+            if (i == 4 && wave == 7) continue;
+            bload_lds16(rs_in, p_goff[i], (uint32_t)c * (kWideCK * 2), dst + (wave * 64 + THREADS * i) * 16);
+        }
+    };
+    const uint32_t w_voff = (uint32_t)tid * 16u;
+    auto issueW = [&](int buf, int tn, int ky, int c) {
+        char* dst = sW + buf * kWideWStage;
+        const uint32_t soff = (uint32_t)((tn * 3 + ky) * kc + c) * (uint32_t)kWideWStage;
+#pragma unroll
+        for (int i = 0; i < 3; i++)
+            bload_lds16(rs_w, w_voff + (uint32_t)(THREADS * 16 * i), soff, dst + (wave * 64 + THREADS * i) * 16);
+    };
+
+    const int wc = wave & 1, wr = wave >> 1;
+    const int fk = lane >> 5, fn = lane & 31;
+    int rr, fx;
+    patch_col(fn, rr, fx);
+    f32x16 acc[2][4];
+    int p_base[4];
+#pragma unroll
+    for (int b = 0; b < 4; b++) p_base[b] = (4 * wr + 2 * (b & 1) + rr) * kWidePW + 16 * (b >> 1) + fx;
+    uint32_t a_rd[2];
+#pragma unroll
+    for (int a = 0; a < 2; a++) a_rd[a] = (uint32_t)((wc * 64 + a * 32 + fn) * 64);
+    const uint32_t a_key = (uint32_t)((fn >> 2) & 3);
+
+    int vb = blockIdx.x;
+    Tile cur = decode(vb);
+    setupP(cur);
+    issueP(0, 0);
+    issueW(0, cur.tn, 0, 0);
+    int s = 0;
+    int gc = 0;
+    for (;;) {
+        const int vnext = vb + (int)gridDim.x;
+        const bool has_next = vnext < nwg;
+        const Tile nxt = decode(has_next ? vnext : vb);
+#pragma unroll
+        for (int a = 0; a < 2; a++)
+#pragma unroll
+            for (int b = 0; b < 4; b++)
+#pragma unroll
+                for (int k = 0; k < 16; k++) acc[a][b][k] = 0.f;
+        uint2 bq[2][4] = {};
+        for (int c = 0; c < kc; c++, gc++) {
+            const char* pa = sP + (gc & 1) * kWidePStage;
+            const bool last_chunk = c + 1 == kc;
+            for (int ky = 0; ky < 3; ky++, s++) {
+                const int bufW = s & 1;
+                asm volatile("s_waitcnt vmcnt(0) lgkmcnt(0)" ::: "memory");
+                __syncthreads();
+                if (!(last_chunk && ky == 2)) {
+                    issueW(bufW ^ 1, cur.tn, ky == 2 ? 0 : ky + 1, ky == 2 ? c + 1 : c);
+                } else {
+                    epi_bias_quads(bq, bias ? bias + (size_t)cur.nimg * bias_img_stride : nullptr, cur.tn * 128 + wc * 64 + 4 * fk,
+                                   Cout);
+                    issueW(bufW ^ 1, has_next ? nxt.tn : cur.tn, 0, 0);
+                }
+                if (ky == 0) {
+                    if (!last_chunk) {
+                        issueP((gc + 1) & 1, c + 1);
+                    } else if (has_next) {
+                        setupP(nxt);
+                        issueP((gc + 1) & 1, 0);
                     }
-                    uint2 o;
-                    o.x = pack_bf16(v[0], v[1]);
-                    o.y = pack_bf16(v[2], v[3]);
-                    *(uint2*)(tr + (j * 32 + fn) * kTrRow + 16 * q + 8 * fk) = o;
-                    if (stat_part) stat_accumulate(st, o);
-                }
-                if (stat_part) {
-                    const float sx = row16_sum(st.x), sy = row16_sum(st.y);
-                    if ((lane & 15) == 0 && cok && cx < t16x)
-                        *(float2*)(stat_part + (((size_t)nimg * (Cout >> 2) + (co >> 2)) * stat_rows + stat_row) * 2) =
-                            make_float2(sx, sy);
-                }
+                }
+                wide_step(acc, pa, sW + bufW * kWideWStage, ky, p_base, a_rd, a_key, fk);
             }
-            __builtin_amdgcn_wave_barrier();
-#pragma unroll
-            for (int i = 0; i < 4; i++) {
-                const int pr = (lane >> 2) + 16 * i, ch = lane & 3;
-                int rr2, fx2;
-                patch_col(pr & 31, rr2, fx2);
-                const int oy = tyi * 16 + 4 * wr + 2 * (pr >> 5) + rr2, ox = txi * 32 + 16 * bh + fx2;
-                const int co8 = n0 + wc * 64 + a * 32 + 8 * ch;
-                if (oy < H && ox < W && co8 < Cout) {
-                    const uint4 v = *(const uint4*)(tr + pr * kTrRow + ch * 16);
-                    *(uint4*)(out + (((size_t)nimg * H + oy) * W + ox) * Cout + co8) = v;
-                }
-            }
-            __builtin_amdgcn_wave_barrier();
-        }
-    }
+        }
+        asm volatile("s_waitcnt lgkmcnt(0)\n\ts_barrier" ::: "memory");
+        wide_epilogue_lanes<true>(acc, sP + ((gc - 1) & 1) * kWidePStage + wave * kTrWave, bq, nullptr, out, stat_part, cur.nimg,
+                                  cur.tyi, cur.txi, cur.tn * 128, wc, wr, lane, H, W, Cout);
+        if (!has_next) break;
+        cur = nxt;
+        vb = vnext;
+    }
+    asm volatile("s_waitcnt vmcnt(0)" ::: "memory");
 }
diff --git a/garmentdreamer_amd/csrc/nn_conv_wino.h b/garmentdreamer_amd/csrc/nn_conv_wino.h
--- a/garmentdreamer_amd/csrc/nn_conv_wino.h
+++ b/garmentdreamer_amd/csrc/nn_conv_wino.h
@@ -287,11 +287,15 @@
                     }
                 }
     }
+    const bool dma = RES && residual != nullptr && tyi * 16 + 16 <= H && txi * 16 + 16 <= W && n0 + BN <= Cout && (Cout & 7) == 0 &&
+                     (uint64_t)Nimg * (uint64_t)(H * W) * (uint64_t)Cout * 2u < (1ull << 32);
+    const uint16_t* bias_n = bias ? bias + (size_t)nimg * bias_img_stride : nullptr;
+    uint2 bq[2][4] = {};
+    if (!dma) epi_bias_quads(bq, bias_n, n0 + wc * 64 + 4 * fk, Cout);
     __syncthreads();
 
     char* tr = smem + wave * kTrWave;
-    if (RES && residual != nullptr && tyi * 16 + 16 <= H && txi * 16 + 16 <= W && n0 + BN <= Cout && (Cout & 7) == 0 &&
-        (uint64_t)Nimg * (uint64_t)(H * W) * (uint64_t)Cout * 2u < (1ull << 32)) {
+    if (dma) {
         const uint32_t res_pix = (uint32_t)Cout * 2u, res_row = (uint32_t)W * res_pix;
         const __amdgpu_buffer_rsrc_t rs_res = buffer_rsrc(residual, (uint32_t)Nimg * (uint32_t)(H * W) * res_pix);
         const uint16_t* bias_d = bias ? bias + (size_t)nimg * bias_img_stride : nullptr;
@@ -335,22 +339,19 @@
         ok[b] = oy < H && ox < W;
         opix[b] = ((size_t)nimg * H + oy) * W + ox;
     }
-    const uint16_t* bias_n = bias ? bias + (size_t)nimg * bias_img_stride : nullptr;
     const int stat_rows = tpi * 8;
     const int stat_row = (tyi * tiles_x + txi) * 8 + (pp * 2 + wq) * 2 + ((lane >> 4) & 1);
     const bool wide = (Cout & 7) == 0;
 #pragma unroll
     for (int a = 0; a < 2; a++) {
+        uint2 rq[2][4];
+        if (residual) epi_residual_round(rq, residual, opix, ok, n0 + wc * 64 + a * 32 + 4 * fk, Cout);
 #pragma unroll
         for (int q = 0; q < 4; q++) {
             const int co = n0 + wc * 64 + a * 32 + 8 * q + 4 * fk;
             const bool cok = co < Cout;
-            float bv[4] = {0.f, 0.f, 0.f, 0.f};
-            if (bias_n && cok) {
-                const uint2 bb = *(const uint2*)(bias_n + co);
-                bv[0] = bf2f((uint16_t)(bb.x & 0xffff)); bv[1] = bf2f((uint16_t)(bb.x >> 16));
-                bv[2] = bf2f((uint16_t)(bb.y & 0xffff)); bv[3] = bf2f((uint16_t)(bb.y >> 16));
-            }
+            const float bv[4] = {bf2f((uint16_t)(bq[a][q].x & 0xffff)), bf2f((uint16_t)(bq[a][q].x >> 16)),
+                                 bf2f((uint16_t)(bq[a][q].y & 0xffff)), bf2f((uint16_t)(bq[a][q].y >> 16))};
             float2 st = make_float2(0.f, 0.f);
 #pragma unroll
             for (int b = 0; b < 2; b++) {
@@ -359,7 +360,7 @@
 #pragma unroll
                 for (int e = 0; e < 4; e++) v[e] = acc[0][a][b][4 * q + e] + bv[e];
                 if (residual) {
-                    const uint2 rv = *(const uint2*)(residual + opix[b] * Cout + co);
+                    const uint2 rv = rq[b][q];
                     v[0] += bf2f((uint16_t)(rv.x & 0xffff)); v[1] += bf2f((uint16_t)(rv.x >> 16));
                     v[2] += bf2f((uint16_t)(rv.y & 0xffff)); v[3] += bf2f((uint16_t)(rv.y >> 16));
                 }
diff --git a/garmentdreamer_amd/nn_ops.py b/garmentdreamer_amd/nn_ops.py
--- a/garmentdreamer_amd/nn_ops.py
+++ b/garmentdreamer_amd/nn_ops.py
@@ -72,6 +72,7 @@
     "gd_nn_conv3x3_s2_dgrad_ws": (_i, [_vp, _vp, _vp, _vp, _i, _i, _i, _i, _i, _i, _vp, C.c_size_t]),
     "gd_nn_conv3x3_up2_forward": (_i, [_vp, _vp, _vp, _vp, _vp, _vp, _i, _i, _i, _i, _i]),
     "gd_nn_conv_force_variant": (_i, [_i]),
+    "gd_nn_conv_wide_persistent_cap": (_i, [_i]),
     "gd_nn_linear_forward": (_i, [_vp, _vp, _vp, _vp, _vp, _vp, C.c_int64, _i, _i]),
     "gd_nn_gemm_supported": (_i, [C.c_int64, _i, _i, _i]),
     "gd_nn_gemm_forward": (_i, [_vp, _vp, _vp, _vp, _vp, _vp, C.c_int64, _i, _i]),
diff --git a/include/gd_nn.h b/include/gd_nn.h
--- a/include/gd_nn.h
+++ b/include/gd_nn.h
@@ -52,6 +52,7 @@
                              const void* residual, void* y, int N, int H, int W, int Cin, int Cout, void* ws,
                              size_t ws_bytes);
 int gd_nn_conv_force_split(int s);
+int gd_nn_conv_wide_persistent_cap(int cap);
 int gd_nn_conv_set_route_scale(int k);
 
 int gd_nn_groupnorm_silu_fused_supported(int N, int HW, int C, int G);
```

Measured after the change: 23.53. No clear change (-0.2%).
